# duckietown/gym-duckietown

Measured on AMD Instinct MI355X. Metric: env-steps/sec (4096 envs, 640x480 RGB) at 1/2/4/8 MI355X; % HBM roofline, higher is better.
Workload: dtype f32 raster -> u8 frames; f64 physics

## Files before the change

gym-duckietown_amd/csrc/dtsim_api.hip:

```cpp
#include <hip/hip_runtime.h>

#include <cmath>
#include <cstdarg>
#include <cstdio>
#include <cstdlib>
#include <cstring>
#include <memory>
#include <string>
#include <vector>

#include "dtsim_dev.h"
#include <dlfcn.h>
#include <mutex>

namespace {

thread_local std::string g_err;

int fail(int code, const char* fmt, ...) {
  char buf[512];
  va_list ap;
  va_start(ap, fmt);
  vsnprintf(buf, sizeof buf, fmt, ap);
  va_end(ap);
  g_err = buf;
  return code;
}

#define HIPCHK(expr)                                                                       \
  do {                                                                                     \
    hipError_t _e = (expr);                                                                \
    if (_e != hipSuccess) return fail(DTSIM_E_HIP, "%s failed: %s", #expr, hipGetErrorString(_e)); \
  } while (0)

struct ProfSlot {
  std::vector<std::pair<hipEvent_t, hipEvent_t>> pending;
  std::vector<std::pair<hipEvent_t, hipEvent_t>> free_;
};

struct HipFree {
  void operator()(void* p) const { (void)hipFree(p); }
};
template <typename T>
using DevPtr = std::unique_ptr<T, HipFree>;

template <typename T>
hipError_t dev_alloc(DevPtr<T>& out, size_t n) {
  T* p = nullptr;
  hipError_t e = hipMalloc(&p, sizeof(T) * n);
  if (e == hipSuccess) out.reset(p);
  return e;
}

template <typename T>
hipError_t dev_upload(DevPtr<T>& out, const T* src, size_t n, size_t min_n = 0) {
  DevPtr<T> p;
  hipError_t e = dev_alloc(p, std::max(n, min_n));
  if (e == hipSuccess && n) e = hipMemcpy(p.get(), src, sizeof(T) * n, hipMemcpyHostToDevice);
  if (e == hipSuccess) out = std::move(p);
  return e;
}

template <typename T>
hipError_t dev_grow(DevPtr<T>& buf, size_t n, hipStream_t s) {
  DevPtr<T> p;
  hipError_t e = dev_alloc(p, n);
  if (e == hipSuccess && buf) e = hipStreamSynchronize(s);
  if (e == hipSuccess) buf = std::move(p);
  return e;
}

struct ObserveSlot {
  ObservePlan plan;
  DevPtr<int32_t> d_tab;
};

struct AssetSlot {
  AssetTables T;
  DevPtr<uint32_t> d_texels;
  DevPtr<TexDev> d_tex;
  DevPtr<MeshDev> d_meshes;
  DevPtr<TriDev> d_tris;
};

struct MapSlot : MapScalars {
  DevPtr<uint64_t> d_blobs;
  DevPtr<DynInit> d_dyn;
  bool renderable = false;
  DevPtr<RenderMapDev> d_rmaps;
  DevPtr<uint32_t> d_rtiles;
  DevPtr<TileLds> d_tilerecs;
  DevPtr<ObjInstDev> d_robjs;
  DevPtr<uint8_t> d_qtex;
  DevPtr<uint32_t> d_qtiles;
  DevPtr<char> d_obj[DT_SLABS];
  void release_render() {
    renderable = false;
    d_rmaps.reset(); d_rtiles.reset(); d_tilerecs.reset(); d_robjs.reset(); d_qtex.reset(); d_qtiles.reset();
    for (auto& p : d_obj) p.reset();
  }
};

}

struct dtsim {
  dtsim_config cfg{};
  hipStream_t stream = nullptr;
  bool own_stream = false;
  int N = 0;
  DevPtr<char> slab;
  size_t slab_bytes = 0;
  SimArrays A{};
  bool have_maps = false, have_reset = false;
  MapSlot maps;
  DevPtr<dtsim_init_state> d_states;
  DevPtr<uint8_t> d_mask;
  DevPtr<dtsim_init_state> d_pool;
  int n_pool = 0;
  DevPtr<char> d_actions;
  size_t actions_cap = 0;
  DevPtr<int32_t> d_qenv;
  DevPtr<double> d_qpose;
  DevPtr<dtsim_probe> d_qout;
  DevPtr<dtsim_agent_info> d_agent;
  bool rendered = false;
  bool masked = false;
  RenderParams last_R{};
  bool last_segment = false;
  bool leds_ok = false;
  DevPtr<float> d_leds;
  int leds_cap = 0;
  DevPtr<float> d_lines;
  int lines_cap = 0;
  int render_tables = 0;
  int render_pipe = 0;
  int q_cap = 0;
  DevPtr<uint8_t> frames_own;
  uint8_t* frames = nullptr;
  size_t frames_bytes = 0;
  DevPtr<float> d_lut;
  bool have_lut = false;
  int n_cal = 0;
  bool camera_rand = false;
  DevPtr<int32_t> d_cal_src;
  DevPtr<int32_t> d_env_cal;
  DevPtr<uint8_t> d_scratch;
  AssetSlot assets;
  DevPtr<uint32_t> d_texels_seg;
  DevPtr<uint8_t> d_mesh_seg;
  DevPtr<char> d_render[DT_SLABS];
  bool raster_old = false;
  int step_lanes = 1;
  DevPtr<dtsim_reset_sampler> d_sampler;
  ObserveSlot obs, obsc;
  ProfSlot prof[DTSIM_KERNEL__COUNT];
};

namespace {

template <typename T>
T* carve(char*& p, size_t count) {
  T* r = reinterpret_cast<T*>(p);
  size_t bytes = (count * sizeof(T) + 255) & ~size_t(255);
  p += bytes;
  return r;
}

size_t layout_arrays(SimArrays& A, int N, char* base) {
  char* p = base;
  const size_t n = (size_t)N;
  A.N = N;
  A.pos_x = carve<double>(p, n); A.pos_z = carve<double>(p, n); A.angle = carve<double>(p, n);
  A.q_x = carve<double>(p, n); A.q_y = carve<double>(p, n); A.q_c = carve<double>(p, n); A.q_s = carve<double>(p, n);
  A.vel_u = carve<double>(p, n); A.vel_w = carve<double>(p, n);
  A.ring = carve<double>(p, n * DTSIM_MAX_DELAY * 2);
  A.war = carve<double>(p, n); A.wal = carve<double>(p, n); A.wheel_dist = carve<double>(p, n);
  A.timestamp = carve<double>(p, n); A.speed = carve<double>(p, n); A.reward = carve<double>(p, n);
  A.lane = carve<double>(p, n * 4); A.prox = carve<double>(p, n); A.wheels = carve<double>(p, n * 2);
  A.ob_cx = carve<double>(p, n * DTSIM_MAX_DYNAMIC); A.ob_cz = carve<double>(p, n * DTSIM_MAX_DYNAMIC);
  A.ob_sx = carve<double>(p, n * DTSIM_MAX_DYNAMIC); A.ob_sz = carve<double>(p, n * DTSIM_MAX_DYNAMIC);
  A.ob_corners = carve<double>(p, n * DTSIM_MAX_DYNAMIC * 8);
  A.ob_vel = carve<double>(p, n * DTSIM_MAX_DYNAMIC); A.ob_wait = carve<double>(p, n * DTSIM_MAX_DYNAMIC);
  A.ob_time = carve<double>(p, n * DTSIM_MAX_DYNAMIC); A.ob_angle = carve<double>(p, n * DTSIM_MAX_DYNAMIC);
  A.ob_wiggle = carve<double>(p, n * DTSIM_MAX_DYNAMIC); A.ob_yrot = carve<double>(p, n * DTSIM_MAX_DYNAMIC);
  A.cam = carve<float>(p, n * 6); A.colors = carve<float>(p, n * 16);
  A.ring_head = carve<int32_t>(p, n); A.step_count = carve<int32_t>(p, n);
  A.tile_i = carve<int32_t>(p, n); A.tile_j = carve<int32_t>(p, n);
  A.map_id = carve<int32_t>(p, n); A.episode = carve<int32_t>(p, n);
  A.done = carve<uint8_t>(p, n); A.done_code = carve<uint8_t>(p, n); A.in_lane = carve<uint8_t>(p, n);
  A.ob_active = carve<uint8_t>(p, n * DTSIM_MAX_DYNAMIC);
  A.ob_visible = carve<uint8_t>(p, n * DTSIM_MAX_OBJECTS);
  A.ob_light = carve<uint8_t>(p, n * DTSIM_MAX_OBJECTS);
  A.tl_time = carve<double>(p, n);
  A.ob_cy = carve<double>(p, n * DTSIM_MAX_DYNAMIC);
  A.ob_ext = carve<double>(p, n * DTSIM_MAX_DYNAMIC * 5);
  return (size_t)(p - base);
}

StepParams step_params(const dtsim* h, int n_steps) {
  StepParams P{};
  P.n_steps = n_steps;
  P.frame_skip = h->cfg.frame_skip;
  P.max_steps = h->cfg.max_steps;
  P.delay_steps = h->cfg.delay_steps;
  P.action_mode = h->cfg.action_mode;
  P.actions_f64 = (h->cfg.flags & DTSIM_F_ACTIONS_F64) ? 1 : 0;
  P.auto_reset = ((h->cfg.flags & DTSIM_F_AUTO_RESET) && (h->n_pool > 0 || h->d_sampler)) ? 1 : 0;
  P.n_pool = h->n_pool;
  P.sampler = h->d_sampler.get();
  P.delta_time = h->cfg.delta_time;
  P.robot_speed = h->cfg.robot_speed;
  P.gain = h->cfg.gain; P.trim = h->cfg.trim; P.radius = h->cfg.radius; P.k = h->cfg.k; P.limit = h->cfg.limit;
  P.lanes = h->step_lanes;
  P.light_capture = (h->cfg.flags & DTSIM_F_LIGHT_CAPTURE) ? 1 : 0;
  P.domain_rand = (h->cfg.flags & DTSIM_F_DOMAIN_RAND) ? 1 : 0;
  P.camera_rand = h->camera_rand ? 1 : 0;
  return P;
}

void render_scratch(const dtsim* h, int max_tris, RenderParams* R) {
  void* base[DT_SLABS];
  for (int i = 0; i < DT_SLABS; ++i) base[i] = i < DT_SLAB_STRIS ? h->d_render[i].get() : h->maps.d_obj[i].get();
  dt_render_layout(h->N, h->cfg.cam_width, h->cfg.cam_height, max_tris, nullptr, base, R);
}

void render_scene(const dtsim* h, bool segment, RenderParams* R) {
  const AssetSlot& a = h->assets;
  const MapSlot& m = h->maps;
  R->texels = segment ? h->d_texels_seg.get() : a.d_texels.get(); R->tex = a.d_tex.get();
  R->meshes = a.d_meshes.get(); R->tris = a.d_tris.get();
  R->n_maps = m.M.n_maps;
  R->maps = m.d_rmaps.get(); R->tiles = m.d_rtiles.get(); R->objs = m.d_robjs.get();
  R->max_tris = m.d_obj[DT_SLAB_STRIS] ? m.max_tris : 0;
  R->tile_recs = m.d_tilerecs.get(); R->n_tile_recs = m.n_tilerecs; R->tex_w = m.tex_w; R->tex_h = m.tex_h;
  R->qtex = m.d_qtex.get(); R->qtiles = m.d_qtiles.get(); R->n_qtiles = m.n_qtiles; R->qlog2 = m.qlog2; R->q_per_m = m.q_per_m;
  R->qmax_tiles = std::max(m.grid_rows, m.grid_cols);
}

int check_renderable(const dtsim* h, const char* who) {
  if (h->have_maps && !h->maps.renderable)
    return fail(DTSIM_E_STATE, "%s: dtsim_set_assets replaced the assets the maps were packed against: call dtsim_set_maps again", who);
  return DTSIM_OK;
}

struct ProfScope {
  dtsim* h; int k; hipEvent_t a = nullptr, b = nullptr; bool on;
  ProfScope(dtsim* h_, int k_) : h(h_), k(k_), on((h_->cfg.flags & DTSIM_F_PROFILE) != 0) {
    if (!on) return;
    ProfSlot& s = h->prof[k];
    if (!s.free_.empty()) { a = s.free_.back().first; b = s.free_.back().second; s.free_.pop_back(); }
    else { (void)hipEventCreate(&a); (void)hipEventCreate(&b); }
    (void)hipEventRecord(a, h->stream);
  }
  ~ProfScope() {
    if (!on) return;
    (void)hipEventRecord(b, h->stream);
    h->prof[k].pending.emplace_back(a, b);
  }
};

}

extern "C" {

int dtsim_abi_version(void) { return DTSIM_ABI_VERSION; }
const char* dtsim_last_error(void) { return g_err.c_str(); }

int dtsim_device_count(void) {
  int n = 0;
  hipError_t e = hipGetDeviceCount(&n);
  if (e != hipSuccess) return fail(DTSIM_E_NOGPU, "hipGetDeviceCount: %s", hipGetErrorString(e));
  return n;
}

int dtsim_create(const dtsim_config* cfg, dtsim_t** out) {
  if (!cfg || !out) return fail(DTSIM_E_INVALID, "null argument");
  *out = nullptr;
  if (cfg->struct_size != sizeof(dtsim_config))
    return fail(DTSIM_E_INVALID, "dtsim_config.struct_size %u != %zu (ABI mismatch)", cfg->struct_size,
                sizeof(dtsim_config));
  if (cfg->num_envs <= 0) return fail(DTSIM_E_INVALID, "num_envs must be > 0");
  if (cfg->delay_steps < 0 || cfg->delay_steps > DTSIM_MAX_DELAY)
    return fail(DTSIM_E_LIMIT, "delay_steps %d outside [0,%d]", cfg->delay_steps, DTSIM_MAX_DELAY);
  if (cfg->frame_skip < 1 || cfg->delta_time <= 0) return fail(DTSIM_E_INVALID, "bad frame_skip/delta_time");
  if (cfg->cam_width <= 0 || cfg->cam_height <= 0) return fail(DTSIM_E_INVALID, "bad camera size");
  int ndev = 0;
  if (hipGetDeviceCount(&ndev) != hipSuccess || ndev <= 0)
    return fail(DTSIM_E_NOGPU, "no HIP device visible: libdtsim has no CPU fallback");
  if (cfg->device < 0 || cfg->device >= ndev) return fail(DTSIM_E_INVALID, "device %d out of range", cfg->device);
  HIPCHK(hipSetDevice(cfg->device));
  dtsim* h = new dtsim();
  { const char* ro = getenv("DTSIM_RASTER_OLD"); h->raster_old = ro && ro[0] == '1'; }
  h->step_lanes = cfg->num_envs * 4 <= 32768 ? 4 : cfg->num_envs * 2 <= 32768 ? 2 : 1;
  h->cfg = *cfg;
  h->N = cfg->num_envs;
  if (cfg->stream) { h->stream = (hipStream_t)cfg->stream; }
  else {
    hipError_t e = hipStreamCreateWithFlags(&h->stream, hipStreamNonBlocking);
    if (e != hipSuccess) { delete h; return fail(DTSIM_E_HIP, "hipStreamCreate: %s", hipGetErrorString(e)); }
    h->own_stream = true;
  }
  SimArrays tmp{};
  h->slab_bytes = layout_arrays(tmp, h->N, reinterpret_cast<char*>(4096));
  hipError_t e = dev_alloc(h->slab, h->slab_bytes);
  if (e != hipSuccess) { dtsim_destroy(h); return fail(DTSIM_E_HIP, "hipMalloc(state %zu B): %s", h->slab_bytes, hipGetErrorString(e)); }
  (void)hipMemsetAsync(h->slab.get(), 0, h->slab_bytes, h->stream);
  layout_arrays(h->A, h->N, h->slab.get());
  (void)hipMemsetAsync(h->A.map_id, 0xFF, sizeof(int32_t) * (size_t)h->N, h->stream);
  e = dev_alloc(h->d_states, (size_t)h->N);
  if (e == hipSuccess) e = dev_alloc(h->d_mask, (size_t)h->N);
  if (e != hipSuccess) { dtsim_destroy(h); return fail(DTSIM_E_HIP, "hipMalloc(reset staging): %s", hipGetErrorString(e)); }
  if (cfg->flags & DTSIM_F_RENDER) {
    h->frames_bytes = (size_t)h->N * cfg->cam_height * cfg->cam_width * 3;
    e = dev_alloc(h->frames_own, h->frames_bytes);
    if (e != hipSuccess) { dtsim_destroy(h); return fail(DTSIM_E_HIP, "hipMalloc(frames %zu B): %s", h->frames_bytes, hipGetErrorString(e)); }
    h->frames = h->frames_own.get();
    e = dev_alloc(h->d_lut, 4 * (size_t)cfg->cam_height * cfg->cam_width);
    size_t bytes[DT_SLABS]; dt_render_layout(h->N, cfg->cam_width, cfg->cam_height, 0, bytes);
    for (int i = DT_SLAB_ENV; i <= DT_SLAB_QEND && e == hipSuccess; ++i) e = dev_alloc(h->d_render[i], bytes[i]);
    RenderParams R{}; render_scratch(h, 0, &R);
    if (e == hipSuccess) e = hipMemset(R.dump, 0, sizeof(RenderDump));
    if (e != hipSuccess) { dtsim_destroy(h); return fail(DTSIM_E_HIP, "hipMalloc(render scratch): %s", hipGetErrorString(e)); }
    if (!(cfg->flags & DTSIM_F_DISTORTION)) {
      int rc = dtsim_set_distortion_lut(h, nullptr, nullptr);
      if (rc != DTSIM_OK) { dtsim_destroy(h); return rc; }
    }
  }
  *out = h;
  return DTSIM_OK;
}

void dtsim_destroy(dtsim_t* h) {
  if (!h) return;
  (void)hipSetDevice(h->cfg.device);
  if (h->stream) (void)hipStreamSynchronize(h->stream);
  for (auto& s : h->prof) {
    for (auto& p : s.pending) { (void)hipEventDestroy(p.first); (void)hipEventDestroy(p.second); }
    for (auto& p : s.free_) { (void)hipEventDestroy(p.first); (void)hipEventDestroy(p.second); }
  }
  if (h->own_stream && h->stream) (void)hipStreamDestroy(h->stream);
  delete h;
}

int dtsim_set_assets(dtsim_t* h, const dtsim_texture* textures, int n_textures, const dtsim_mesh* meshes,
                     int n_meshes) {
  if (!h) return fail(DTSIM_E_INVALID, "null handle");
  h->leds_ok = false;
  h->render_tables = 0;
  AssetSlot next;
  std::string err;
  if (int rc = dt_pack_assets(next.T, err, textures, n_textures, meshes, n_meshes)) return fail(rc, "%s", err.c_str());
  HIPCHK(hipSetDevice(h->cfg.device));
  HIPCHK(hipStreamSynchronize(h->stream));
  HIPCHK(dev_upload(next.d_texels, next.T.pool.data(), next.T.pool.size()));
  HIPCHK(dev_upload(next.d_tex, next.T.tex.data(), next.T.tex.size()));
  HIPCHK(dev_upload(next.d_meshes, next.T.meshes.data(), next.T.meshes.size()));
  HIPCHK(dev_upload(next.d_tris, next.T.tris.data(), next.T.tris.size()));
  next.T.tris = {};
  h->assets = std::move(next);
  h->maps.release_render();
  h->d_texels_seg.reset();
  return DTSIM_OK;
}

int dtsim_set_segment_assets(dtsim_t* h, const dtsim_texture* textures, int n_textures, const uint8_t* mesh_rgb, int n_meshes) {
  if (!h) return fail(DTSIM_E_INVALID, "null handle");
  std::vector<uint32_t> pool;
  std::vector<uint8_t> rgbx;
  std::string err;
  if (int rc = dt_pack_segment_texels(pool, rgbx, err, textures, n_textures, mesh_rgb, n_meshes, h->assets.T)) return fail(rc, "%s", err.c_str());
  HIPCHK(hipSetDevice(h->cfg.device));
  HIPCHK(hipStreamSynchronize(h->stream));
  DevPtr<uint32_t> d_texels_seg;
  DevPtr<uint8_t> d_mesh_seg;
  HIPCHK(dev_upload(d_texels_seg, pool.data(), pool.size(), 1));
  HIPCHK(dev_upload(d_mesh_seg, rgbx.data(), rgbx.size()));
  h->d_texels_seg = std::move(d_texels_seg); h->d_mesh_seg = std::move(d_mesh_seg);
  return DTSIM_OK;
}

int dtsim_set_maps(dtsim_t* h, const dtsim_map* maps, int n_maps) {
  if (!h) return fail(DTSIM_E_INVALID, "null argument");
  h->leds_ok = false;
  h->render_tables = 0;
  MapTables T;
  std::string err;
  if (int rc = dt_pack_maps(T, err, maps, n_maps, h->assets.T, (h->cfg.flags & DTSIM_F_RENDER) != 0)) return fail(rc, "%s", err.c_str());
  HIPCHK(hipSetDevice(h->cfg.device));
  HIPCHK(hipStreamSynchronize(h->stream));
  MapSlot next;
  static_cast<MapScalars&>(next) = T;
  HIPCHK(dev_upload(next.d_blobs, T.blobs.data(), T.blobs.size()));
  HIPCHK(dev_upload(next.d_dyn, T.dyn.data(), T.dyn.size()));
  HIPCHK(dev_upload(next.d_rmaps, T.rmaps.data(), T.rmaps.size()));
  HIPCHK(dev_upload(next.d_rtiles, T.rtiles.data(), T.rtiles.size(), 1));
  HIPCHK(dev_upload(next.d_robjs, T.robjs.data(), T.robjs.size(), 1));
  HIPCHK(dev_upload(next.d_tilerecs, T.trecs.data(), T.trecs.size(), 1));
  HIPCHK(dev_upload(next.d_qtex, reinterpret_cast<const uint8_t*>(T.qblocks.data()), T.qblocks.size() * 4));
  HIPCHK(dev_upload(next.d_qtiles, T.qtiles.data(), T.qtiles.size()));
  size_t bytes[DT_SLABS]; dt_render_layout(h->N, h->cfg.cam_width, h->cfg.cam_height, T.max_tris, bytes);
  for (int i = DT_SLAB_STRIS; i <= DT_SLAB_OBJMASK; ++i)
    if (bytes[i] && (h->cfg.flags & DTSIM_F_RENDER)) HIPCHK(dev_alloc(next.d_obj[i], bytes[i]));
  HIPCHK(hipMemsetAsync(h->A.map_id, 0xFF, sizeof(int32_t) * (size_t)h->N, h->stream));
  next.M.blobs = next.d_blobs.get();
  next.M.dyn = next.d_dyn.get();
  next.renderable = true;
  h->maps = std::move(next);
  h->have_maps = true;
  h->have_reset = false;
  return DTSIM_OK;
}

static void drop_luts(dtsim_t* h) {
  h->d_cal_src.reset(); h->d_env_cal.reset(); h->d_scratch.reset();
  h->n_cal = 0;
}

int dtsim_set_distortion_lut(dtsim_t* h, const float* rmapx, const float* rmapy) {
  if (!h) return fail(DTSIM_E_INVALID, "null handle");
  h->leds_ok = false;
  h->render_tables = 0;
  if (!h->d_lut) return fail(DTSIM_E_STATE, "handle created without DTSIM_F_RENDER");
  if ((rmapx == nullptr) != (rmapy == nullptr)) return fail(DTSIM_E_INVALID, "rmapx/rmapy must both be given");
  if (rmapx && !(h->cfg.flags & DTSIM_F_DISTORTION)) return fail(DTSIM_E_STATE, "handle created without DTSIM_F_DISTORTION");
  HIPCHK(hipSetDevice(h->cfg.device));
  const int W = h->cfg.cam_width, H = h->cfg.cam_height;
  std::vector<float> lut;
  dt_pack_lut(W, H, rmapx, rmapy, lut);
  HIPCHK(hipStreamSynchronize(h->stream));
  HIPCHK(dev_upload(h->d_lut, lut.data(), lut.size()));
  drop_luts(h);
  h->have_lut = true;
  return DTSIM_OK;
}

int dtsim_set_distortion_luts(dtsim_t* h, int n_cal, const int32_t* src_index, const int32_t* env_cal, uint32_t flags) {
  if (!h) return fail(DTSIM_E_INVALID, "null handle");
  if (flags & ~(uint32_t)DTSIM_LUTS_CAMERA_RAND) return fail(DTSIM_E_INVALID, "unknown flags 0x%x", flags);
  if (!h->d_lut) return fail(DTSIM_E_STATE, "handle created without DTSIM_F_RENDER");
  if (n_cal == 0) {
    if (src_index || env_cal) return fail(DTSIM_E_INVALID, "n_cal = 0 takes no tables");
    if ((flags & DTSIM_LUTS_CAMERA_RAND) && (h->cfg.flags & DTSIM_F_LIGHT_CAPTURE))
      return fail(DTSIM_E_STATE, "DTSIM_LUTS_CAMERA_RAND with DTSIM_F_LIGHT_CAPTURE is not supported");
    HIPCHK(hipSetDevice(h->cfg.device));
    HIPCHK(hipStreamSynchronize(h->stream));
    drop_luts(h);
    h->camera_rand = (flags & DTSIM_LUTS_CAMERA_RAND) != 0;
    return DTSIM_OK;
  }
  if (n_cal < 0 || !src_index || !env_cal) return fail(DTSIM_E_INVALID, "n_cal %d, src_index %p, env_cal %p", n_cal, (const void*)src_index, (const void*)env_cal);
  if (!(h->cfg.flags & DTSIM_F_DISTORTION)) return fail(DTSIM_E_STATE, "handle created without DTSIM_F_DISTORTION");
  if (h->cfg.flags & DTSIM_F_LIGHT_CAPTURE) return fail(DTSIM_E_STATE, "per-env distortion tables with DTSIM_F_LIGHT_CAPTURE are not supported");
  const int W = h->cfg.cam_width, H = h->cfg.cam_height;
  const size_t hw = (size_t)W * H;
  for (int e = 0; e < h->N; ++e)
    if (env_cal[e] < 0 || env_cal[e] >= n_cal) return fail(DTSIM_E_INVALID, "env_cal[%d] = %d outside [0, %d)", e, env_cal[e], n_cal);
  for (size_t i = 0; i < (size_t)n_cal * hw; ++i)
    if (src_index[i] < -1 || src_index[i] >= (int64_t)hw) return fail(DTSIM_E_INVALID, "src_index[%zu] = %d outside [-1, %zu)", i, src_index[i], hw);
  HIPCHK(hipSetDevice(h->cfg.device));
  DevPtr<int32_t> d_src, d_cal;
  DevPtr<uint8_t> d_scr;
  HIPCHK(dev_upload(d_src, src_index, hw * n_cal));
  HIPCHK(dev_upload(d_cal, env_cal, (size_t)h->N));
  HIPCHK(dev_alloc(d_scr, h->frames_bytes));
  if (int rc = dtsim_set_distortion_lut(h, nullptr, nullptr)) return rc;
  h->d_cal_src = std::move(d_src); h->d_env_cal = std::move(d_cal); h->d_scratch = std::move(d_scr);
  h->n_cal = n_cal;
  h->camera_rand = (flags & DTSIM_LUTS_CAMERA_RAND) != 0;
  return DTSIM_OK;
}

int dtsim_build_remap_maps(int width, int height, int n_cal, const double* K, const double* D, const double* inv_new_K, float* rmapx, float* rmapy) {
  if (width < 5 || height < 5 || n_cal < 0 || (n_cal && (!K || !D || !inv_new_K || !rmapx || !rmapy)))
    return fail(DTSIM_E_INVALID, "dtsim_build_remap_maps: %d x %d, n_cal %d, null tables", width, height, n_cal);
  dt_build_remap_maps(width, height, n_cal, K, D, inv_new_K, rmapx, rmapy);
  return DTSIM_OK;
}

int dtsim_fill_pack_remap(int width, int height, int n_cal, float* rmapx, float* rmapy, const int32_t* hole_order, const int64_t* hole_off,
                          int32_t* src_index) {
  if (width <= 0 || height <= 0 || n_cal < 0 || (n_cal && (!rmapx || !rmapy || !hole_off)))
    return fail(DTSIM_E_INVALID, "dtsim_fill_pack_remap: %d x %d, n_cal %d, null tables", width, height, n_cal);
  const int64_t hw = (int64_t)width * height;
  for (int i = 0; i < n_cal; ++i) {
    if (hole_off[i] < 0 || hole_off[i + 1] < hole_off[i] || (hole_off[i + 1] > hole_off[i] && !hole_order))
      return fail(DTSIM_E_INVALID, "hole_off[%d..%d] = %lld, %lld", i, i + 1, (long long)hole_off[i], (long long)hole_off[i + 1]);
    for (int64_t k = hole_off[i]; k < hole_off[i + 1]; ++k)
      if (hole_order[k] < 0 || hole_order[k] >= hw) return fail(DTSIM_E_INVALID, "hole_order[%lld] = %d outside the image", (long long)k, hole_order[k]);
  }
  dt_fill_pack_remap(width, height, n_cal, rmapx, rmapy, hole_order, hole_off, src_index);
  return DTSIM_OK;
}

static int check_states(const dtsim* h, const dtsim_init_state* st, int n, const uint8_t* mask) {
  for (int e = 0; e < n; ++e) {
    if (mask && !mask[e]) continue;
    const int mid = st[e].map_id & ~DTSIM_MAP_RELOAD;
    if (st[e].map_id < 0 || mid >= h->maps.M.n_maps) return fail(DTSIM_E_INVALID, "state %d: map_id %d out of range", e, st[e].map_id);
  }
  return DTSIM_OK;
}

int dtsim_set_reset_sampler(dtsim_t* h, const dtsim_reset_sampler* sampler) {
  if (!h) return fail(DTSIM_E_INVALID, "null handle");
  HIPCHK(hipSetDevice(h->cfg.device));
  HIPCHK(hipStreamSynchronize(h->stream));
  if (!sampler) {
    h->d_sampler.reset();
    return DTSIM_OK;
  }
  if (!h->have_maps) return fail(DTSIM_E_STATE, "dtsim_set_reset_sampler before dtsim_set_maps");
  if (sampler->max_attempts <= 0 || !(sampler->accept_start_angle_deg > 0))
    return fail(DTSIM_E_INVALID, "sampler: max_attempts %d, accept_start_angle_deg %g", sampler->max_attempts, sampler->accept_start_angle_deg);
  for (int m = 0; m < h->maps.M.n_maps; ++m) {
    const int i = sampler->start_tile[m][0], j = sampler->start_tile[m][1];
    if (i < 0) continue;
    if (i >= h->maps.grid_w[m] || j < 0 || j >= h->maps.grid_h[m]) return fail(DTSIM_E_INVALID, "sampler: start tile (%d,%d) outside map %d", i, j, m);
  }
  HIPCHK(dev_upload(h->d_sampler, sampler, 1));
  return DTSIM_OK;
}

int dtsim_reset_done(dtsim_t* h) {
  if (!h) return fail(DTSIM_E_INVALID, "null handle");
  if (!h->have_reset) return fail(DTSIM_E_STATE, "dtsim_reset_done before the first dtsim_reset");
  if (!h->d_sampler) return fail(DTSIM_E_STATE, "dtsim_reset_done needs dtsim_set_reset_sampler");
  h->rendered = false;
  HIPCHK(hipSetDevice(h->cfg.device));
  {
    ProfScope ps(h, DTSIM_KERNEL_RESET);
    dt_launch_reset(h->stream, h->A, h->maps.M, step_params(h, 0), h->A.done, nullptr);
  }
  HIPCHK(hipGetLastError());
  return DTSIM_OK;
}

int dtsim_reset(dtsim_t* h, const uint8_t* mask, const dtsim_init_state* states) {
  if (!h) return fail(DTSIM_E_INVALID, "null argument");
  if (!h->have_maps) return fail(DTSIM_E_STATE, "dtsim_reset before dtsim_set_maps");
  h->rendered = false;
  if (!states) {
    if (!h->d_sampler) return fail(DTSIM_E_STATE, "dtsim_reset(states = NULL) needs dtsim_set_reset_sampler");
    HIPCHK(hipSetDevice(h->cfg.device));
    if (mask) HIPCHK(hipMemcpyAsync(h->d_mask.get(), mask, (size_t)h->N, hipMemcpyHostToDevice, h->stream));
    {
      ProfScope ps(h, DTSIM_KERNEL_RESET);
      dt_launch_reset(h->stream, h->A, h->maps.M, step_params(h, 0), mask ? h->d_mask.get() : nullptr, nullptr);
    }
    HIPCHK(hipGetLastError());
    HIPCHK(hipStreamSynchronize(h->stream));
    h->have_reset = true;
    return DTSIM_OK;
  }
  int rc = check_states(h, states, h->N, mask);
  if (rc) return rc;
  HIPCHK(hipSetDevice(h->cfg.device));
  HIPCHK(hipMemcpyAsync(h->d_states.get(), states, sizeof(dtsim_init_state) * (size_t)h->N, hipMemcpyHostToDevice, h->stream));
  if (mask) HIPCHK(hipMemcpyAsync(h->d_mask.get(), mask, (size_t)h->N, hipMemcpyHostToDevice, h->stream));
  {
    ProfScope ps(h, DTSIM_KERNEL_RESET);
    dt_launch_reset(h->stream, h->A, h->maps.M, step_params(h, 0), mask ? h->d_mask.get() : nullptr, h->d_states.get());
  }
  HIPCHK(hipGetLastError());
  HIPCHK(hipStreamSynchronize(h->stream));
  h->have_reset = true;
  return DTSIM_OK;
}

int dtsim_set_spawn_pool(dtsim_t* h, const dtsim_init_state* pool, int n_pool) {
  if (!h || !pool || n_pool <= 0) return fail(DTSIM_E_INVALID, "bad pool");
  if (!h->have_maps) return fail(DTSIM_E_STATE, "dtsim_set_spawn_pool before dtsim_set_maps");
  int rc = check_states(h, pool, n_pool, nullptr);
  if (rc) return rc;
  HIPCHK(hipSetDevice(h->cfg.device));
  HIPCHK(hipStreamSynchronize(h->stream));
  HIPCHK(dev_upload(h->d_pool, pool, (size_t)n_pool));
  h->n_pool = n_pool;
  return DTSIM_OK;
}

int dtsim_step(dtsim_t* h, const void* actions, int n_steps, int actions_on_device) {
  return dtsim_step_ex(h, actions, n_steps, actions_on_device, 0u);
}

int dtsim_step_ex(dtsim_t* h, const void* actions, int n_steps, int actions_on_device, uint32_t flags) {
  if (!h || !actions || n_steps <= 0) return fail(DTSIM_E_INVALID, "bad argument");
  if (flags & ~(uint32_t)(DTSIM_STEP_ONE_UPDATE | DTSIM_STEP_POSE_ONLY)) return fail(DTSIM_E_INVALID, "unknown step flags 0x%x", flags);
  if (!h->have_maps || !h->have_reset) return fail(DTSIM_E_STATE, "dtsim_step before dtsim_set_maps/dtsim_reset");
  h->rendered = false;
  HIPCHK(hipSetDevice(h->cfg.device));
  const size_t esz = (h->cfg.flags & DTSIM_F_ACTIONS_F64) ? 8 : 4;
  const size_t bytes = (size_t)n_steps * h->N * 2 * esz;
  const void* dptr = actions;
  if (!actions_on_device) {
    if (bytes > h->actions_cap) {
      HIPCHK(dev_grow(h->d_actions, bytes, h->stream));
      h->actions_cap = bytes;
    }
    HIPCHK(hipMemcpyAsync(h->d_actions.get(), actions, bytes, hipMemcpyHostToDevice, h->stream));
    dptr = h->d_actions.get();
  }
  {
    ProfScope ps(h, DTSIM_KERNEL_STEP);
    StepParams sp = step_params(h, n_steps);
    sp.step_flags = flags;
    dt_launch_step(h->stream, h->A, h->maps.M, sp, dptr, h->d_pool.get());
  }
  HIPCHK(hipGetLastError());
  return DTSIM_OK;
}

int dtsim_render(dtsim_t* h) { return dtsim_render_ex(h, 0u); }

static int render_pass(dtsim_t* h, uint32_t flags, const uint8_t* mask);
int dtsim_render_ex(dtsim_t* h, uint32_t flags) { return render_pass(h, flags, nullptr); }
int dtsim_render_masked(dtsim_t* h, uint32_t flags, const uint8_t* mask) {
  if (!mask) return fail(DTSIM_E_INVALID, "dtsim_render_masked: null mask");
  return render_pass(h, flags, mask);
}

static int render_pass(dtsim_t* h, uint32_t flags, const uint8_t* mask) {
  if (!h) return fail(DTSIM_E_INVALID, "null handle");
  if (flags & ~(uint32_t)(DTSIM_RENDER_SEGMENT | DTSIM_RENDER_GL_FILTER)) return fail(DTSIM_E_INVALID, "unknown render flags 0x%x", flags);
  const bool segment = (flags & DTSIM_RENDER_SEGMENT) != 0;
  if (segment && !h->d_texels_seg) return fail(DTSIM_E_STATE, "DTSIM_RENDER_SEGMENT before dtsim_set_segment_assets");
  if (!h->frames) return fail(DTSIM_E_STATE, "handle created without DTSIM_F_RENDER");
  if (!h->have_maps || !h->have_reset) return fail(DTSIM_E_STATE, "dtsim_render before dtsim_set_maps/dtsim_reset");
  if (!h->have_lut) return fail(DTSIM_E_STATE, "DTSIM_F_DISTORTION set but dtsim_set_distortion_lut was not called");
  if (int rc = check_renderable(h, "dtsim_render")) return rc;
  HIPCHK(hipSetDevice(h->cfg.device));
  RenderParams R{};
  R.N = h->N; R.W = h->cfg.cam_width; R.H = h->cfg.cam_height;
  R.distortion = (h->cfg.flags & DTSIM_F_DISTORTION) ? 1 : 0;
  R.domain_rand = (h->cfg.flags & DTSIM_F_DOMAIN_RAND) ? 1 : 0;
  R.frames = h->n_cal ? h->d_scratch.get() : h->frames;
  R.lut = h->d_lut.get();
  R.segment = segment ? 1 : 0; R.mesh_seg = h->d_mesh_seg.get();
  render_scene(h, segment, &R);
  render_scratch(h, R.max_tris, &R);
  R.light = ((h->cfg.flags & DTSIM_F_LIGHT_CAPTURE) && !R.domain_rand) ? 1 : 0;
  if (flags & DTSIM_RENDER_GL_FILTER) R.qtex = nullptr;
  const int pipe = dt_raster_pipe(R, h->maps.grid_rows, h->maps.grid_cols, h->raster_old);
  {
    ProfScope ps(h, DTSIM_KERNEL_RENDER);
    h->render_tables = dt_launch_render(h->stream, h->A, R, pipe, h->render_tables, mask);
    h->render_pipe = pipe | (R.light ? DTSIM_PIPE_ENV_LIGHT : 0);
    if (h->n_cal) dt_launch_remap_cal(h->stream, h->d_scratch.get(), h->frames, h->d_cal_src.get(), h->d_env_cal.get(), mask, h->N, R.W, R.H);
  }
  HIPCHK(hipGetLastError());
  h->rendered = true; h->last_R = R; h->last_segment = segment; h->leds_ok = true; h->masked = mask != nullptr;
  return DTSIM_OK;
}

int dtsim_draw_lines(dtsim_t* h, const float* lines, const int32_t* env_idx, int n) {
  if (!h || (n > 0 && !lines)) return fail(DTSIM_E_INVALID, "null argument");
  if (n < 0) return fail(DTSIM_E_INVALID, "n = %d", n);
  if (!h->frames) return fail(DTSIM_E_STATE, "handle created without DTSIM_F_RENDER");
  if (int rc = check_renderable(h, "dtsim_draw_lines")) return rc;
  if (!h->have_maps || !h->have_reset || !h->have_lut || !h->rendered) return fail(DTSIM_E_STATE, "dtsim_draw_lines before the first dtsim_render (the pass writes the cameras the lines go through)");
  if (h->masked) return fail(DTSIM_E_STATE, "dtsim_draw_lines after dtsim_render_masked: the post-passes need a full dtsim_render");
  if (h->n_cal) return fail(DTSIM_E_STATE, "dtsim_draw_lines with per-env distortion tables installed (the overlays read the single table)");
  if (n == 0) return DTSIM_OK;
  for (int i = 0; i < n; ++i) {
    const int e = env_idx ? env_idx[i] : 0;
    if (e < 0 || e >= h->N) return fail(DTSIM_E_INVALID, "env_idx[%d] = %d out of range [0, %d)", i, e, h->N);
    if (env_idx && i && env_idx[i] < env_idx[i - 1]) return fail(DTSIM_E_INVALID, "env_idx must be non-decreasing (segments grouped by env)");
  }
  HIPCHK(hipSetDevice(h->cfg.device));
  if (h->lines_cap < n) {
    const int cap = std::max(n, 1024);
    HIPCHK(dev_grow(h->d_lines, 9 * (size_t)cap, h->stream));
    h->lines_cap = cap;
  }
  HIPCHK(hipMemcpyAsync(h->d_lines.get(), lines, sizeof(float) * 9 * (size_t)n, hipMemcpyHostToDevice, h->stream));
  RenderParams R{};
  R.N = h->N; R.W = h->cfg.cam_width; R.H = h->cfg.cam_height; R.frames = h->frames; R.lut = h->d_lut.get();
  render_scratch(h, 0, &R);
  int i0 = 0;
  while (i0 < n) {
    const int e = env_idx ? env_idx[i0] : 0;
    int i1 = i0;
    while (i1 < n && (env_idx ? env_idx[i1] : 0) == e) ++i1;
    dt_launch_overlay_lines(h->stream, R, h->d_lines.get(), i0, i1 - i0, e);
    i0 = i1;
  }
  HIPCHK(hipGetLastError());
  HIPCHK(hipStreamSynchronize(h->stream));
  return DTSIM_OK;
}

int dtsim_draw_leds(dtsim_t* h, const float* spheres, const int32_t* env_idx, int n) {
  if (!h || (n > 0 && !spheres)) return fail(DTSIM_E_INVALID, "null argument");
  if (n < 0) return fail(DTSIM_E_INVALID, "n = %d", n);
  if (!h->frames) return fail(DTSIM_E_STATE, "handle created without DTSIM_F_RENDER");
  if (int rc = check_renderable(h, "dtsim_draw_leds")) return rc;
  if (!h->rendered || !h->leds_ok || h->last_segment) return fail(DTSIM_E_STATE, "dtsim_draw_leds needs a preceding dtsim_render (colour view): it tests the spheres against that pass's scene");
  if (h->masked) return fail(DTSIM_E_STATE, "dtsim_draw_leds after dtsim_render_masked: the post-passes need a full dtsim_render");
  if (h->n_cal) return fail(DTSIM_E_STATE, "dtsim_draw_leds with per-env distortion tables installed (the overlays read the single table)");
  if (n == 0) return DTSIM_OK;
  for (int i = 0; i < n; ++i) {
    const int e = env_idx ? env_idx[i] : 0;
    if (e < 0 || e >= h->N) return fail(DTSIM_E_INVALID, "env_idx[%d] = %d out of range [0, %d)", i, e, h->N);
    if (env_idx && i && env_idx[i] < env_idx[i - 1]) return fail(DTSIM_E_INVALID, "env_idx must be non-decreasing (spheres grouped by env, in draw order)");
  }
  HIPCHK(hipSetDevice(h->cfg.device));
  if (h->leds_cap < n) {
    const int cap = std::max(n, 256);
    HIPCHK(dev_grow(h->d_leds, 8 * (size_t)cap, h->stream));
    h->leds_cap = cap;
  }
  HIPCHK(hipMemcpyAsync(h->d_leds.get(), spheres, sizeof(float) * 8 * (size_t)n, hipMemcpyHostToDevice, h->stream));
  RenderParams R = h->last_R;
  R.frames = h->frames;
  int i0 = 0;
  while (i0 < n) {
    const int e = env_idx ? env_idx[i0] : 0;
    int i1 = i0;
    while (i1 < n && (env_idx ? env_idx[i1] : 0) == e) ++i1;
    dt_launch_overlay_leds(h->stream, R, h->d_leds.get(), i0, i1 - i0, e);
    i0 = i1;
  }
  HIPCHK(hipGetLastError());
  HIPCHK(hipStreamSynchronize(h->stream));
  return DTSIM_OK;
}

void* dtsim_frames_devptr(dtsim_t* h) { return h ? h->frames : nullptr; }
size_t dtsim_frames_bytes(const dtsim_t* h) { return h ? h->frames_bytes : 0; }

int dtsim_bind_frames(dtsim_t* h, void* devptr) {
  if (!h) return fail(DTSIM_E_INVALID, "null handle");
  if (!h->frames_own) return fail(DTSIM_E_STATE, "handle created without DTSIM_F_RENDER");
  h->frames = devptr ? (uint8_t*)devptr : h->frames_own.get();
  return DTSIM_OK;
}

namespace {
typedef int (*nccl_allgather_fn)(const void*, void*, size_t, int , void* , hipStream_t);
typedef const char* (*nccl_errstr_fn)(int);
nccl_allgather_fn g_nccl_allgather = nullptr;
nccl_errstr_fn g_nccl_errstr = nullptr;
std::once_flag g_nccl_once;
std::string g_nccl_why;
void resolve_rccl() {
  std::call_once(g_nccl_once, [] {
    void* lib = nullptr;
    for (const char* name : {"librccl.so.1", "librccl.so", "/opt/rocm/lib/librccl.so.1"}) {
      lib = dlopen(name, RTLD_NOW | RTLD_GLOBAL);
      if (lib) break;
      if (const char* e = dlerror()) g_nccl_why = e;
    }
    if (!lib) return;
    g_nccl_allgather = reinterpret_cast<nccl_allgather_fn>(dlsym(lib, "ncclAllGather"));
    g_nccl_errstr = reinterpret_cast<nccl_errstr_fn>(dlsym(lib, "ncclGetErrorString"));
    if (!g_nccl_allgather) { const char* e = dlerror(); g_nccl_why = e ? e : "ncclAllGather not exported"; }
  });
}
}

int dtsim_allgather_frames(dtsim_t* h, void* nccl_comm, void* recv, const void* send, size_t send_bytes) {
  if (!h || !nccl_comm || !recv) return fail(DTSIM_E_INVALID, "bad argument");
  if (!send) {
    if (!h->frames) return fail(DTSIM_E_STATE, "handle created without DTSIM_F_RENDER");
    send = h->frames;
    send_bytes = dtsim_frames_bytes(h);
  }
  if (send_bytes == 0) return fail(DTSIM_E_INVALID, "empty send buffer");
  resolve_rccl();
  if (!g_nccl_allgather)
    return fail(DTSIM_E_STATE, "librccl.so (ncclAllGather) could not be loaded: %s", g_nccl_why.empty() ? "library or symbol not found" : g_nccl_why.c_str());
  HIPCHK(hipSetDevice(h->cfg.device));
  const int rc = g_nccl_allgather(send, recv, send_bytes,  1, nccl_comm, h->stream);
  if (rc != 0) return fail(DTSIM_E_HIP, "ncclAllGather: %s", g_nccl_errstr ? g_nccl_errstr(rc) : "error");
  return DTSIM_OK;
}

static int observe_run(dtsim_t* h, bool cubic, void* out, int out_h, int out_w, int flags, const uint8_t* mask,
                       const int32_t* bounds_x, const int32_t* taps_x, int ksize_x, const int32_t* bounds_y, const int32_t* taps_y, int ksize_y) {
  if (!h || !out) return fail(DTSIM_E_INVALID, "bad argument");
  if (!h->frames) return fail(DTSIM_E_STATE, "handle created without DTSIM_F_RENDER");
  const int W = h->cfg.cam_width, H = h->cfg.cam_height;
  ObserveSlot& slot = cubic ? h->obsc : h->obs;
  ObservePlan next;
  std::string err;
  int rc = cubic ? dt_observe_pack_cubic(next, err, W, H, h->N, out_h, out_w, bounds_x, taps_x, bounds_y, taps_y)
                 : dt_observe_pack(next, err, W, H, h->N, out_h, out_w, bounds_x, taps_x, ksize_x, bounds_y, taps_y, ksize_y);
  if (rc != DTSIM_OK) return fail(rc, "%s", err.c_str());
  HIPCHK(hipSetDevice(h->cfg.device));
  if (!slot.d_tab || !next.same_tables(slot.plan)) {
    rc = cubic ? dt_observe_plan_cubic(next, err)
               : dt_observe_plan(next, err, getenv("DTSIM_OBSERVE_STAGED") != nullptr, getenv("DTSIM_OBSERVE_GENERIC") != nullptr);
    if (rc != DTSIM_OK) return fail(rc, "%s", err.c_str());
    HIPCHK(hipStreamSynchronize(h->stream));
    HIPCHK(dev_upload(slot.d_tab, next.tab.data(), next.tab.size()));
    slot.plan = std::move(next);
  }
  const ObservePlan& plan = slot.plan;
  ObserveParams P = plan.P;
  P.chw = (flags & DTSIM_OBS_CHW) ? 1 : 0; P.f32 = (flags & DTSIM_OBS_F32) ? 1 : 0;
  P.frames = h->frames; P.out = out;
  const int32_t* tab = slot.d_tab.get();
  P.bx = tab + plan.off_bx; P.kkx = tab + plan.off_kkx; P.by = tab + plan.off_by; P.kky = tab + plan.off_kky;
  {
    ProfScope ps(h, DTSIM_KERNEL_OBSERVE);
    dt_launch_observe(h->stream, plan, P, mask);
  }
  HIPCHK(hipGetLastError());
  return DTSIM_OK;
}

int dtsim_observe(dtsim_t* h, void* out, int out_h, int out_w, int flags,
                  const int32_t* bounds_x, const int32_t* taps_x, int ksize_x,
                  const int32_t* bounds_y, const int32_t* taps_y, int ksize_y) {
  return observe_run(h, false, out, out_h, out_w, flags, nullptr, bounds_x, taps_x, ksize_x, bounds_y, taps_y, ksize_y);
}
int dtsim_observe_masked(dtsim_t* h, void* out, int out_h, int out_w, int flags, const uint8_t* mask,
                         const int32_t* bounds_x, const int32_t* taps_x, int ksize_x,
                         const int32_t* bounds_y, const int32_t* taps_y, int ksize_y) {
  if (!mask) return fail(DTSIM_E_INVALID, "dtsim_observe_masked: null mask");
  return observe_run(h, false, out, out_h, out_w, flags, mask, bounds_x, taps_x, ksize_x, bounds_y, taps_y, ksize_y);
}
int dtsim_observe_cubic(dtsim_t* h, void* out, int out_h, int out_w, int flags,
                        const int32_t* first_x, const int32_t* taps_x, const int32_t* first_y, const int32_t* taps_y) {
  return observe_run(h, true, out, out_h, out_w, flags, nullptr, first_x, taps_x, 4, first_y, taps_y, 4);
}
int dtsim_observe_cubic_masked(dtsim_t* h, void* out, int out_h, int out_w, int flags, const uint8_t* mask,
                               const int32_t* first_x, const int32_t* taps_x, const int32_t* first_y, const int32_t* taps_y) {
  if (!mask) return fail(DTSIM_E_INVALID, "dtsim_observe_cubic_masked: null mask");
  return observe_run(h, true, out, out_h, out_w, flags, mask, first_x, taps_x, 4, first_y, taps_y, 4);
}

int dtsim_copy_rows(dtsim_t* h, void* dst, const void* src, size_t row_bytes, const uint8_t* mask) {
  if (!h || !dst || !src || !mask) return fail(DTSIM_E_INVALID, "dtsim_copy_rows: null argument");
  if (row_bytes == 0) return DTSIM_OK;
  HIPCHK(hipSetDevice(h->cfg.device));
  dt_launch_copy_rows(h->stream, h->N, dst, src, row_bytes, mask);
  HIPCHK(hipGetLastError());
  return DTSIM_OK;
}

int dtsim_query(dtsim_t* h, int n, const int32_t* env_idx, const double* poses, double safety_factor,
                dtsim_probe* out) {
  if (!h || n <= 0 || !env_idx || !poses || !out) return fail(DTSIM_E_INVALID, "bad argument");
  if (!h->have_maps || !h->have_reset) return fail(DTSIM_E_STATE, "dtsim_query before dtsim_set_maps/dtsim_reset");
  for (int i = 0; i < n; ++i)
    if (env_idx[i] < 0 || env_idx[i] >= h->N) return fail(DTSIM_E_INVALID, "env_idx[%d]=%d out of range", i, env_idx[i]);
  HIPCHK(hipSetDevice(h->cfg.device));
  if (n > h->q_cap) {
    const int cap = n < 256 ? 256 : n;
    HIPCHK(dev_grow(h->d_qenv, cap, h->stream));
    HIPCHK(dev_grow(h->d_qpose, 3 * (size_t)cap, h->stream));
    HIPCHK(dev_grow(h->d_qout, cap, h->stream));
    h->q_cap = cap;
  }
  HIPCHK(hipMemcpyAsync(h->d_qenv.get(), env_idx, sizeof(int32_t) * n, hipMemcpyHostToDevice, h->stream));
  HIPCHK(hipMemcpyAsync(h->d_qpose.get(), poses, sizeof(double) * 3 * n, hipMemcpyHostToDevice, h->stream));
  {
    ProfScope ps(h, DTSIM_KERNEL_QUERY);
    dt_launch_query(h->stream, h->A, h->maps.M, step_params(h, 0), n, h->d_qenv.get(), h->d_qpose.get(), safety_factor, h->d_qout.get());
  }
  HIPCHK(hipGetLastError());
  HIPCHK(hipMemcpyAsync(out, h->d_qout.get(), sizeof(dtsim_probe) * n, hipMemcpyDeviceToHost, h->stream));
  HIPCHK(hipStreamSynchronize(h->stream));
  return DTSIM_OK;
}

namespace {
struct FieldDesc { void* base; size_t elem; int comps; size_t comp_stride_elems; bool planar; };

bool field_desc(dtsim* h, int field, FieldDesc& d) {
  const SimArrays& A = h->A;
  const size_t N = (size_t)h->N;
  switch (field) {
    case DTSIM_FIELD_ANGLE: d = {A.angle, 8, 1, N, true}; return true;
    case DTSIM_FIELD_REWARD: d = {A.reward, 8, 1, N, true}; return true;
    case DTSIM_FIELD_DONE: d = {A.done, 1, 1, N, true}; return true;
    case DTSIM_FIELD_DONE_CODE: d = {A.done_code, 1, 1, N, true}; return true;
    case DTSIM_FIELD_STEP_COUNT: d = {A.step_count, 4, 1, N, true}; return true;
    case DTSIM_FIELD_LANE: d = {A.lane, 8, 4, N, true}; return true;
    case DTSIM_FIELD_IN_LANE: d = {A.in_lane, 1, 1, N, true}; return true;
    case DTSIM_FIELD_PROX: d = {A.prox, 8, 1, N, true}; return true;
    case DTSIM_FIELD_SPEED: d = {A.speed, 8, 1, N, true}; return true;
    case DTSIM_FIELD_TIMESTAMP: d = {A.timestamp, 8, 1, N, true}; return true;
    case DTSIM_FIELD_WHEELS: d = {A.wheels, 8, 2, N, true}; return true;
    case DTSIM_FIELD_MAP_ID: d = {A.map_id, 4, 1, N, true}; return true;
    case DTSIM_FIELD_OBJ_ACTIVE: d = {A.ob_active, 1, DTSIM_MAX_DYNAMIC, N, true}; return true;
    case DTSIM_FIELD_OBJ_YROT: d = {A.ob_yrot, 8, DTSIM_MAX_DYNAMIC, N, true}; return true;
    case DTSIM_FIELD_OBJ_VISIBLE: d = {A.ob_visible, 1, DTSIM_MAX_OBJECTS, N, true}; return true;
    case DTSIM_FIELD_OBJ_LIGHT: d = {A.ob_light, 1, DTSIM_MAX_OBJECTS, N, true}; return true;
    case DTSIM_FIELD_OBJ_Y: d = {A.ob_cy, 8, DTSIM_MAX_DYNAMIC, N, true}; return true;
    case DTSIM_FIELD_EPISODE: d = {A.episode, 4, 1, N, true}; return true;
    case DTSIM_FIELD_CAMERA: d = {A.cam, 4, 6, N, true}; return true;
    case DTSIM_FIELD_COLORS: d = {A.colors, 4, 16, N, true}; return true;
    case DTSIM_FIELD_WHEEL_DIST: d = {A.wheel_dist, 8, 1, N, true}; return true;
    default: return false;
  }
}

size_t public_bytes(const dtsim* h, int field) {
  const size_t N = (size_t)h->N;
  switch (field) {
    case DTSIM_FIELD_POS: return N * 3 * 8;
    case DTSIM_FIELD_TILE: return N * 2 * 4;
    case DTSIM_FIELD_OBJ_CENTER: return N * DTSIM_MAX_DYNAMIC * 2 * 8;
    case DTSIM_FIELD_OBJ_PARAMS: return N * DTSIM_MAX_DYNAMIC * 3 * 8;
    case DTSIM_FIELD_OBJ_EXTRA: return N * DTSIM_MAX_DYNAMIC * 5 * 8;
    case DTSIM_FIELD_STATE_BLOB: return h->slab_bytes;
    case DTSIM_FIELD_RENDER_POS: return N * 4;
    case DTSIM_FIELD_RENDER_PIPE: return N * 4;
    default: {
      FieldDesc d;
      if (!field_desc(const_cast<dtsim*>(h), field, d)) return 0;
      return N * d.comps * d.elem;
    }
  }
}

int xfer_planar(dtsim* h, void* const* bases, int ncomp, size_t elem, void* host, bool to_host) {
  const size_t N = (size_t)h->N;
  std::vector<char> tmp(N * elem);
  for (int c = 0; c < ncomp; ++c) {
    if (to_host) {
      if (bases[c] == nullptr) { memset(tmp.data(), 0, tmp.size()); }
      else {
        hipError_t e = hipMemcpy(tmp.data(), bases[c], N * elem, hipMemcpyDeviceToHost);
        if (e != hipSuccess) return fail(DTSIM_E_HIP, "hipMemcpy D2H: %s", hipGetErrorString(e));
      }
      for (size_t i = 0; i < N; ++i) memcpy((char*)host + (i * ncomp + c) * elem, tmp.data() + i * elem, elem);
    } else {
      if (bases[c] == nullptr) continue;
      for (size_t i = 0; i < N; ++i) memcpy(tmp.data() + i * elem, (const char*)host + (i * ncomp + c) * elem, elem);
      hipError_t e = hipMemcpy(bases[c], tmp.data(), N * elem, hipMemcpyHostToDevice);
      if (e != hipSuccess) return fail(DTSIM_E_HIP, "hipMemcpy H2D: %s", hipGetErrorString(e));
    }
  }
  return DTSIM_OK;
}

__global__ void k_agent_info(SimArrays A, int e, dtsim_agent_info* out) {
  const size_t N = A.N;
  dtsim_agent_info r;
  r.pos[0] = A.pos_x[e]; r.pos[1] = 0.0; r.pos[2] = A.pos_z[e];
  r.angle = A.angle[e]; r.speed = A.speed[e]; r.timestamp = A.timestamp[e];
// ... 126 lines not shown
```

gym-duckietown_amd/csrc/dtsim_dev.h:

```cpp
#pragma once
#include <hip/hip_runtime.h>
#include <stdint.h>
#include "../../include/dtsim.h"
#include "observe_plan.h"
#include "scene_tables.h"

#define DT_CAMERA_FORWARD_DIST 0.066
#define DT_ROBOT_WIDTH (0.13 + 0.02)
#define DT_ROBOT_LENGTH 0.18
#define DT_CENTER_SHIFT (DT_CAMERA_FORWARD_DIST - (DT_ROBOT_LENGTH / 2))
#define DT_SAFETY_RAD_MULT 1.8
#define DT_AGENT_SAFETY_RAD ((DT_ROBOT_LENGTH / 2) * DT_SAFETY_RAD_MULT)
#define DT_REWARD_INVALID_POSE (-1000.0)

struct SimArrays {
  int32_t N;
  double *pos_x, *pos_z, *angle;
  double *q_x, *q_y, *q_c, *q_s, *vel_u, *vel_w;
  double *ring;
  double *war, *wal;
  double *wheel_dist;
  double *timestamp, *speed;
  double *reward;
  double *lane;
  double *prox;
  double *wheels;
  double *ob_cx, *ob_cz, *ob_sx, *ob_sz;
  double *ob_corners;
  double *ob_vel, *ob_wait, *ob_time, *ob_angle, *ob_wiggle, *ob_yrot;
  float *cam;
  float *colors;
  int32_t *ring_head, *step_count, *tile_i, *tile_j, *map_id, *episode;
  uint8_t *done, *done_code, *in_lane;
  uint8_t *ob_active;
  uint8_t *ob_visible;
  uint8_t *ob_light;
  double *ob_cy;
  double *ob_ext;
  double *tl_time;
};

struct StepParams {
  int32_t n_steps, frame_skip, max_steps, delay_steps;
  int32_t action_mode, actions_f64, auto_reset, n_pool;
  uint32_t step_flags;
  int32_t light_capture, domain_rand;
  int32_t lanes;
  int32_t camera_rand;
  const dtsim_reset_sampler* sampler;
  double delta_time, robot_speed;
  double gain, trim, radius, k, limit;
};

void dt_launch_step(hipStream_t s, const SimArrays& A, const MapSet& M, const StepParams& P,
                    const void* actions, const dtsim_init_state* pool);
void dt_launch_reset(hipStream_t s, const SimArrays& A, const MapSet& M, const StepParams& P,
                     const uint8_t* mask, const dtsim_init_state* states);
void dt_launch_query(hipStream_t s, const SimArrays& A, const MapSet& M, const StepParams& P, int n,
                     const int32_t* env_idx, const double* poses, double safety_factor, dtsim_probe* out);

struct alignas(16) ScreenTri {
  float bx0, bx1, by0, by1;
  float sx[3], sy[3], iw[3];
  float inv_area;
  int32_t index;
  int32_t pad;
  float cw[3][3];
  float uw[3], vw[3];
  int32_t tex;
};
static_assert(sizeof(ScreenTri) == 128, "ScreenTri is 128 bytes");
struct ObjBox { float bx0, bx1, by0, by1; int32_t first, count, pad[2]; };

#ifndef DT_WAVE_W
#define DT_WAVE_W 128
#endif
#ifndef DT_PPT
#define DT_PPT 4
#endif
#ifndef DT_V3_WW
#define DT_V3_WW 128
#endif
#define DT_TILE_W DT_WAVE_W
#define DT_TILE_H (4 * (64 * DT_PPT / DT_WAVE_W))
#ifndef DT_ENVS_PER_BLOCK
#define DT_ENVS_PER_BLOCK 64
#endif
#ifndef DT_ITEM_B
#define DT_ITEM_B 8
#endif
#define DT_ITEMS_PER_WG (4 * (DT_PPT * DT_ENVS_PER_BLOCK) / DT_ITEM_B)
static inline size_t dt_raster_tiles(int W, int H) {
  return (size_t)((W + DT_TILE_W - 1) / DT_TILE_W) * (size_t)((H + DT_TILE_H - 1) / DT_TILE_H);
}
static inline size_t dt_raster_groups(int N, int W, int H) { return dt_raster_tiles(W, H) * (((size_t)N + DT_ENVS_PER_BLOCK - 1) / DT_ENVS_PER_BLOCK); }

struct RenderParams {
  int32_t N, W, H, distortion;
  int32_t domain_rand, n_maps, n_tile_recs;
  int32_t tex_w, tex_h;
  const TileLds* tile_recs;
  uint8_t* frames;
  const float* lut;
  const uint32_t* texels;
  const TexDev* tex;
  const RenderMapDev* maps;
  const uint32_t* tiles;
  const ObjInstDev* objs;
  const MeshDev* meshes;
  const TriDev* tris;
  void* envcam;
  int32_t max_tris, segment;
  ScreenTri* stris;
  float4* tribox;
  ObjBox* objbox;
  float* blockbox;
  unsigned long long* objmask;
  uint2* objrange;
  uint16_t* queue;
  int32_t* qcount;
  uint16_t* qend;
  int32_t* work;
  uint32_t* items;
  uint32_t* items2;
  const uint8_t* mesh_seg;
  const uint8_t* qtex;
  const uint32_t* qtiles;
  int32_t n_qtiles, qlog2;
  float q_per_m;
  int32_t qmax_tiles;
  int32_t* envpos;
  void* dump;
  void* pixtab;
  void* envv;
  void* envd;
  int32_t q3_rows;
  int32_t light;
};
#define DT_WORK_INTS 8
#define DT_WORK_LIVE 7
struct RenderDump { uint8_t store[64 * 16]; };
enum RenderSlab { DT_SLAB_ENV, DT_SLAB_PIX, DT_SLAB_QUEUE, DT_SLAB_QCOUNT, DT_SLAB_ITEMS, DT_SLAB_QEND, DT_SLAB_STRIS, DT_SLAB_OBJBOX, DT_SLAB_OBJMASK, DT_SLABS };
void dt_render_layout(int N, int W, int H, int max_tris, size_t* bytes, void* const* base = nullptr, RenderParams* R = nullptr);
int dt_raster_pipe(RenderParams& R, int grid_rows, int grid_cols, bool raster_old);
int dt_launch_render(hipStream_t s, const SimArrays& A, const RenderParams& R, int pipe, int tables, const uint8_t* mask = nullptr);
void dt_launch_overlay_lines(hipStream_t s, const RenderParams& R, const float* d_lines, int first, int count, int env);
void dt_launch_overlay_leds(hipStream_t s, const RenderParams& R, const float* d_spheres, int first, int count, int env);
void dt_launch_remap_cal(hipStream_t s, const uint8_t* scratch, uint8_t* frames, const int32_t* src, const int32_t* env_cal,
                         const uint8_t* mask, int N, int W, int H);
void dt_build_remap_maps(int W, int H, int n_cal, const double* K, const double* D, const double* ir, float* rx, float* ry);
void dt_fill_pack_remap(int W, int H, int n_cal, float* rx, float* ry, const int32_t* order, const int64_t* order_off, int32_t* src_index);

void dt_launch_observe(hipStream_t s, const ObservePlan& plan, const ObserveParams& P, const uint8_t* mask = nullptr);
void dt_launch_copy_rows(hipStream_t s, int N, void* dst, const void* src, size_t row_bytes, const uint8_t* mask);
```

gym-duckietown_amd/csrc/render.hip:

```cpp
#include "dtsim_dev.h"
#include <hip/hip_fp16.h>
#include <type_traits>
#include <algorithm>
#include <map>
#include <mutex>
#include <tuple>

typedef int v3_i32x4 __attribute__((ext_vector_type(4)));
typedef uint32_t v3_u32x3 __attribute__((ext_vector_type(3)));
__device__ void v3_buf_store_v3i32(v3_u32x3 data, v3_i32x4 rsrc, int voffset, int soffset, int aux) __asm("llvm.amdgcn.raw.buffer.store.v3i32");
typedef uint32_t v3_u32x4 __attribute__((ext_vector_type(4)));
__device__ void v3_buf_store_v4i32(v3_u32x4 data, v3_i32x4 rsrc, int voffset, int soffset, int aux) __asm("llvm.amdgcn.raw.buffer.store.v4i32");
#define V3_RSRC_W3 0x00027000
__device__ inline v3_i32x4 v3_rsrc(const void* p, uint32_t bytes) {
  v3_i32x4 r;
  r.x = (int)(uint32_t)reinterpret_cast<uintptr_t>(p); r.y = (int)((reinterpret_cast<uintptr_t>(p) >> 32) & 0xFFFFu); r.z = (int)bytes; r.w = V3_RSRC_W3;
  return r;
}


#define RB 256
#define PPT DT_PPT
#define WAVE_W DT_WAVE_W
#define SLOT_X(k, l) (((k) * 64 + (l)) % WAVE_W)
// ... 1030 lines not shown
  }
}

template <bool OBJ>
struct ChunkObjMasks {
  static_assert(ENVS_PER_BLOCK <= 64, "one lane per env of the chunk");
  uint32_t lo, hi;
  int e0;
  __device__ void load(const RenderParams& R, const int e0_, const int e1, const int n_blk, const int blk, const int lane) {
    uint32_t om_lo = 0u, om_hi = 0u;
    if (OBJ && lane < e1 - e0_) {
      const unsigned long long v = R.objmask[(size_t)(e0_ + lane) * n_blk + blk];
      om_lo = (uint32_t)v; om_hi = (uint32_t)(v >> 32);
    }
    lo = om_lo; hi = om_hi; e0 = e0_;
  }
  __device__ unsigned long long of(const int e) const {
    if (!OBJ) return 0ull;
    return ((unsigned long long)(uint32_t)__builtin_amdgcn_readlane((int)hi, e - e0) << 32) | (uint32_t)__builtin_amdgcn_readlane((int)lo, e - e0);
  }
};

__device__ inline uint32_t spxy_pack(const float4& l, const int W, const int H) {
  const float sx = (l.x + 1.f) * 0.5f * (float)W, sy = (1.f - l.y) * 0.5f * (float)H;
  return (uint32_t)__half_as_ushort(__float2half(sx)) | ((uint32_t)__half_as_ushort(__float2half(sy)) << 16);
}
__device__ inline void spxy_unpack(uint32_t t, float& sx, float& sy) {
  asm volatile("" : "+v"(t));
  sx = __half2float(__ushort_as_half((unsigned short)(t & 0xFFFFu)));
  sy = __half2float(__ushort_as_half((unsigned short)(t >> 16)));
}

struct alignas(4) U3 { uint32_t a, b, c; };

template <bool DR, bool OBJ>
__global__ __launch_bounds__(RB) void k_raster(RenderParams R, const EnvCam* __restrict__ cams,
                                               const EnvFast* __restrict__ fasts, uint8_t* __restrict__ frames, const uint32_t* __restrict__ texels,
                                               const float4* __restrict__ lut, const RenderMapDev* __restrict__ maps,
                                               const TileLds* __restrict__ tile_recs, uint16_t* __restrict__ queue,
                                               int32_t* __restrict__ qcount) {
  extern __shared__ uint32_t s_mem[];
  TileLds* s_tiles = reinterpret_cast<TileLds*>(s_mem);

  const int tid = threadIdx.x;
  const int npix = R.W * R.H;
  const int tiles_x = (R.W + DT_TILE_W - 1) / DT_TILE_W, n_tiles = tiles_x * ((R.H + DT_TILE_H - 1) / DT_TILE_H);
  const int tile = blockIdx.x % n_tiles;
  const int chunk = blockIdx.x / n_tiles;
  const int e0 = chunk * ENVS_PER_BLOCK;
  const int e1 = min(e0 + ENVS_PER_BLOCK, R.N);
  {
    const uint32_t* src = reinterpret_cast<const uint32_t*>(tile_recs);
    for (int i = tid; i < R.n_tile_recs * (int)(sizeof(TileLds) / 4); i += RB) s_mem[i] = src[i];
  }
  __syncthreads();

  const int wave = tid >> 6, lane = tid & 63;
  const int blk = tile * 4 + __builtin_amdgcn_readfirstlane(wave);
  const int tile_x0 = (tile % tiles_x) * DT_TILE_W;
  const int wave_y0 = (tile / tiles_x) * DT_TILE_H + wave * (WAVE_PIX / WAVE_W);
  const float aspect = (float)R.W / (float)R.H;
  const float ex_n = 0.375f * 2.f / (float)R.W * 1.01f, ey_n = 0.375f * 2.f / (float)R.H * 1.01f;

  float nx[PPT], ny[PPT];
  bool ok[PPT];
#pragma unroll
  for (int k = 0; k < PPT; ++k) {
    if (tile_x0 + SLOT_X(k, lane) < R.W && wave_y0 + SLOT_Y(k, lane) < R.H) {
      const float4 l = lut[(wave_y0 + SLOT_Y(k, lane)) * R.W + tile_x0 + SLOT_X(k, lane)];
      nx[k] = l.x; ny[k] = l.y; ok[k] = l.z != 0.f;
    } else { nx[k] = ny[k] = 0.f; ok[k] = false; }
  }
  PixInv pv[PPT];
  if (!DR) {
    const CamShared cs = default_cam(aspect);
#pragma unroll
    for (int k = 0; k < PPT; ++k) {
      pv[k] = pix_inv(nx[k], ny[k], ok[k], cs.tx, cs.ty, cs.sth, cs.cth, cs.Cy, cs.L, ex_n, ey_n);
      pv[k].ndl = fminf(fmaf(cs.dif, pv[k].ndl, cs.base), 1.f);
    }
  }

  float spx[PPT], spy[PPT];
  float wbx0 = 1e30f, wbx1 = -1e30f, wby0 = 1e30f, wby1 = -1e30f;
#pragma unroll
  for (int k = 0; k < PPT; ++k) {
    spx[k] = (nx[k] + 1.f) * 0.5f * (float)R.W; spy[k] = (1.f - ny[k]) * 0.5f * (float)R.H;
    if (ok[k]) { wbx0 = fminf(wbx0, spx[k]); wbx1 = fmaxf(wbx1, spx[k]); wby0 = fminf(wby0, spy[k]); wby1 = fmaxf(wby1, spy[k]); }
  }
#pragma unroll
  for (int d = 32; d > 0; d >>= 1) {
    wbx0 = fminf(wbx0, __shfl_xor(wbx0, d)); wbx1 = fmaxf(wbx1, __shfl_xor(wbx1, d));
    wby0 = fminf(wby0, __shfl_xor(wby0, d)); wby1 = fmaxf(wby1, __shfl_xor(wby1, d));
  }

  uint16_t* w_queue = queue + ((size_t)blockIdx.x * (RB / 64) + wave) * QREGION;
  int qn = 0, qo = 0;
  int qend_v = 0;
  uint32_t* s_px = s_mem + R.n_tile_recs * (sizeof(TileLds) / 4) + wave * WAVE_PIX;
  const int st_x = tile_x0 + (lane * 4) % WAVE_W, st_y = wave_y0 + (lane * 4) / WAVE_W;
  const bool aligned_rows = (R.W & 3) == 0;
  const bool st_ok = aligned_rows && lane * 4 < WAVE_PIX && st_x < R.W && st_y < R.H;
  const size_t st_off = ((size_t)st_y * R.W + st_x) * 3;
  const int tw1 = R.tex_w + 1, xmask = R.tex_w - 1, ymask = R.tex_h - 1;

  uint32_t om_lo = 0u, om_hi = 0u;
  if (OBJ && lane < e1 - e0) {
    const unsigned long long v = R.objmask[(size_t)(e0 + lane) * (n_tiles * 4) + blk];
    om_lo = (uint32_t)v; om_hi = (uint32_t)(v >> 32);
  }
  for (int e = e0; e < e1; ++e) {
    const EnvFast f = fasts[e];
    float base0 = 0.f, base1 = 0.f, base2 = 0.f, dif0 = 0.f, dif1 = 0.f, dif2 = 0.f;
    if (DR) {
      const EnvCam c = cams[e];
      base0 = c.base[0]; base1 = c.base[1]; base2 = c.base[2]; dif0 = c.dif[0]; dif1 = c.dif[1]; dif2 = c.dif[2];
      const DrCam dc = dr_cam(c, ex_n, ey_n);
#pragma unroll
      for (int k = 0; k < PPT; ++k)
        pv[k] = pix_inv_dr(nx[k], ny[k], ok[k], dc, c.L);
    }
    const uint32_t hor_rgb = f.hor_rgb;
    const float A = f.A, B = f.B, Cxi = f.Cxi, Czi = f.Czi;

    uint32_t px[PPT];
    bool edge[PPT], oedge[PPT];
#pragma unroll
    for (int k = 0; k < PPT; ++k) oedge[k] = false;
    bool any_work = false;
#pragma unroll
    for (int k = 0; k < PPT; ++k) any_work |= (pv[k].flags & (PF_VALID | PF_SKY)) == PF_VALID;
    if (!__ballot(any_work)) {
#pragma unroll
      for (int k = 0; k < PPT; ++k) { px[k] = (pv[k].flags & PF_VALID) ? hor_rgb : 0u; edge[k] = false; }
    } else {
      float fx[PPT], fz[PPT], gxs[PPT], gzs[PPT];
      bool cand[PPT], is_tile[PPT], fast[PPT];
      bool need_ground = false;
      TileLds tr[PPT];
#pragma unroll
      for (int k = 0; k < PPT; ++k) {
        const PixInv& p = pv[k];
        const float gx = fmaf(p.lf, B, fmaf(p.lr, A, Cxi));
        const float gz = fmaf(p.lf, -A, fmaf(p.lr, B, Czi));
        gxs[k] = gx; gzs[k] = gz;
        fx[k] = __builtin_amdgcn_fractf(gx); fz[k] = __builtin_amdgcn_fractf(gz);
        const int ti = flr_i32(gx), tj = flr_i32(gz);
        cand[k] = (p.flags & (PF_VALID | PF_SKY | PF_ALWAYS_EDGE)) == PF_VALID;
        const bool ingrid = cand[k] & ((p.flags & PF_TILE_OK) != 0) & ((unsigned)ti < (unsigned)f.gw) & ((unsigned)tj < (unsigned)f.gh);
        const int idx = ingrid ? f.tile_off + (int)__umul24(tj, f.gw) + ti : f.tile_off;
        tr[k] = s_tiles[idx];
        is_tile[k] = ingrid & (tr[k].flags != 0u);
        const float dmax = absmax(fx[k] - 0.5f, fz[k] - 0.5f);
        const bool inside = dmax < fmaf(-p.mrg, f.its, 0.5f);
        fast[k] = ingrid & (tr[k].flags == 3u) & inside;
        need_ground |= cand[k] & !is_tile[k];
        edge[k] = ((p.flags & (PF_VALID | PF_ALWAYS_EDGE)) == (PF_VALID | PF_ALWAYS_EDGE)) | (is_tile[k] & !fast[k]);
      }
      bool any_fast = false;
#pragma unroll
      for (int k = 0; k < PPT; ++k) any_fast |= fast[k];
      if (!__ballot(any_fast)) {
#pragma unroll
        for (int k = 0; k < PPT; ++k) px[k] = (pv[k].flags & PF_VALID) ? hor_rgb : 0u;
      } else {
      uint2 top2[PPT], bot2[PPT];
      int wxi[PPT], wyi[PPT];
      const uint8_t* tex_bytes = reinterpret_cast<const uint8_t*>(texels);
      const uint32_t row_bytes = (uint32_t)tw1 * 4u;
#pragma unroll
      for (int k = 0; k < PPT; ++k) {
        const float x = fmaf(tr[k].mxz, fz[k], fmaf(tr[k].mxx, fx[k], tr[k].ox));
        const float y = fmaf(tr[k].myz, fz[k], fmaf(tr[k].myx, fx[k], tr[k].oy));
        const int xf = gl_fix(x), yf = gl_fix(y);
        wxi[k] = xf & 255; wyi[k] = yf & 255;
        const uint32_t x0 = (uint32_t)((xf >> 8) & xmask), y0 = (uint32_t)((yf >> 8) & ymask);
        const uint32_t off = (__umul24(y0, (uint32_t)tw1) + x0 + tr[k].tex_off) << 2;
        __builtin_memcpy(&top2[k], tex_bytes + off, 8);
        __builtin_memcpy(&bot2[k], tex_bytes + (off + row_bytes), 8);
      }
#pragma unroll
      for (int k = 0; k < PPT; ++k) {
        const PixInv& p = pv[k];
        int T[3];
        gl_linear_rgb(top2[k].x, top2[k].y, bot2[k].x, bot2[k].y, wxi[k], wyi[k], T);
        float v0 = (float)T[0], v1 = (float)T[1], v2 = (float)T[2];
        if (DR) {
          v0 *= fminf(fmaf(dif0, p.ndl, base0), 1.f);
          v1 *= fminf(fmaf(dif1, p.ndl, base1), 1.f);
          v2 *= fminf(fmaf(dif2, p.ndl, base2), 1.f);
        } else { v0 *= p.ndl; v1 *= p.ndl; v2 *= p.ndl; }
        uint32_t rgb = 0;
        rgb = __builtin_amdgcn_cvt_pk_u8_f32(v0, 0, rgb);
        rgb = __builtin_amdgcn_cvt_pk_u8_f32(v1, 1, rgb);
        rgb = __builtin_amdgcn_cvt_pk_u8_f32(v2, 2, rgb);
        px[k] = fast[k] ? rgb : ((p.flags & PF_VALID) ? hor_rgb : 0u);
      }
      }
      if (__ballot(need_ground)) {
        const EnvCam c = cams[e];
#pragma unroll
        for (int k = 0; k < PPT; ++k) {
          const PixInv& p = pv[k];
          const bool gcand = cand[k] & !is_tile[k];
          const float wx = gxs[k] * f.ts, wz = gzs[k] * f.ts;
          const float wxg = fmaf(f.kg, wx - f.Cx, f.Cx), wzg = fmaf(f.kg, wz - f.Cz, f.Cz);
          const bool clear = (wx < -p.mrg) | (wx > f.gw_m + p.mrg) | (wz < -p.mrg) | (wz > f.gh_m + p.mrg);
          const bool inq = (fabsf(wxg) + 2.f * p.mrg < GROUND_HALF) & (fabsf(wzg) + 2.f * p.mrg < GROUND_HALF);
          const bool gfast = gcand & clear & inq & ((p.flags & PF_GROUND_OK) != 0);
          const float ndl = ground_ndl(c, wxg, wzg);
          uint32_t rgb = 0;
          rgb = __builtin_amdgcn_cvt_pk_u8_f32(c.gnd[0] * fminf(c.base[0] + c.dif[0] * ndl, 1.f), 0, rgb);
          rgb = __builtin_amdgcn_cvt_pk_u8_f32(c.gnd[1] * fminf(c.base[1] + c.dif[1] * ndl, 1.f), 1, rgb);
          rgb = __builtin_amdgcn_cvt_pk_u8_f32(c.gnd[2] * fminf(c.base[2] + c.dif[2] * ndl, 1.f), 2, rgb);
          px[k] = gfast ? rgb : px[k];
          edge[k] = edge[k] | (gcand & !gfast);
        }
      }
    }

    if (OBJ) {
      unsigned long long om = ((unsigned long long)(uint32_t)__builtin_amdgcn_readlane((int)om_hi, e - e0) << 32) |
                              (uint32_t)__builtin_amdgcn_readlane((int)om_lo, e - e0);
      const ObjBox* boxes = R.objbox + (size_t)e * DTSIM_MAX_OBJECTS;
      while (om) {
        const ObjBox ob = boxes[__builtin_ctzll(om)];
        om &= om - 1ull;
#pragma unroll
        for (int k = 0; k < PPT; ++k)
          if (ok[k] && spx[k] >= ob.bx0 && spx[k] <= ob.bx1 && spy[k] >= ob.by0 && spy[k] <= ob.by1) oedge[k] = true;
      }
    }

    if (aligned_rows) {
#pragma unroll
      for (int k = 0; k < PPT; ++k) s_px[k * 64 + lane] = px[k];
      const uint4 q = *reinterpret_cast<const uint4*>(s_px + (lane * 4) % WAVE_PIX);
      if (st_ok) {
        uint32_t* d32 = reinterpret_cast<uint32_t*>(frames + (size_t)e * npix * 3 + st_off);
        __builtin_nontemporal_store(q.x | (q.y << 24), d32);
        __builtin_nontemporal_store((q.y >> 8) | (q.z << 16), d32 + 1);
        __builtin_nontemporal_store((q.z >> 16) | (q.w << 8), d32 + 2);
      }
    } else {
#pragma unroll
      for (int k = 0; k < PPT; ++k)
        if (tile_x0 + SLOT_X(k, lane) < R.W && wave_y0 + SLOT_Y(k, lane) < R.H) {
          uint8_t* dst = frames + ((size_t)e * npix + (size_t)(wave_y0 + SLOT_Y(k, lane)) * R.W + tile_x0 + SLOT_X(k, lane)) * 3;
          dst[0] = (uint8_t)px[k]; dst[1] = (uint8_t)(px[k] >> 8); dst[2] = (uint8_t)(px[k] >> 16);
        }
    }

    bool any_edge = false, any_oedge = false;
#pragma unroll
    for (int k = 0; k < PPT; ++k) { any_oedge |= oedge[k]; edge[k] &= !oedge[k]; any_edge |= edge[k]; }
    const uint32_t etag = (uint32_t)(e - e0) << 8;
    if (OBJ && __ballot(any_oedge)) {
#pragma unroll
      for (int k = 0; k < PPT; ++k) {
        const bool ek = oedge[k];
        const unsigned long long mk = __ballot(ek);
        if (ek) {
          const int rank = __builtin_amdgcn_mbcnt_hi((uint32_t)(mk >> 32), __builtin_amdgcn_mbcnt_lo((uint32_t)mk, 0u));
          w_queue[QREGION - 1 - (qo + rank)] = (uint16_t)(etag | QE_PLANE_EDGE | (uint32_t)(k * 64 + lane));
        }
        qo += __popcll(mk);
      }
    }
    if (__ballot(any_edge)) {
#pragma unroll
      for (int k = 0; k < PPT; ++k) {
        const bool ek = edge[k];
        const unsigned long long mk = __ballot(ek);
        if (ek) {
          const int rank = __builtin_amdgcn_mbcnt_hi((uint32_t)(mk >> 32), __builtin_amdgcn_mbcnt_lo((uint32_t)mk, 0u));
          w_queue[qn + rank] = (uint16_t)(etag | (uint32_t)(k * 64 + lane));
        }
        qn += __popcll(mk);
      }
    }
    if (OBJ) qend_v = lane >= e - e0 ? qo : qend_v;
  }
  if (lane == 0) qcount[blockIdx.x * (RB / 64) + wave] = qn;
  if (OBJ && lane < ENVS_PER_BLOCK) R.qend[((size_t)blockIdx.x * (RB / 64) + wave) * ENVS_PER_BLOCK + lane] = (uint16_t)qend_v;
  __shared__ int s_nb[RB / 64], s_no[RB / 64];
  if (lane == 0) { s_nb[wave] = (qn + 63) >> 6; s_no[wave] = qo; }
  __syncthreads();
  if (tid == 0) {
    int nb = 0, no = 0;
#pragma unroll
    for (int r = 0; r < RB / 64; ++r) { nb += s_nb[r]; no += s_no[r]; }
    if (nb > 0) {
      const int ni = (nb + ITEM_B - 1) / ITEM_B;
      const int pos = atomicAdd(R.work, ni);
      for (int i = 0; i < ni; ++i) R.items[pos + i] = (uint32_t)blockIdx.x * ITEMS_PER_WG + (uint32_t)i;
    }
    if (OBJ && no > 0) push_obj_items(R, (uint32_t)blockIdx.x);
  }
}


struct alignas(16) PixTab { float lr, lf, lit; uint32_t mi; };
struct alignas(16) SampTab { uint32_t dlr[2], dlf[2]; uint32_t flags; uint32_t pad[3]; };
static_assert(sizeof(PixTab) == 16 && sizeof(SampTab) == 32, "table records");

__global__ void k_pix_setup(RenderParams R, const float4* __restrict__ lut, PixTab* __restrict__ pixtab, SampTab* __restrict__ samptab) {
  const int pix = blockIdx.x * blockDim.x + threadIdx.x;
  if (pix >= R.W * R.H) return;
  const float aspect = (float)R.W / (float)R.H;
  const float ex_n = 0.375f * 2.f / (float)R.W * 1.01f, ey_n = 0.375f * 2.f / (float)R.H * 1.01f;
  const CamShared cs = default_cam(aspect);
  const float4 l = lut[pix];
  const bool ok = l.z != 0.f;
  const PixInv p = pix_inv(l.x, l.y, ok, cs.tx, cs.ty, cs.sth, cs.cth, cs.Cy, cs.L, ex_n, ey_n);
  const bool cand = (p.flags & (PF_VALID | PF_SKY)) == PF_VALID;
  const bool plain = cand && !(p.flags & PF_ALWAYS_EDGE) && (p.flags & PF_TILE_OK) && (p.flags & PF_GROUND_OK);
  PixTab t;
  t.lr = p.lr; t.lf = p.lf;
  t.lit = !ok ? -1.f : !cand ? 0.f : fminf(fmaf(cs.dif, p.ndl, cs.base), 1.f);
  t.mi = plain ? (uint32_t)fminf(floorf(fmaf(p.mrg, R.q_per_m, 0.5f)), 65534.f) : 0xFFFFu;
  t.mi |= (uint32_t)__half_as_ushort(__float2half_ru(fminf(p.mrg, 60000.f))) << 16;
  pixtab[pix] = t;
  SampTab sp;
  const float ox[4] = {-0.125f, 0.375f, -0.375f, 0.125f};
  const float oy[4] = {0.375f, 0.125f, -0.125f, -0.375f};
  const float sxn = 2.f / (float)R.W, syn = 2.f / (float)R.H;
  sp.flags = 0u;
  float dlr[4], dlf[4];
#pragma unroll
  for (int k = 0; k < 4; ++k) {
    const Ray r = make_ray(l.x + ox[k] * sxn, l.y - oy[k] * syn, cs.tx, cs.ty, cs.sth, cs.cth);
    dlr[k] = dlf[k] = 0.f;
    if (r.yla < 0.f) {
      const float inv = frcp(-r.yla);
      const float t = cs.Cy * inv, tg = (cs.Cy - GROUND_Y) * inv;
      dlr[k] = fminf(fmaxf(t * r.xe - p.lr, -60000.f), 60000.f); dlf[k] = fminf(fmaxf(t * r.fwd - p.lf, -60000.f), 60000.f);
      if (t >= NEAR_Z && t <= FAR_Z) sp.flags |= 1u << k;
      if (tg >= NEAR_Z && tg <= FAR_Z) sp.flags |= 16u << k;
    }
  }
#pragma unroll
  for (int j = 0; j < 2; ++j) {
    sp.dlr[j] = (uint32_t)__half_as_ushort(__float2half_rn(dlr[2 * j])) | ((uint32_t)__half_as_ushort(__float2half_rn(dlr[2 * j + 1])) << 16);
    sp.dlf[j] = (uint32_t)__half_as_ushort(__float2half_rn(dlf[2 * j])) | ((uint32_t)__half_as_ushort(__float2half_rn(dlf[2 * j + 1])) << 16);
  }
  sp.pad[0] = __float_as_uint(t.lr); sp.pad[1] = __float_as_uint(t.lf); sp.pad[2] = __float_as_uint(t.lit);
  samptab[pix] = sp;
}

__device__ inline float med3f(float x, float lo, float hi) { return __builtin_amdgcn_fmed3f(x, lo, hi); }

#define Q8_SNAP 32768.f
#define Q8_LIT (1.f / 256.f)
__device__ inline uint32_t q8_bits(float X) { return __float_as_uint(X + Q8_SNAP); }
__device__ inline uint32_t q8_cell(uint32_t b) { return (b >> 8) & 0x7FFFu; }
__device__ inline float q8_frac(uint32_t b) { return (float)(b & 255u); }
__device__ inline uint32_t q8_rec256(uint32_t xb, uint32_t zb, uint32_t m) {
  uint32_t P, Zs;
  asm("v_mul_u32_u24_sdwa %0, %1, %2 dst_sel:DWORD dst_unused:UNUSED_PAD src0_sel:BYTE_1 src1_sel:DWORD" : "=v"(P) : "v"(xb), "s"(0x1010u));
  asm("v_lshlrev_b32_sdwa %0, 6, %1 dst_sel:DWORD dst_unused:UNUSED_PAD src0_sel:DWORD src1_sel:BYTE_1" : "=v"(Zs) : "v"(zb));
  return ((P & 0xFC030u) | Zs) & m;
}
typedef float f2_t __attribute__((ext_vector_type(2)));
__device__ inline f2_t fma2(f2_t a, f2_t b, f2_t c) { return __builtin_elementwise_fma(a, b, c); }
__device__ inline uint32_t quad_weights8(float a8, float b8, float l) {
#pragma clang fp contract(off)
  const float u = a8 * l, v = fmaf(l, 256.f, -u);
  const float w11 = u * b8, w01 = v * b8, w10 = fmaf(u, 256.f, -w11), w00 = fmaf(v, 256.f, -w01);
  uint32_t W = __builtin_amdgcn_cvt_pk_u8_f32(w00, 0, 0u);
  W = __builtin_amdgcn_cvt_pk_u8_f32(w10, 1, W);
  W = __builtin_amdgcn_cvt_pk_u8_f32(w01, 2, W);
  return __builtin_amdgcn_cvt_pk_u8_f32(w11, 3, W);
}
__device__ inline float env_lit8(const EnvL& l, float lr, float lf, float base8) {
#pragma clang fp contract(off)
  const float dx = l.Lr - lr, dz = l.Lf - lf;
  return fminf(fmaf(l.kd8, frsq(fmaf(dx, dx, fmaf(dz, dz, l.h2))), base8), Q8_LIT);
}
__device__ inline float env_base8() { return default_cam(1.f).base * Q8_LIT; }
__device__ inline f2_t env_lit8_2(const EnvL& l, const f2_t lr, const f2_t lf) {
#pragma clang fp contract(off)
  const f2_t dx = f2_t{l.Lr, l.Lr} - lr, dz = f2_t{l.Lf, l.Lf} - lf;
  const f2_t d2 = fma2(dx, dx, fma2(dz, dz, f2_t{l.h2, l.h2}));
  const float b8 = env_base8();
  const f2_t t = fma2(f2_t{l.kd8, l.kd8}, f2_t{frsq(d2.x), frsq(d2.y)}, f2_t{b8, b8});
  return f2_t{fminf(t.x, Q8_LIT), fminf(t.y, Q8_LIT)};
}
__device__ inline uint32_t quad_filter(const uint4& q, float a8, float b8, float I) {
  const uint32_t W = quad_weights8(a8, b8, I * Q8_LIT);
  const uint32_t vr = __builtin_amdgcn_udot4(q.x, W, 128u, false), vg = __builtin_amdgcn_udot4(q.y, W, 128u, false),
                 vb = __builtin_amdgcn_udot4(q.z, W, 128u, false);
  const uint32_t rg = __builtin_amdgcn_perm(vg, vr, 0x0c0c0501u);
  return __builtin_amdgcn_perm(vb, rg, 0x0c050100u);
}
__device__ inline void quad_filter3(const uint4& q, float a8, float b8, float I, float out[3]) {
  const uint32_t W = quad_weights8(a8, b8, I * Q8_LIT);
  out[0] = (float)__builtin_amdgcn_udot4(q.x, W, 0u, false) * (1.f / 256.f);
  out[1] = (float)__builtin_amdgcn_udot4(q.y, W, 0u, false) * (1.f / 256.f);
  out[2] = (float)__builtin_amdgcn_udot4(q.z, W, 0u, false) * (1.f / 256.f);
}

#define RQ_LIST 256
__device__ inline void store_rgb(uint8_t* frames, const int npix, const int e, const int pix, const uint32_t rgb) {
  uint8_t* dst = frames + ((size_t)e * npix + pix) * 3;
  const bool odd = (reinterpret_cast<uintptr_t>(dst) & 1u) != 0u;
  uint8_t* p8 = odd ? dst : dst + 2;
  uint16_t* p16 = reinterpret_cast<uint16_t*>(odd ? dst + 1 : dst);
  *p8 = (uint8_t)(odd ? rgb : rgb >> 16);
  *p16 = (uint16_t)(odd ? rgb >> 8 : rgb);
}
template <bool S256, bool LIGHT = false>
__device__ inline void resolve_region_q(const RenderParams& R, const EnvCam* __restrict__ cams, const EnvQ* __restrict__ envq,
                                        const PixTab* __restrict__ pixtab, const SampTab* __restrict__ samptab,
                                        const uint8_t* __restrict__ qtex, const uint32_t* s_qt, uint32_t* w_list,
                                        const uint16_t* w_queue, const int n, const int e0, const int tile_x0, const int wave_y0,
                                        const int lane, const EnvL* __restrict__ envl) {
  const int npix = R.W * R.H;
  const int LS = R.qlog2;
  const uint32_t SM = (1u << LS) - 1u;
  const float Sf = (float)(1 << LS), lo = 0.5f * Sf;
  const char* qtb = reinterpret_cast<const char*>(s_qt);
  const uint32_t tex_min = 32u;

  auto tile_entry = [&](float X, float Z, const float Xhi, const float Zhi, const uint32_t tab_b, const uint32_t pitch4, uint32_t& ta,
                        float& ox, float& oz) -> uint2 {
    const float Xc = med3f(X - 0.5f, lo, Xhi), Zc = med3f(Z - 0.5f, lo, Zhi);
    const uint32_t ti = (uint32_t)flr_i32(Xc) >> LS, tj = (uint32_t)flr_i32(Zc) >> LS;
    ox = (float)(ti << LS) + 0.5f; oz = (float)(tj << LS) + 0.5f;
    ta = (ti << 3) + __umul24(tj, pitch4) + tab_b;
    return *reinterpret_cast<const uint2*>(qtb + ta);
  };
  auto tile_quad = [&](const uint2 te, const uint32_t xb, const uint32_t zb) -> uint4 {
    if (S256) return *reinterpret_cast<const uint4*>(qtex + (te.x | q8_rec256(xb, zb, te.y)));
    const uint32_t local = (((q8_cell(zb) & SM) << LS) | (q8_cell(xb) & SM)) & te.y;
    return *reinterpret_cast<const uint4*>(qtex + (te.x + (local << 4)));
  };

  auto phase1 = [&](auto utag, const int r0) __attribute__((always_inline)) -> int {
    constexpr int U = decltype(utag)::value;
    int n_list = 0;
    bool have[U], interior[U], tagged[U], skip[U];
    int pix[U], el[U], env[U];
    PixTab pt[U];
    float Xu[U], Zu[U];
    uint2 te_c[U];
#pragma unroll
    for (int u = 0; u < U; ++u) {
      have[u] = r0 + u * 64 + lane < n;
      const int qoff = r0 + u * 64 + lane;
      const uint32_t ent = have[u] ? (uint32_t)__builtin_nontemporal_load(w_queue + qoff) : 0u;
      el[u] = (int)((ent >> 8) & 63u);
      tagged[u] = (ent & QE_ALWAYS_EDGE) != 0u;
      skip[u] = !__ballot(have[u] && !tagged[u]);
      const int lp = (int)(ent & 255u);
      pix[u] = (wave_y0 + lp / WAVE_W) * R.W + tile_x0 + lp % WAVE_W;
    }
    float4 qa[U];
    uint4 qb[U];
#pragma unroll
    for (int u = 0; u < U; ++u) {
      qa[u] = make_float4(0.f, 0.f, 0.f, 0.f); qb[u] = make_uint4(0u, 0u, 0u, 0u); env[u] = 0;
      pt[u] = PixTab{0.f, 0.f, 0.f, 0xFFFFu};
      if (skip[u]) continue;
      pt[u] = pixtab[pix[u]];
      const EnvQ* fq = envq + min(e0 + el[u], R.N - 1);
      qa[u] = *reinterpret_cast<const float4*>(&fq->A);
      qb[u] = *reinterpret_cast<const uint4*>(&fq->Xhi);
      const uint4 qd = *reinterpret_cast<const uint4*>(&fq->reach);
      env[u] = (int)qd.y;
      if constexpr (LIGHT) { const EnvL l = envl[min(e0 + el[u], R.N - 1)]; pt[u].lit = pt[u].lit > 0.f ? 256.f * env_lit8(l, pt[u].lr, pt[u].lf, env_base8()) : pt[u].lit; }
    }
#pragma unroll
    for (int u = 0; u < U; ++u) {
      interior[u] = false; Xu[u] = Zu[u] = 0.f; te_c[u] = make_uint2(0u, 0u);
      if (skip[u]) continue;
      const float A = qa[u].x, B = qa[u].y, Cx = qa[u].z, Cz = qa[u].w;
      const float Xhi = __uint_as_float(qb[u].x), Zhi = __uint_as_float(qb[u].y);
      Xu[u] = fmaf(pt[u].lf, B, fmaf(pt[u].lr, A, Cx)); Zu[u] = fmaf(pt[u].lf, -A, fmaf(pt[u].lr, B, Cz));
      uint32_t ta_c;
      float ox, oz;
      te_c[u] = tile_entry(Xu[u], Zu[u], Xhi, Zhi, qb[u].z, qb[u].w, ta_c, ox, oz);
      const float mrg = __half2float(__ushort_as_half((unsigned short)(pt[u].mi >> 16)));
      const float ux = Xu[u] - ox, uz = Zu[u] - oz;
      const float d = fminf(fminf(ux, Sf - ux), fminf(uz, Sf - uz));
      const bool in_range = Xu[u] - 0.5f >= lo && Xu[u] - 0.5f <= Xhi && Zu[u] - 0.5f >= lo && Zu[u] - 0.5f <= Zhi;
      interior[u] = have[u] && !tagged[u] && in_range && te_c[u].x >= tex_min && pt[u].lit > 0.f && (pt[u].mi & 0xFFFFu) < 0xFFF0u && d > mrg * R.q_per_m;
    }
    uint4 qc[U];
#pragma unroll
    for (int u = 0; u < U; ++u) { qc[u] = make_uint4(0u, 0u, 0u, 0u); if (!skip[u] && interior[u]) qc[u] = tile_quad(te_c[u], q8_bits(Xu[u]), q8_bits(Zu[u])); }
#pragma unroll
    for (int u = 0; u < U; ++u) {
      if (!skip[u]) {
        const uint32_t rgb = quad_filter(qc[u], q8_frac(q8_bits(Xu[u])), q8_frac(q8_bits(Zu[u])), pt[u].lit);
        if (interior[u]) store_rgb(R.frames, npix, env[u], pix[u], rgb);
      }
      const bool msaa = have[u] && !interior[u];
      const unsigned long long mm = __ballot(msaa);
      if (msaa) w_list[n_list + __builtin_amdgcn_mbcnt_hi((uint32_t)(mm >> 32), __builtin_amdgcn_mbcnt_lo((uint32_t)mm, 0u))] = (uint32_t)pix[u] | ((uint32_t)el[u] << 24);
      n_list += __popcll(mm);
    }
    return n_list;
  };
  for (int r0 = 0; r0 < n; r0 += RQ_LIST) {
    const int rem = n - r0;
    const int n_list = rem > 128 ? phase1(std::integral_constant<int, 4>{}, r0)
                     : rem > 64 ? phase1(std::integral_constant<int, 2>{}, r0) : phase1(std::integral_constant<int, 1>{}, r0);
    __builtin_amdgcn_fence(__ATOMIC_RELEASE, "wavefront");
    __builtin_amdgcn_wave_barrier();
    __builtin_amdgcn_fence(__ATOMIC_ACQUIRE, "wavefront");
    for (int l0 = 0; l0 < n_list; l0 += 64) {
      const bool have = l0 + lane < n_list;
      const uint32_t le = have ? w_list[l0 + lane] : 0u;
      const int pix = (int)(le & 0xFFFFFFu), el = (int)(le >> 24);
      const SampTab sp = samptab[pix];
      const PixTab pt = pixtab[pix];
      const EnvQ* fq = envq + min(e0 + el, R.N - 1);
      const float A = fq->A, B = fq->B, Cx = fq->Cx, Cz = fq->Cz, Xhi = fq->Xhi, Zhi = fq->Zhi;
      const uint32_t tab_b = fq->tab_b, pitch4 = fq->pitch4;
      const int e = (int)fq->env;
      const EnvCam* c = cams + e;
      const float wCx = c->Cx, wCy = c->Cy, wCz = c->Cz, sa = c->sa, ca = c->ca;
      const float kg = (wCy - GROUND_Y) / wCy;
      const float Xu = fmaf(pt.lf, B, fmaf(pt.lr, A, Cx)), Zu = fmaf(pt.lf, -A, fmaf(pt.lr, B, Cz));
      const uint32_t xub = q8_bits(Xu), zub = q8_bits(Zu);
      const float ax = q8_frac(xub), az = q8_frac(zub);
      float lit = pt.lit > 0.f ? pt.lit : 0.55f;
      if constexpr (LIGHT) { if (pt.lit > 0.f) lit = 256.f * env_lit8(envl[min(e0 + el, R.N - 1)], pt.lr, pt.lf, env_base8()); }
      uint32_t key[4];
      uint2 te[4];
      int n_sky = 0, n_gnd = 0;
      float gwx = 0.f, gwz = 0.f;
#pragma unroll
      for (int s = 3; s >= 0; --s) {
        const uint32_t hr = sp.dlr[s >> 1], hf = sp.dlf[s >> 1];
        const float slr = pt.lr + __half2float(__ushort_as_half((unsigned short)((s & 1) ? hr >> 16 : hr)));
        const float slf = pt.lf + __half2float(__ushort_as_half((unsigned short)((s & 1) ? hf >> 16 : hf)));
        const float Xs = fmaf(slf, B, fmaf(slr, A, Cx)), Zs = fmaf(slf, -A, fmaf(slr, B, Cz));
        uint32_t ta;
        float sox, soz;
        te[s] = tile_entry(Xs, Zs, Xhi, Zhi, tab_b, pitch4, ta, sox, soz);
        const bool s_in = Xs - 0.5f >= lo && Xs - 0.5f <= Xhi && Zs - 0.5f >= lo && Zs - 0.5f <= Zhi;
        const bool is_tile = ((sp.flags >> s) & 1u) && s_in && te[s].x != 0u;
        const float wx = kg * (slr * sa + slf * ca) + wCx, wz = kg * (slr * ca - slf * sa) + wCz;
        const bool is_gnd = !is_tile && ((sp.flags >> (4 + s)) & 1u) && fabsf(wx) <= GROUND_HALF && fabsf(wz) <= GROUND_HALF;
        key[s] = !have ? 0u : is_tile ? 2u + ta : is_gnd ? 1u : 0u;
        n_sky += key[s] == 0u; n_gnd += key[s] == 1u;
        if (is_gnd) { gwx = wx; gwz = wz; }
      }
      float acc[3];
      acc[0] = (float)n_sky * c->hor[0]; acc[1] = (float)n_sky * c->hor[1]; acc[2] = (float)n_sky * c->hor[2];
      if (__ballot(have && n_gnd > 0)) {
        if (pt.lit > 0.f && (pt.lr != 0.f || pt.lf != 0.f)) {
          gwx = kg * (pt.lr * sa + pt.lf * ca) + wCx; gwz = kg * (pt.lr * ca - pt.lf * sa) + wCz;
        }
        const float a_ = fminf(fmaxf((gwx + GROUND_HALF) * (0.5f / GROUND_HALF), 0.f), 1.f);
        const float b_ = fminf(fmaxf((gwz + GROUND_HALF) * (0.5f / GROUND_HALF), 0.f), 1.f);
        const float n0 = c->gndl[0] + a_ * (c->gndl[1] - c->gndl[0]), n1 = c->gndl[2] + a_ * (c->gndl[3] - c->gndl[2]);
        const float ndl = n0 + b_ * (n1 - n0);
#pragma unroll
        for (int k = 0; k < 3; ++k) acc[k] += (float)n_gnd * (c->gnd[k] * fminf(c->base[k] + c->dif[k] * ndl, 1.f));
      }
      uint32_t todo = 0u;
#pragma unroll
      for (int s = 0; s < 4; ++s) todo |= key[s] >= 2u ? (1u << s) : 0u;
      while (__ballot(todo != 0u)) {
        const int s0 = todo ? __builtin_ctz(todo) : 0;
        const uint32_t k0 = s0 == 0 ? key[0] : s0 == 1 ? key[1] : s0 == 2 ? key[2] : key[3];
        uint2 t0;
        t0.x = s0 == 0 ? te[0].x : s0 == 1 ? te[1].x : s0 == 2 ? te[2].x : te[3].x;
        t0.y = s0 == 0 ? te[0].y : s0 == 1 ? te[1].y : s0 == 2 ? te[2].y : te[3].y;
        int cnt = 0;
#pragma unroll
        for (int s = 0; s < 4; ++s) { const bool same = ((todo >> s) & 1u) && key[s] == k0; cnt += same; todo &= same ? ~(1u << s) : ~0u; }
        const uint4 qt = tile_quad(t0, xub, zub);
        float col[3];
        quad_filter3(qt, ax, az, lit, col);
#pragma unroll
        for (int k = 0; k < 3; ++k) acc[k] += (float)cnt * col[k];
      }
      const float o[3] = {0.25f * acc[0], 0.25f * acc[1], 0.25f * acc[2]};
      if (have) store_rgb(R.frames, npix, e, pix, pack_rgb(o));
    }
    __builtin_amdgcn_fence(__ATOMIC_RELEASE, "wavefront");
    __builtin_amdgcn_wave_barrier();
  }
}


#ifndef DT_Q_WAVES
#define DT_Q_WAVES 5
#endif
#ifndef DT_Q_PRIO
#define DT_Q_PRIO 3
#endif
template <bool OBJ, bool S256, bool LIGHT = false, bool SUB = false>
__global__ __launch_bounds__(RB) __attribute__((amdgpu_waves_per_eu(OBJ ? DT_Q_WAVES - 1 : DT_Q_WAVES, OBJ ? DT_Q_WAVES - 1 : DT_Q_WAVES))) void k_raster_q(RenderParams R, const EnvCam* __restrict__ cams, const EnvFast* __restrict__ fasts,
                                                 const EnvQ* __restrict__ envq, uint8_t* __restrict__ frames,
                                                 const uint8_t* __restrict__ qtex, const float4* __restrict__ lut, const PixTab* __restrict__ pixtab, const SampTab* __restrict__ samptab,
                                                 const uint32_t* __restrict__ qtiles, uint16_t* __restrict__ queue,
                                                 int32_t* __restrict__ qcount, const EnvL* __restrict__ envl) {
  extern __shared__ uint32_t s_mem[];
  uint32_t* s_qt = s_mem;
  const int tid = threadIdx.x;
  const int npix = R.W * R.H;
  const int tiles_x = (R.W + DT_TILE_W - 1) / DT_TILE_W, n_tiles = tiles_x * ((R.H + DT_TILE_H - 1) / DT_TILE_H);
  const RasterWg wg = raster_wg<SUB, false>(R, n_tiles, blockIdx.x);
  if (!wg.live) return;
  const int tile = wg.tile, rwg = wg.rwg(n_tiles), e0 = wg.e0(), e1 = wg.e1();
  for (int i = tid; i < R.n_qtiles * 2; i += RB) s_qt[i] = qtiles[i];
  __syncthreads();

  const int wave = tid >> 6, lane = tid & 63;
  const int tile_x0 = (tile % tiles_x) * DT_TILE_W;
  const int wave_y0 = (tile / tiles_x) * DT_TILE_H + wave * (WAVE_PIX / WAVE_W);
  const int LS = R.qlog2;
  const uint32_t SM = (1u << LS) - 1u;
  const float lo = 0.5f * (float)(1 << LS);

  float lr[PPT], lf[PPT], lit[PPT];
  uint32_t Mi[PPT];
  bool cand[PPT], gok[PPT], valid[PPT];
  uint32_t spxy[PPT];
  bool any_cand = false;
#pragma unroll
  for (int k = 0; k < PPT; ++k) {
    PixTab t{0.f, 0.f, -1.f, 0xFFFFu};
    const bool inimg = tile_x0 + SLOT_X(k, lane) < R.W && wave_y0 + SLOT_Y(k, lane) < R.H;
    const int pix = (wave_y0 + SLOT_Y(k, lane)) * R.W + tile_x0 + SLOT_X(k, lane);
    if (inimg) t = pixtab[pix];
    lr[k] = t.lr; lf[k] = t.lf; lit[k] = fmaxf(t.lit, 0.f); Mi[k] = t.mi;
    valid[k] = t.lit >= 0.f; cand[k] = t.lit > 0.f; gok[k] = (t.mi & 0xFFFFu) != 0xFFFFu;
    any_cand |= cand[k];
    spxy[k] = 0u;
    if (OBJ && inimg) spxy[k] = spxy_pack(lut[pix], R.W, R.H);
  }

  uint16_t* w_queue = queue + ((size_t)rwg * (RB / 64) + wave) * QREGION;
  int qn = 0, qo = 0;
  int qend_v = 0;
  uint32_t* s_px = s_mem + R.n_qtiles * 2 + wave * WAVE_PIX;
  const int st_x = tile_x0 + (lane * 4) % WAVE_W, st_y = wave_y0 + (lane * 4) / WAVE_W;
  const bool st_ok = lane * 4 < WAVE_PIX && st_x < R.W && st_y < R.H;
  const size_t st_off = ((size_t)st_y * R.W + st_x) * 3;

  ChunkObjMasks<OBJ> objmasks;
  objmasks.load(R, e0, e1, n_tiles * 4, tile * 4 + __builtin_amdgcn_readfirstlane(wave), lane);
  auto push_obj = [&](const int e, const uint32_t env, unsigned long long om, bool oedge[PPT]) __attribute__((always_inline)) {
// ... 557 lines not shown
          for (int k = 0; k < 3; ++k) pe[vb][k] += t * (pe[vf][k] - pe[vb][k]);
          w0 = -pe[0][2]; w1 = -pe[1][2];
        }
        if (ok) {
#pragma unroll
          for (int v = 0; v < 2; ++v) {
            float ndl;
            if (c.L[3] == 0.f) ndl = c.cth * c.L[1] + c.sth * c.L[2];
            else {
              const float lx = c.L[0] - pe[v][0], ly = c.L[1] - pe[v][1], lz = c.L[2] - pe[v][2];
              ndl = (c.cth * ly + c.sth * lz) * rsqrtf(lx * lx + ly * ly + lz * lz);
            }
            lit[v] = fmaxf(ndl, 0.f);
          }
          const float ndl = 0.5f * (lit[0] + lit[1]);
          sg.ax = (pe[0][0] / w0 / c.tx + 1.f) * 0.5f * (float)R.W; sg.ay = (1.f - pe[0][1] / w0 / c.ty) * 0.5f * (float)R.H;
          sg.bx = (pe[1][0] / w1 / c.tx + 1.f) * 0.5f * (float)R.W; sg.by = (1.f - pe[1][1] / w1 / c.ty) * 0.5f * (float)R.H;
          const float dx = sg.bx - sg.ax, dy = sg.by - sg.ay, l2 = dx * dx + dy * dy;
          sg.inv_len2 = l2 > 1e-12f ? 1.f / l2 : -1.f;
          sg.r = 255.f * fminf(L[6] * (c.base[0] + c.dif[0] * ndl), 1.f);
          sg.g = 255.f * fminf(L[7] * (c.base[1] + c.dif[1] * ndl), 1.f);
          sg.b = 255.f * fminf(L[8] * (c.base[2] + c.dif[2] * ndl), 1.f);
        }
      }
      s_seg[tid] = sg;
    }
    __syncthreads();
    if (!live) continue;
    const int n = min(256, count - base);
    for (int i = 0; i < n; ++i) {
      const OvSeg sg = s_seg[i];
      if (sg.inv_len2 < 0.f) continue;
      if (sxp < fminf(sg.ax, sg.bx) - 1.f || sxp > fmaxf(sg.ax, sg.bx) + 1.f || syp < fminf(sg.ay, sg.by) - 1.f || syp > fmaxf(sg.ay, sg.by) + 1.f) continue;
      const float dx = sg.bx - sg.ax, dy = sg.by - sg.ay;
#pragma unroll
      for (int q = 0; q < 4; ++q) {
        const float qx = sxp + ox[q] - sg.ax, qy = syp + oy[q] - sg.ay;
        const float u = (qx * dx + qy * dy) * sg.inv_len2;
        const float cr = qx * dy - qy * dx;
        const bool in = u >= 0.f && u <= 1.f && cr * cr * sg.inv_len2 <= 0.25f;
        if (in && !((covered >> q) & 1u)) { covered |= 1u << q; acc[0] += sg.r; acc[1] += sg.g; acc[2] += sg.b; }
      }
    }
  }
  if (live && covered) {
    const float nf = (float)(4 - __popc(covered));
    uint8_t* dst = R.frames + ((size_t)env * R.W * R.H + pix) * 3;
#pragma unroll
    for (int k = 0; k < 3; ++k) dst[k] = (uint8_t)(fminf(fmaxf(0.25f * (nf * (float)dst[k] + acc[k]), 0.f), 255.f) + 0.5f);
  }
}


struct LedS { float ex, ey, ez, r, cr, cg, cb, a, bx0, bx1, by0, by1; };
__global__ __launch_bounds__(256) void k_overlay_leds(RenderParams R, const EnvCam* __restrict__ cams, const float* __restrict__ spheres,
                                                      const int first, const int count, const int env) {
  __shared__ LedS s_led[64];
  const int tid = threadIdx.x;
  const int pix = blockIdx.x * 256 + tid;
  const EnvCam c = cams[env];
  const MapU m = map_u(R.maps[c.map_id]);
  const TileLds* tiles = reinterpret_cast<const TileLds*>(R.tile_recs);
  float nx = 0.f, ny = 0.f, sxp = 0.f, syp = 0.f;
  bool live = false;
  if (pix < R.W * R.H) {
    const float4 l = reinterpret_cast<const float4*>(R.lut)[pix];
    live = l.z != 0.f;
    nx = l.x; ny = l.y;
    sxp = (l.x + 1.f) * 0.5f * (float)R.W; syp = (1.f - l.y) * 0.5f * (float)R.H;
  }
  const float ox[4] = {-0.125f, 0.375f, -0.375f, 0.125f};
  const float oy[4] = {0.375f, 0.125f, -0.125f, -0.375f};
  const float sxn = 2.f / (float)R.W, syn = 2.f / (float)R.H;
  float add[3] = {0.f, 0.f, 0.f};
  float depth[4] = {0.f, 0.f, 0.f, 0.f};
  bool have_depth = false, any = false;
  for (int base = 0; base < count; base += 64) {
    __syncthreads();
    if (tid < 64) {
      LedS sp; sp.r = -1.f; sp.ex = sp.ey = sp.ez = sp.cr = sp.cg = sp.cb = sp.a = 0.f; sp.bx0 = sp.by0 = 1.f; sp.bx1 = sp.by1 = 0.f;
      if (base + tid < count) {
        const float* S = spheres + (size_t)(first + base + tid) * 8;
        const float rx = S[0] - c.Cx, ry = S[1] - c.Cy, rz = S[2] - c.Cz;
        const float xla = rx * c.sa + rz * c.ca, zla = -(rx * c.ca - rz * c.sa);
        sp.ex = xla; sp.ey = ry * c.cth - zla * c.sth; sp.ez = ry * c.sth + zla * c.cth;
        const float w = -sp.ez, r = S[3];
        if (r > 0.f && w + r > NEAR_Z) {
          sp.r = r; sp.cr = S[4]; sp.cg = S[5]; sp.cb = S[6]; sp.a = S[7];
          const float wn = fmaxf(w - r, NEAR_Z);
          const float cx = (sp.ex / w / c.tx + 1.f) * 0.5f * (float)R.W, cy = (1.f - sp.ey / w / c.ty) * 0.5f * (float)R.H;
          const float rad = r / wn / fminf(c.tx / (float)R.W, c.ty / (float)R.H) * 0.5f * 1.5f + 2.f;
          sp.bx0 = cx - rad; sp.bx1 = cx + rad; sp.by0 = cy - rad; sp.by1 = cy + rad;
          if (!(w > 0.f)) { sp.bx0 = sp.by0 = -1e30f; sp.bx1 = sp.by1 = 1e30f; }
        }
      }
      s_led[tid] = sp;
    }
    __syncthreads();
    if (!live) continue;
    const int n = min(64, count - base);
    for (int i = 0; i < n; ++i) {
      const LedS sp = s_led[i];
      if (!(sp.r > 0.f) || sxp < sp.bx0 || sxp > sp.bx1 || syp < sp.by0 || syp > sp.by1) continue;
      if (!have_depth) {
        have_depth = true;
        float wbest[4] = {0.f, 0.f, 0.f, 0.f};
        int tbest[4] = {-1, -1, -1, -1};
        if (R.stris && R.objbox) {
          const ObjBox* boxes = R.objbox + (size_t)env * DTSIM_MAX_OBJECTS;
          const ScreenTri* tb = R.stris + (size_t)env * R.max_tris;
          const int n_obj = R.maps[c.map_id].n_obj;
          for (int o = 0; o < n_obj; ++o) {
            const ObjBox ob = boxes[o];
            if (ob.count <= 0 || sxp < ob.bx0 - 1.f || sxp > ob.bx1 + 1.f || syp < ob.by0 - 1.f || syp > ob.by1 + 1.f) continue;
            for (int t = ob.first; t < ob.first + ob.count; ++t) test_tri(tb[t], sxp, syp, wbest, tbest);
          }
        }
#pragma unroll
        for (int q = 0; q < 4; ++q) {
          const Ray rs = make_ray(nx + ox[q] * sxn, ny - oy[q] * syn, c.tx, c.ty, c.sth, c.cth);
          const Hit h = classify(c, m, tiles, rs);
          float d = h.cls == CLS_SKY ? 3.0e38f : h.t;
          if (tbest[q] >= 0) d = fminf(d, 1.f / wbest[q]);
          depth[q] = d;
        }
      }
#pragma unroll
      for (int q = 0; q < 4; ++q) {
        const float dx = (nx + ox[q] * sxn) * c.tx, dy = (ny - oy[q] * syn) * c.ty;
        const float a = dx * dx + dy * dy + 1.f;
        const float b = dx * sp.ex + dy * sp.ey - sp.ez;
        const float cc = sp.ex * sp.ex + sp.ey * sp.ey + sp.ez * sp.ez - sp.r * sp.r;
        const float disc = b * b - a * cc;
        if (!(disc > 0.f)) continue;
        const float t = (b - sqrtf(disc)) / a;
        if (!(t >= NEAR_Z && t <= FAR_Z && t < depth[q])) continue;
        const float px = t * dx, py = t * dy, pz = -t;
        const float inv_r = 1.f / sp.r;
        const float nxe = (px - sp.ex) * inv_r, nye = (py - sp.ey) * inv_r, nze = (pz - sp.ez) * inv_r;
        float ndl;
        if (c.L[3] == 0.f) ndl = nxe * c.L[0] + nye * c.L[1] + nze * c.L[2];
        else {
          const float lx = c.L[0] - px, ly = c.L[1] - py, lz = c.L[2] - pz;
          ndl = (nxe * lx + nye * ly + nze * lz) * rsqrtf(lx * lx + ly * ly + lz * lz);
        }
        ndl = fmaxf(ndl, 0.f);
        add[0] += sp.a * 255.f * fminf(sp.cr * (c.base[0] + c.dif[0] * ndl), 1.f);
        add[1] += sp.a * 255.f * fminf(sp.cg * (c.base[1] + c.dif[1] * ndl), 1.f);
        add[2] += sp.a * 255.f * fminf(sp.cb * (c.base[2] + c.dif[2] * ndl), 1.f);
        depth[q] = t;
        any = true;
      }
    }
  }
  if (live && any) {
    uint8_t* dst = R.frames + ((size_t)env * R.W * R.H + pix) * 3;
#pragma unroll
    for (int k = 0; k < 3; ++k) dst[k] = (uint8_t)(fminf(fmaxf((float)dst[k] + 0.25f * add[k], 0.f), 255.f) + 0.5f);
  }
}

}

void dt_launch_overlay_leds(hipStream_t s, const RenderParams& R, const float* d_spheres, int first, int count, int env) {
  if (count <= 0) return;
  hipLaunchKernelGGL(k_overlay_leds, dim3((unsigned)((R.W * R.H + 255) / 256)), dim3(256), 0, s, R, reinterpret_cast<const EnvCam*>(R.envcam), d_spheres, first, count, env);
}

void dt_launch_overlay_lines(hipStream_t s, const RenderParams& R, const float* d_lines, int first, int count, int env) {
  if (count <= 0) return;
  hipLaunchKernelGGL(k_overlay_lines, dim3((unsigned)((R.W * R.H + 255) / 256)), dim3(256), 0, s, R, reinterpret_cast<const EnvCam*>(R.envcam), d_lines, first, count, env);
}

template <class K> static size_t resident_blocks(K kernel, size_t lds) {
  static std::mutex mu;
  static std::map<std::tuple<int, size_t, const void*>, size_t> cache;
  int dev = 0;
  (void)hipGetDevice(&dev);
  std::lock_guard<std::mutex> lk(mu);
  const auto key = std::make_tuple(dev, lds, reinterpret_cast<const void*>(kernel));
  auto it = cache.find(key);
  if (it != cache.end()) return it->second;
  int per_cu = 0, n_cu = 0;
  if (hipOccupancyMaxActiveBlocksPerMultiprocessor(&per_cu, kernel, RB, lds) != hipSuccess || per_cu < 1) per_cu = 3;
  if (hipDeviceGetAttribute(&n_cu, hipDeviceAttributeMultiprocessorCount, dev) != hipSuccess || n_cu < 1) n_cu = 256;
  return cache[key] = (size_t)per_cu * (size_t)n_cu;
}

#define DT_SCRATCH_ALIGN 64
static_assert(DT_SCRATCH_ALIGN % 64 == 0 && DT_SCRATCH_ALIGN % alignof(EnvD) == 0 && DT_SCRATCH_ALIGN % alignof(float4) == 0,
              "EnvQ, EnvV and EnvD records are 64-byte aligned (one scalar load each), tribox 16-byte aligned (float4)");
struct Slab {
  char* base; size_t bytes = 0;
  template <class T> T* take(size_t n) {
    const size_t off = (bytes + DT_SCRATCH_ALIGN - 1) / DT_SCRATCH_ALIGN * DT_SCRATCH_ALIGN;
    bytes = off + n * sizeof(T); return base ? reinterpret_cast<T*>(base + off) : nullptr;
  }
};
struct EnvRecs { EnvCam* cams; EnvFast* fasts; EnvQ* envq; EnvV* envv; EnvD* envd; EnvL* envl; PixTab* pixtab; SampTab* samptab; };
static EnvRecs render_layout(int N, int W, int H, int max_tris, size_t* bytes, void* const* base, RenderParams& R) {
  const size_t n = (size_t)N, n_pix = (size_t)W * H, n_tiles = dt_raster_tiles(W, H), n_wg = dt_raster_groups(N, W, H);
  Slab sl[DT_SLABS];
  for (int i = 0; i < DT_SLABS; ++i) sl[i].base = base ? static_cast<char*>(base[i]) : nullptr;
  Slab &env = sl[DT_SLAB_ENV], &pix = sl[DT_SLAB_PIX], &qc = sl[DT_SLAB_QCOUNT], &it = sl[DT_SLAB_ITEMS], &ob = sl[DT_SLAB_OBJMASK];
  EnvRecs x;
  R.envcam = x.cams = env.take<EnvCam>(n); x.fasts = env.take<EnvFast>(n); x.envq = env.take<EnvQ>(n); R.envpos = env.take<int32_t>(n);
  R.envv = x.envv = env.take<EnvV>(n + 1); R.envd = x.envd = env.take<EnvD>(n); x.envl = env.take<EnvL>(n + 1);
  R.pixtab = x.pixtab = pix.take<PixTab>(n_pix); x.samptab = pix.take<SampTab>(n_pix); R.dump = pix.take<RenderDump>(1);
  R.queue = sl[DT_SLAB_QUEUE].take<uint16_t>(n_wg * (RB / 64) * QREGION);
  R.qcount = qc.take<int32_t>(n_wg * (RB / 64)); R.work = qc.take<int32_t>(DT_WORK_INTS);
  R.items = it.take<uint32_t>(n_wg * ITEMS_PER_WG); R.items2 = it.take<uint32_t>(n_wg * ENVS_PER_BLOCK);
  R.qend = sl[DT_SLAB_QEND].take<uint16_t>(n_wg * (RB / 64) * ENVS_PER_BLOCK);
  if (max_tris > 0) {
    R.stris = sl[DT_SLAB_STRIS].take<ScreenTri>(n * max_tris); R.tribox = sl[DT_SLAB_STRIS].take<float4>(n * max_tris);
    R.objbox = sl[DT_SLAB_OBJBOX].take<ObjBox>(n * DTSIM_MAX_OBJECTS);
    R.blockbox = reinterpret_cast<float*>(ob.take<float4>(n_tiles * 4)); R.objrange = ob.take<uint2>((size_t)DTSIM_MAX_MAPS * DTSIM_MAX_OBJECTS);
    R.objmask = ob.take<unsigned long long>(n * n_tiles * 4);
  }
  if (bytes) for (int i = 0; i < DT_SLABS; ++i) bytes[i] = sl[i].bytes;
  return x;
}
void dt_render_layout(int N, int W, int H, int max_tris, size_t* bytes, void* const* base, RenderParams* R) { RenderParams tmp{}; render_layout(N, W, H, max_tris, bytes, base, R ? *R : tmp); }

int dt_raster_pipe(RenderParams& R, int grid_rows, int grid_cols, bool raster_old) {
  const bool v3 = R.qlog2 == 8 && grid_rows <= V3_MAX_ROWS && grid_cols <= V3_MAP_COLS && R.n_maps * V3_MAP_COLS <= V3_TAB_PITCH / 2 && !raster_old;
  R.q3_rows = v3 ? grid_rows : 0;
  const bool records = R.qtex && !R.segment && (R.W & 3) == 0;
  if (records && !R.domain_rand && (size_t)R.n_qtiles * 8 <= 32768 && !(R.qlog2 == 8 && R.qmax_tiles >= 256)) return v3 ? DTSIM_PIPE_V3 : DTSIM_PIPE_Q;
  if (records && R.domain_rand && v3) return DTSIM_PIPE_V3DR;
  return (R.domain_rand || R.segment || R.light) ? DTSIM_PIPE_GENERIC_ENV : DTSIM_PIPE_GENERIC;
}

template <bool SUB>
static void launch_raster_resolve(hipStream_t s, const RenderParams& R, const EnvRecs& x, int pipe, bool has_pos) {
  const bool obj = R.max_tris > 0, quad = pipe == DTSIM_PIPE_V3 || pipe == DTSIM_PIPE_Q;
  const int n_chunks = (R.N + ENVS_PER_BLOCK - 1) / ENVS_PER_BLOCK;
  const size_t lds = (size_t)R.n_tile_recs * sizeof(TileLds);
  const size_t lds1 = lds + (size_t)RB * PPT * sizeof(uint32_t);
  const size_t lds2 = lds + (size_t)(RB / 64) * ENVS_PER_BLOCK * sizeof(EnvCam);
  const dim3 grid((unsigned)(dt_raster_tiles(R.W, R.H) * n_chunks));
  const dim3 gridq((unsigned)raster_wg_grid(dt_raster_tiles(R.W, R.H), n_chunks));
  const size_t ldsq = (size_t)R.n_qtiles * 8 + (size_t)RB * PPT * sizeof(uint32_t);
  const size_t lds_tab = (size_t)R.q3_rows * V3_TAB_PITCH * 4;
  const size_t lds3 = lds_tab + (size_t)(RB / 64) * V3_WAVE_LDS * 4 + (size_t)ENVS_PER_BLOCK * sizeof(EnvQ);
  const size_t ldsd = lds_tab + (size_t)(RB / 64) * RQ_LIST * 4;
  const bool s256 = R.qlog2 == 8 && R.qmax_tiles < 256;
#define LAUNCH_RASTER(DR_, OBJ_)                                                                              \
  hipLaunchKernelGGL((k_raster<DR_, OBJ_>), grid, dim3(RB), lds1, s, R, x.cams, x.fasts, R.frames, R.texels,                  \
                     reinterpret_cast<const float4*>(R.lut), R.maps, R.tile_recs, R.queue, R.qcount)
#define LAUNCH_Q(OBJ_, S256_) do { if (R.light) hipLaunchKernelGGL((k_raster_q<OBJ_, S256_, true, SUB>), gridq, dim3(RB), ldsq, s, R, x.cams, x.fasts, x.envq, R.frames, \
                                           R.qtex, reinterpret_cast<const float4*>(R.lut), x.pixtab, x.samptab, R.qtiles, R.queue, R.qcount, x.envl); \
                                else hipLaunchKernelGGL((k_raster_q<OBJ_, S256_, false, SUB>), gridq, dim3(RB), ldsq, s, R, x.cams, x.fasts, x.envq, R.frames, R.qtex, \
                                           reinterpret_cast<const float4*>(R.lut), x.pixtab, x.samptab, R.qtiles, R.queue, R.qcount, nullptr); } while (0)
#define LAUNCH_V3(OBJ_) do { if (R.light) hipLaunchKernelGGL((k_raster_v3<OBJ_, true, SUB>), gridq, dim3(RB), lds3, s, R, x.cams, x.fasts, x.envq, x.envv, R.frames, \
                                           R.qtex, reinterpret_cast<const float4*>(R.lut), x.pixtab, x.samptab, R.qtiles, R.queue, R.qcount, x.envl); \
                                else hipLaunchKernelGGL((k_raster_v3<OBJ_, false, SUB>), gridq, dim3(RB), lds3, s, R, x.cams, x.fasts, x.envq, x.envv, R.frames, R.qtex, \
                                           reinterpret_cast<const float4*>(R.lut), x.pixtab, x.samptab, R.qtiles, R.queue, R.qcount, nullptr); } while (0)
  switch (pipe) {
    case DTSIM_PIPE_V3: if (obj) LAUNCH_V3(true); else LAUNCH_V3(false); break;
    case DTSIM_PIPE_Q: if (obj) { if (s256) LAUNCH_Q(true, true); else LAUNCH_Q(true, false); } else if (s256) LAUNCH_Q(false, true); else LAUNCH_Q(false, false); break;
    case DTSIM_PIPE_V3DR:
      if (obj) hipLaunchKernelGGL((k_raster_v3dr<true, SUB>), gridq, dim3(RB), ldsd, s, R, x.cams, x.envd, R.frames, R.qtex, reinterpret_cast<const float4*>(R.lut), R.qtiles, R.queue, R.qcount);
      else hipLaunchKernelGGL((k_raster_v3dr<false, SUB>), gridq, dim3(RB), ldsd, s, R, x.cams, x.envd, R.frames, R.qtex, reinterpret_cast<const float4*>(R.lut), R.qtiles, R.queue, R.qcount);
      break;
    case DTSIM_PIPE_GENERIC_ENV: if (obj) LAUNCH_RASTER(true, true); else LAUNCH_RASTER(true, false); break;
    default: if (obj) LAUNCH_RASTER(false, true); else LAUNCH_RASTER(false, false);
  }
#undef LAUNCH_V3
#undef LAUNCH_Q
#undef LAUNCH_RASTER
  if (pipe == DTSIM_PIPE_V3DR) {
    const dim3 rgrid((unsigned)std::min<size_t>(grid.x, resident_blocks(k_resolve_dr, lds_tab)));
    hipLaunchKernelGGL(k_resolve_dr, rgrid, dim3(RB), lds_tab, s, R, x.cams, x.envd, R.qtex, reinterpret_cast<const float4*>(R.lut), R.qtiles, R.queue, R.qcount);
  } else if (!quad) {
    const dim3 rgrid((unsigned)std::min<size_t>(grid.x, resident_blocks(k_resolve, lds2)));
    hipLaunchKernelGGL(k_resolve, rgrid, dim3(RB), lds2, s, R, x.cams, R.queue, R.qcount);
  }
  if (obj) {
    const size_t lds4 = lds + (size_t)(RB / 64) * TRI_CAP * sizeof(TriCov) + (size_t)(RB / 64) * RO_SCR_BYTES;
    const dim3 rgrid((unsigned)std::min<size_t>(grid.x, resident_blocks(k_resolve_obj<DT_RES_NB>, lds4)));
    hipLaunchKernelGGL(k_resolve_obj<DT_RES_NB>, rgrid, dim3(RB), lds4, s, R, x.cams, R.queue, 1, has_pos ? x.envq : (const EnvQ*)nullptr);
  }
}

int dt_launch_render(hipStream_t s, const SimArrays& A, const RenderParams& R_in, int pipe, int tables, const uint8_t* mask) {
  RenderParams R = R_in;
  tables &= 3;
  void* base[DT_SLABS] = {R.envcam, R.pixtab}; RenderParams carved{};
  const EnvRecs x = render_layout(A.N, R.W, R.H, 0, nullptr, base, carved);
  const bool quad = pipe == DTSIM_PIPE_V3 || pipe == DTSIM_PIPE_Q, v3dr = pipe == DTSIM_PIPE_V3DR;
  int32_t* pos = ((quad || v3dr) && R.envpos && A.N > ENVS_PER_BLOCK) ? R.envpos : nullptr;
  const bool sub = mask && (quad || v3dr) && R.envpos;
  if (sub) {
    pos = R.envpos;
    (void)hipMemsetAsync(R.work, 0, DT_WORK_INTS * sizeof(int32_t), s);
    hipLaunchKernelGGL(k_env_sort<true>, dim3(1), dim3(1024), 0, s, A, R.maps, pos, mask, R.work + DT_WORK_LIVE);
    tables |= 4;
  } else if (pos) { hipLaunchKernelGGL(k_env_sort<false>, dim3(1), dim3(1024), 0, s, A, R.maps, pos, nullptr, nullptr); tables |= 4; }
#define LAUNCH_CAM(M_) hipLaunchKernelGGL(k_cam_setup<M_>, dim3((A.N + 63) / 64), dim3(64), 0, s, A, R.domain_rand, R.segment,                  \
                     (float)R.W / (float)R.H, x.cams, x.fasts, R.maps, (quad || v3dr) ? x.envq : nullptr, R.qlog2, pos, quad ? x.envv : nullptr,  \
                     v3dr ? x.envd : nullptr, R.W, R.H, R.light, (quad && R.light) ? x.envl : nullptr)
  if (sub) LAUNCH_CAM(true); else LAUNCH_CAM(false);
#undef LAUNCH_CAM
  if (!sub) (void)hipMemsetAsync(R.work, 0, DT_WORK_INTS * sizeof(int32_t), s);
  if (R.max_tris > 0) {
    if (!(tables & 2)) hipLaunchKernelGGL(k_blk_setup, dim3((unsigned)dt_raster_tiles(R.W, R.H)), dim3(RB), 0, s, R, reinterpret_cast<const float4*>(R.lut), reinterpret_cast<float4*>(R.blockbox));
    tables |= 2;
    if (sub) hipLaunchKernelGGL(k_obj_setup<true>, dim3(A.N), dim3(DT_OBJSETUP_T), 0, s, A, R, x.cams, pos);
    else hipLaunchKernelGGL(k_obj_setup<false>, dim3(A.N), dim3(DT_OBJSETUP_T), 0, s, A, R, x.cams, pos);
  }

  if (quad && !(tables & 1)) {
    hipLaunchKernelGGL(k_pix_setup, dim3((R.W * R.H + 255) / 256), dim3(256), 0, s, R, reinterpret_cast<const float4*>(R.lut), x.pixtab, x.samptab);
    tables |= 1;
  }
  if (sub) launch_raster_resolve<true>(s, R, x, pipe, true);
  else launch_raster_resolve<false>(s, R, x, pipe, pos != nullptr);
  return tables;
}
```

gym-duckietown_amd/csrc/render_v3.inc:

```

#ifndef DT_V3_WAVES
#define DT_V3_WAVES 6
#endif
#ifndef DT_V3_WAVES_OBJ
#define DT_V3_WAVES_OBJ (DT_V3_WAVES - 1)
#endif
#define DT_V3_SW (DT_V3_WW / 4)
#define V3_ROWS (WAVE_PIX / DT_V3_WW)
#define V3_WX (DT_TILE_W / DT_V3_WW)
static_assert(PPT == 4 && DT_V3_WW == 128 && DT_V3_WW == WAVE_W && DT_TILE_W % DT_V3_WW == 0 && (RB / 64) % V3_WX == 0 &&
              V3_ROWS * ((RB / 64) / V3_WX) == DT_TILE_H, "k_raster_v3 / k_raster_v3dr: 128 x 2 wavefront blocks tiling the 128 x 8 workgroup tile "
              "(the generic k_resolve / k_resolve_obj decode the queue entries as row-major pixel numbers of such a block)");
#define V3_MAX_ROWS 24
#define V3_SEL_TILE 0x0c0c0602u
#define V3_WAVE_LDS RQ_LIST
static_assert(DT_V3_WW == 4 * DT_V3_SW && 64 % DT_V3_SW == 0, "four slots side by side");
#define V3_PIX(k, l) (((l) / DT_V3_SW) * DT_V3_WW + (k) * DT_V3_SW + ((l) % DT_V3_SW))
#define V3_XP_LANE(l) (((l) / DT_V3_SW) * DT_V3_WW + ((l) % DT_V3_SW))
#define V3_XO1 "96"
#define V3_XO1G "97"
#define V3_XO1B "98"
#define V3_XO2 "192"
#define V3_XO2G "193"
#define V3_XO2B "194"
#define V3_XO3 "288"
#define V3_XO3G "289"
#define V3_XO3B "290"
#define V3_ROW16 (DT_V3_WW * 3 / 16)

struct U4 { uint32_t a, b, c, d; };
#define V3_XPOSE_WAIT " s_waitcnt lgkmcnt(0)"

struct C3 { uint32_t rb, g; };
__device__ inline C3 c3_of_rgb(const uint32_t rgb) { return C3{rgb, rgb}; }

struct GndK { float Cx, Cz, sa, ca, kg, gnd[3], base[3], dif[3], gndl[4], pad[2]; };

template <bool LIGHT>
__device__ inline void resolve_region_v3(const RenderParams& R, const EnvCam* __restrict__ cams, const SampTab* __restrict__ samptab,
                                         const uint8_t* __restrict__ qtex, const uint32_t* s_qt, const uint16_t* w_queue, const int n,
                                         const int e0, const int bx0, const int by0, const int lane, const uint4* s_envq,
                                         const EnvL* __restrict__ envl) {
  const int npix = R.W * R.H;
  const float Sf = (float)(1 << R.qlog2), lo = 0.5f * Sf;
  const char* qtb = reinterpret_cast<const char*>(s_qt);
  for (int r0 = 0; r0 < n; r0 += RQ_LIST) {
    const int n_list = min(n - r0, RQ_LIST);
    for (int l0 = 0; l0 < n_list; l0 += 64) {
      const bool have = l0 + lane < n_list;
      const uint32_t ent = have ? (uint32_t)__builtin_nontemporal_load(w_queue + r0 + l0 + lane) : 0u;
      const int lp = (int)(ent & 255u);
      const int el = (int)((ent >> 8) & 63u);
      const int pix = have ? (by0 + lp / DT_V3_WW) * R.W + bx0 + lp % DT_V3_WW : 0;
      const SampTab sp = samptab[pix];
      PixTab pt;
      pt.lr = __uint_as_float(sp.pad[0]); pt.lf = __uint_as_float(sp.pad[1]); pt.lit = __uint_as_float(sp.pad[2]); pt.mi = 0u;
      const uint4* fl = s_envq + el * 4;
      const uint4 a4 = fl[0];
      const float4 qa = make_float4(__uint_as_float(a4.x), __uint_as_float(a4.y), __uint_as_float(a4.z), __uint_as_float(a4.w));
      const uint4 qb = fl[1], qd = fl[3];
      const float A = qa.x, B = qa.y, Cx = qa.z, Cz = qa.w, Xhi = __uint_as_float(qb.x), Zhi = __uint_as_float(qb.y);
      const uint32_t tab = qd.z;
      const int e = (int)qd.y;
      const float4* c4 = reinterpret_cast<const float4*>(cams + e);
      const float wCy = default_cam((float)R.W / (float)R.H).Cy;
      const float kg = (wCy - GROUND_Y) / wCy;
      const float qpm = __uint_as_float(qd.w);
      const float goff = (float)DT_QRING * Sf + 0.5f, ghalf = GROUND_HALF * qpm;
      const float Xu = fmaf(pt.lf, B, fmaf(pt.lr, A, Cx)), Zu = fmaf(pt.lf, -A, fmaf(pt.lr, B, Cz));
      const uint32_t xic = q8_bits(Xu), zic = q8_bits(Zu);
      float lit8 = (pt.lit > 0.f ? pt.lit : 0.55f) * Q8_LIT;
      if constexpr (LIGHT) { if (pt.lit > 0.f) lit8 = env_lit8(envl[min(e0 + el, R.N - 1)], pt.lr, pt.lf, env_base8()); }
      const uint32_t W8 = quad_weights8(q8_frac(xic), q8_frac(zic), lit8);
      uint32_t aS[3] = {0u, 0u, 0u};
      int n_sky = 0, n_gnd = 0;
      float gX = 0.f, gZ = 0.f;
      uint4 rec = make_uint4(0u, 0u, 0u, 0u);
      uint32_t raddr_prev = 0u;
#pragma unroll
      for (int s = 3; s >= 0; --s) {
        const uint32_t hr = sp.dlr[s >> 1], hf = sp.dlf[s >> 1];
        const float slr = pt.lr + __half2float(__ushort_as_half((unsigned short)((s & 1) ? hr >> 16 : hr)));
        const float slf = pt.lf + __half2float(__ushort_as_half((unsigned short)((s & 1) ? hf >> 16 : hf)));
        const float Xs = fmaf(slf, B, fmaf(slr, A, Cx)), Zs = fmaf(slf, -A, fmaf(slr, B, Cz));
        const float Xo = Xs - 0.5f, Zo = Zs - 0.5f;
        const float Xc = med3f(Xo, lo, Xhi), Zc = med3f(Zo, lo, Zhi);
        const bool s_in = (Xc == Xo) & (Zc == Zo);
        const uint32_t ta = (__builtin_amdgcn_perm((uint32_t)flr_i32(Zc), (uint32_t)flr_i32(Xc), 0x0c0c0501u) << 2) + tab;
        const uint32_t* tp = reinterpret_cast<const uint32_t*>(qtb + ta);
        const uint32_t tb = tp[0], sel = tp[128];
        const bool is_tile = have & (((sp.flags >> s) & 1u) != 0u) & s_in & (tb != 0u);
        const float Xg = fmaf(kg, Xs - Cx, Cx), Zg = fmaf(kg, Zs - Cz, Cz);
        const bool is_gnd = have & !is_tile & (((sp.flags >> (4 + s)) & 1u) != 0u) & (fabsf(Xg - goff) <= ghalf) & (fabsf(Zg - goff) <= ghalf);
        n_gnd += is_gnd; n_sky += !(is_tile | is_gnd);
        if (is_gnd) { gX = Xg; gZ = Zg; }
        const uint32_t raddr = is_tile ? (tb | q8_rec256(xic, zic, sel)) : 0u;
        if (s == 3 || raddr != raddr_prev) rec = *reinterpret_cast<const uint4*>(qtex + raddr);
        raddr_prev = raddr;
        aS[0] = __builtin_amdgcn_udot4(rec.x, W8, aS[0], false);
        aS[1] = __builtin_amdgcn_udot4(rec.y, W8, aS[1], false);
        aS[2] = __builtin_amdgcn_udot4(rec.z, W8, aS[2], false);
      }
      float acc[3];
      float4 hc = make_float4(0.f, 0.f, 0.f, 0.f);
      if (__ballot(n_sky > 0)) hc = c4[2];
      acc[0] = fmaf((float)n_sky, hc.y, (float)aS[0] * (1.f / 256.f));
      acc[1] = fmaf((float)n_sky, hc.z, (float)aS[1] * (1.f / 256.f));
      acc[2] = fmaf((float)n_sky, hc.w, (float)aS[2] * (1.f / 256.f));
      if (__ballot(n_gnd > 0)) {
        if (pt.lit > 0.f && (pt.lr != 0.f || pt.lf != 0.f)) { gX = fmaf(kg, Xu - Cx, Cx); gZ = fmaf(kg, Zu - Cz, Cz); }
        const float hs = 0.5f / ghalf;
        const float a_ = fminf(fmaxf(fmaf(gX - goff, hs, 0.5f), 0.f), 1.f), b_ = fminf(fmaxf(fmaf(gZ - goff, hs, 0.5f), 0.f), 1.f);
        const float4 q3 = c4[3], q4 = c4[4], q5 = c4[5], q6 = c4[6], q7 = c4[7];
        const float n0 = q6.y + a_ * (q6.z - q6.y), n1 = q6.w + a_ * (q7.x - q6.w);
        const float ndl = n0 + b_ * (n1 - n0);
        const float ng = (float)n_gnd;
        acc[0] += ng * (q3.x * fminf(q3.w + q4.z * ndl, 1.f));
        acc[1] += ng * (q3.y * fminf(q4.x + q4.w * ndl, 1.f));
        acc[2] += ng * (q3.z * fminf(q4.y + q5.x * ndl, 1.f));
      }
      const float o[3] = {0.25f * acc[0], 0.25f * acc[1], 0.25f * acc[2]};
      if (have) store_rgb(R.frames, npix, e, pix, pack_rgb(o));
    }
    __builtin_amdgcn_fence(__ATOMIC_RELEASE, "wavefront");
    __builtin_amdgcn_wave_barrier();
  }
}

template <bool OBJ, bool LIGHT = false, bool SUB = false>
__global__ __launch_bounds__(RB) __attribute__((amdgpu_waves_per_eu(OBJ ? DT_V3_WAVES_OBJ : DT_V3_WAVES, OBJ ? DT_V3_WAVES_OBJ : DT_V3_WAVES)))
void k_raster_v3(RenderParams R, const EnvCam* __restrict__ cams, const EnvFast* __restrict__ fasts, const EnvQ* __restrict__ envq,
                 const EnvV* __restrict__ envv, uint8_t* __restrict__ frames, const uint8_t* __restrict__ qtex, const float4* __restrict__ lut,
                 const PixTab* __restrict__ pixtab, const SampTab* __restrict__ samptab, const uint32_t* __restrict__ qtiles,
                 uint16_t* __restrict__ queue, int32_t* __restrict__ qcount, const EnvL* __restrict__ envl) {
  extern __shared__ uint32_t s_mem[];
  uint32_t* s_qt = s_mem;
  const int tid = threadIdx.x;
  const int npix = R.W * R.H;
  const int tiles_x = (R.W + DT_TILE_W - 1) / DT_TILE_W, n_tiles = tiles_x * ((R.H + DT_TILE_H - 1) / DT_TILE_H);
  const RasterWg wg = raster_wg<SUB, true>(R, n_tiles, blockIdx.x);
  if (!wg.live) return;
  const int NL = wg.NL, tile = wg.tile, rwg = wg.rwg(n_tiles), e0 = wg.e0(), e1 = wg.e1();
  v3_fill_tile_table(R, qtiles, s_qt, tid);
  uint4* s_envq = reinterpret_cast<uint4*>(s_mem + R.q3_rows * V3_TAB_PITCH + (RB / 64) * V3_WAVE_LDS);
  static_assert(ENVS_PER_BLOCK * 4 <= RB, "one 16-byte piece per thread");
  if (tid < ENVS_PER_BLOCK * 4) s_envq[tid] = reinterpret_cast<const uint4*>(envq + min(e0 + tid / 4, NL - 1))[tid & 3];
  __syncthreads();

  const int wave = __builtin_amdgcn_readfirstlane(tid >> 6), lane = tid & 63;
  const int bx0 = (tile % tiles_x) * DT_TILE_W + (wave % V3_WX) * DT_V3_WW;
  const int by0 = (tile / tiles_x) * DT_TILE_H + (wave / V3_WX) * V3_ROWS;
  const float lo = 0.5f * 256.f;

  float lr[PPT], lf[PPT], lit[PPT];
  uint32_t Mi[PPT];
  bool cand[PPT], gok[PPT], valid[PPT];
  uint32_t spxy[PPT];
#pragma unroll
  for (int k = 0; k < PPT; ++k) {
    PixTab t{0.f, 0.f, -1.f, 0xFFFFu};
    const int x = bx0 + V3_PIX(k, lane) % DT_V3_WW, y = by0 + V3_PIX(k, lane) / DT_V3_WW;
    const bool inimg = x < R.W && y < R.H;
    if (inimg) t = pixtab[y * R.W + x];
    lr[k] = t.lr; lf[k] = t.lf; lit[k] = fmaxf(t.lit, 0.f) * Q8_LIT; Mi[k] = t.mi;
    valid[k] = t.lit >= 0.f; cand[k] = t.lit > 0.f; gok[k] = (t.mi & 0xFFFFu) != 0xFFFFu;
    spxy[k] = 0u;
    if (OBJ && inimg) spxy[k] = spxy_pack(lut[y * R.W + x], R.W, R.H);
  }
  bool any_cand = false;
#pragma unroll
  for (int k = 0; k < PPT; ++k) any_cand |= cand[k];

  uint16_t* w_queue = queue + ((size_t)rwg * (RB / 64) + wave) * QREGION;
  int qn = 0, qo = 0;
  int qend_v = 0;
  uint32_t* w_lds = s_mem + R.q3_rows * V3_TAB_PITCH + wave * V3_WAVE_LDS;
  const int st_x = bx0 + (lane * 4) % DT_V3_WW, st_y = by0 + (lane * 4) / DT_V3_WW;
  const bool st_ok = st_x < R.W && st_y < R.H;
  const size_t st_off = ((size_t)st_y * R.W + st_x) * 3;

  ChunkObjMasks<OBJ> objmasks;
  objmasks.load(R, e0, e1, n_tiles * 4, tile * 4 + wave, lane);
  auto push_obj = [&](const int e, const uint32_t env, unsigned long long om, unsigned long long oem[PPT], const unsigned long long em[PPT]) __attribute__((always_inline)) {
    const ObjBox* boxes = R.objbox + (size_t)env * DTSIM_MAX_OBJECTS;
    bool oedge[PPT];
#pragma unroll
    for (int k = 0; k < PPT; ++k) oedge[k] = false;
    const float obj_mrg = (R.W > 2048 || R.H > 2048) ? 0.95f : (R.W > 1024 || R.H > 1024) ? 0.45f : 0.3f;
    float sx[PPT], sy[PPT];
#pragma unroll
    for (int k = 0; k < PPT; ++k) spxy_unpack(spxy[k], sx[k], sy[k]);
    while (om) {
      const int o = __builtin_ctzll(om);
      const ObjBox ob = boxes[o];
      om &= om - 1ull;
#pragma unroll
      for (int k = 0; k < PPT; ++k)
        if (valid[k] && sx[k] >= ob.bx0 - obj_mrg && sx[k] <= ob.bx1 + obj_mrg && sy[k] >= ob.by0 - obj_mrg && sy[k] <= ob.by1 + obj_mrg) oedge[k] = true;
    }
    bool any_oedge = false;
#pragma unroll
    for (int k = 0; k < PPT; ++k) any_oedge |= oedge[k];
    if (__ballot(any_oedge)) {
      const uint32_t etag = (uint32_t)(e - e0) << 8;
#pragma unroll
      for (int k = 0; k < PPT; ++k) {
        const bool ek = oedge[k];
        const unsigned long long mk = __ballot(ek);
        oem[k] = mk;
        if (ek) {
          const int rank = __builtin_amdgcn_mbcnt_hi((uint32_t)(mk >> 32), __builtin_amdgcn_mbcnt_lo((uint32_t)mk, 0u));
          w_queue[QREGION - 1 - (qo + rank)] = (uint16_t)(etag | (__builtin_amdgcn_inverse_ballot_w64(em[k]) ? QE_PLANE_EDGE : 0u) | (uint32_t)V3_PIX(k, lane));
        }
        qo += __popcll(mk);
      }
    }
  };
  const uint32_t st_voff = st_ok ? (uint32_t)st_off : 0x80000000u;
  const uint32_t frame_bytes = (uint32_t)npix * 3u;
  const bool wide = __builtin_amdgcn_readfirstlane((int)(R.W % DT_V3_WW == 0 && R.H % V3_ROWS == 0)) != 0;
  const uint32_t st_voff16 = lane < 48 ? (uint32_t)(((size_t)(by0 + lane / V3_ROW16) * R.W + bx0) * 3u) + (uint32_t)(lane % V3_ROW16) * 16u : 0x80000000u;
  auto store = [&](const uint32_t env, const U4& o) __attribute__((always_inline)) {
    const v3_i32x4 fr = v3_rsrc(frames + (size_t)env * frame_bytes, frame_bytes);
    if (wide) v3_buf_store_v4i32(v3_u32x4{o.a, o.b, o.c, o.d}, fr, (int)st_voff16, 0, 2);
    else v3_buf_store_v3i32(v3_u32x3{o.a, o.b, o.c}, fr, (int)st_voff, 0, 2);
  };
  const uint32_t xp_wr = static_cast<uint32_t>(reinterpret_cast<uintptr_t>(w_lds)) + (uint32_t)V3_XP_LANE(lane) * 3u;
  const uint32_t xp_rd = static_cast<uint32_t>(reinterpret_cast<uintptr_t>(w_lds)) + (wide ? (uint32_t)(lane % 48) * 16u : (uint32_t)lane * 12u);
  auto transpose = [&](const C3 c[PPT]) __attribute__((always_inline)) -> U4 {
    U4 out;
    out.d = 0u;
    uint2 rd01, rd23;
    const uint32_t g01 = __builtin_amdgcn_perm(c[1].g, c[0].g, 0x0c050c01u), g23 = __builtin_amdgcn_perm(c[3].g, c[2].g, 0x0c050c01u);
    asm volatile(
        "ds_write_b8 %3, %4\n ds_write_b8 %3, %5 offset:1\n ds_write_b8_d16_hi %3, %4 offset:2\n"
        "ds_write_b8 %3, %6 offset:" V3_XO1 "\n ds_write_b8_d16_hi %3, %5 offset:" V3_XO1G "\n ds_write_b8_d16_hi %3, %6 offset:" V3_XO1B "\n"
        "ds_write_b8 %3, %7 offset:" V3_XO2 "\n ds_write_b8 %3, %8 offset:" V3_XO2G "\n ds_write_b8_d16_hi %3, %7 offset:" V3_XO2B "\n"
        "ds_write_b8 %3, %9 offset:" V3_XO3 "\n ds_write_b8_d16_hi %3, %8 offset:" V3_XO3G "\n ds_write_b8_d16_hi %3, %9 offset:" V3_XO3B "\n"
        "ds_read2_b32 %0, %10 offset1:1\n ds_read2_b32 %1, %10 offset0:2 offset1:3\n" V3_XPOSE_WAIT
        : "=&v"(rd01), "=&v"(rd23)
        : "v"(xp_wr), "v"(xp_wr), "v"(c[0].rb), "v"(g01), "v"(c[1].rb), "v"(c[2].rb), "v"(g23), "v"(c[3].rb), "v"(xp_rd)
        : "memory");
    out.a = rd01.x; out.b = rd01.y; out.c = rd23.x; out.d = rd23.y;
    return out;
  };

  const bool wave_sky = !__ballot(any_cand);
  if (wave_sky) {
    C3 vm[PPT];
#pragma unroll
    for (int k = 0; k < PPT; ++k) vm[k] = c3_of_rgb(valid[k] ? 0x00FFFFFFu : 0u);
    U4 m = transpose(vm);
    asm volatile("s_waitcnt lgkmcnt(0)" : "+v"(m.a), "+v"(m.b), "+v"(m.c), "+v"(m.d));
    uint32_t hsel[4];
    {
      const uint32_t ph = wide ? (uint32_t)((lane % V3_ROW16) % 3) : 0u;
#pragma unroll
      for (int i = 0; i < 4; ++i) {
        uint32_t v = 0u;
#pragma unroll
        for (int j = 0; j < 4; ++j) v |= ((ph + 4u * i + j) % 3u) << (8 * j);
        hsel[i] = v;
      }
    }
    for (int e = e0; e < e1; ++e) {
      const EnvV f = envv[e];
      const unsigned long long om = objmasks.of(e);
      const uint32_t s0 = __builtin_amdgcn_perm(f.hor_rgb, f.hor_rgb, hsel[0]), s1 = __builtin_amdgcn_perm(f.hor_rgb, f.hor_rgb, hsel[1]),
                     s2 = __builtin_amdgcn_perm(f.hor_rgb, f.hor_rgb, hsel[2]), s3 = __builtin_amdgcn_perm(f.hor_rgb, f.hor_rgb, hsel[3]);
      if (OBJ && om) {
        unsigned long long oem[PPT] = {0ull, 0ull, 0ull, 0ull};
        const unsigned long long noe[PPT] = {0ull, 0ull, 0ull, 0ull};
        push_obj(e, f.env, om, oem, noe);
      }
      store(f.env, U4{s0 & m.a, s1 & m.b, s2 & m.c, s3 & m.d});
      if (OBJ) qend_v = lane >= e - e0 ? qo : qend_v;
    }
    if (lane == 0) qcount[rwg * (RB / 64) + wave] = OBJ ? qo : 0;
  } else {
    typedef float f2 __attribute__((ext_vector_type(2)));
    f2 lr2[PPT / 2], lf2[PPT / 2], lit2[PPT / 2];
#pragma unroll
    for (int j = 0; j < PPT / 2; ++j) {
      lr2[j] = f2{lr[2 * j], lr[2 * j + 1]}; lf2[j] = f2{lf[2 * j], lf[2 * j + 1]}; lit2[j] = f2{lit[2 * j], lit[2 * j + 1]};
    }
    const char* s_qtb = reinterpret_cast<const char*>(s_qt);
    unsigned long long candm[PPT], validm[PPT], plainm[PPT];
#pragma unroll
    for (int k = 0; k < PPT; ++k) { candm[k] = __ballot(cand[k]); validm[k] = __ballot(valid[k]); plainm[k] = __ballot(gok[k]); }
    bool mixed = false;
#pragma unroll
    for (int k = 0; k < PPT; ++k) mixed |= candm[k] != ~0ull;
    uint32_t blk_reach;
    {
      float r2 = 0.f;
#pragma unroll
      for (int k = 0; k < PPT; ++k) r2 = fmaxf(r2, lr[k] * lr[k] + lf[k] * lf[k]);
#pragma unroll
      for (int d = 32; d > 0; d >>= 1) r2 = fmaxf(r2, __shfl_xor(r2, d));
      const float r = fsqrt_(r2) * R.q_per_m * 1.0001f + 1.f;
      blk_reach = (uint32_t)__builtin_amdgcn_readfirstlane((int)(r < 1.0e9f ? (uint32_t)r : 0x7FFFFFFFu));
    }
    typedef uint4 Rec;
    struct QStage { Rec q[PPT]; f2 ax2[PPT / 2], az2[PPT / 2]; };
    auto issue_t = [&](const EnvV& f, QStage& st, auto clamp_tag) __attribute__((always_inline)) {
      constexpr bool CLAMP = decltype(clamp_tag)::value;
      const f2 vA = f2{f.A2[0], f.A2[1]}, vB = f2{f.B2[0], f.B2[1]}, vCx = f2{f.Cx2[0], f.Cx2[1]}, vCz = f2{f.Cz2[0], f.Cz2[1]};
      const f2 vK = f2{Q8_SNAP, Q8_SNAP};
#pragma unroll
      for (int j = 0; j < PPT / 2; ++j) {
        const f2 X2 = fma2(lf2[j], vB, fma2(lr2[j], vA, vCx)) + vK;
        const f2 Z2 = fma2(lf2[j], -vA, fma2(lr2[j], vB, vCz)) + vK;
#pragma unroll
        for (int h = 0; h < 2; ++h) {
          const int k = 2 * j + h;
          float X = h ? X2.y : X2.x, Z = h ? Z2.y : Z2.x;
          if (CLAMP) { X = med3f(X, lo + Q8_SNAP, f.Xhi + Q8_SNAP); Z = med3f(Z, lo + Q8_SNAP, f.Zhi + Q8_SNAP); }
          const uint32_t xi = __float_as_uint(X), zi = __float_as_uint(Z);
          if (h) { st.ax2[j].y = (float)(xi & 255u); st.az2[j].y = (float)(zi & 255u); }
          else { st.ax2[j].x = (float)(xi & 255u); st.az2[j].x = (float)(zi & 255u); }
          const uint32_t ta = (__builtin_amdgcn_perm(zi, xi, V3_SEL_TILE) << 2) + f.tab3;
          const uint32_t* tp = reinterpret_cast<const uint32_t*>(s_qtb + ta);
          const uint32_t tb = tp[0], sel = tp[V3_TAB_PITCH / 2];
          const uint32_t cell = q8_rec256(xi, zi, sel);
          st.q[k] = *reinterpret_cast<const uint4*>(qtex + (tb | cell));
        }
      }
    };
    auto issue = [&](const EnvV& f, QStage& st) __attribute__((always_inline)) {
#if DT_Q_PRIO
      __builtin_amdgcn_s_setprio(DT_Q_PRIO);
#endif
      if (f.reach > blk_reach) issue_t(f, st, std::false_type{});
      else issue_t(f, st, std::true_type{});
#if DT_Q_PRIO
      __builtin_amdgcn_s_setprio(0);
#endif
    };
    auto ground_rgb = [&](const GndK& c, const float lrk, const float lfk) __attribute__((always_inline)) -> uint32_t {
      const float wx = c.Cx + lrk * c.sa + lfk * c.ca, wz = c.Cz + lrk * c.ca - lfk * c.sa;
      const float wxg = fmaf(c.kg, wx - c.Cx, c.Cx), wzg = fmaf(c.kg, wz - c.Cz, c.Cz);
      const float a = fminf(fmaxf((wxg + GROUND_HALF) * (0.5f / GROUND_HALF), 0.f), 1.f);
      const float b = fminf(fmaxf((wzg + GROUND_HALF) * (0.5f / GROUND_HALF), 0.f), 1.f);
      const float n0 = c.gndl[0] + a * (c.gndl[1] - c.gndl[0]), n1 = c.gndl[2] + a * (c.gndl[3] - c.gndl[2]);
      const float ndl = n0 + b * (n1 - n0);
      uint32_t rgb = 0;
      rgb = __builtin_amdgcn_cvt_pk_u8_f32(c.gnd[0] * fminf(c.base[0] + c.dif[0] * ndl, 1.f), 0, rgb);
      rgb = __builtin_amdgcn_cvt_pk_u8_f32(c.gnd[1] * fminf(c.base[1] + c.dif[1] * ndl, 1.f), 1, rgb);
      rgb = __builtin_amdgcn_cvt_pk_u8_f32(c.gnd[2] * fminf(c.base[2] + c.dif[2] * ndl, 1.f), 2, rgb);
      return rgb;
    };
    auto append_edges = [&](const int e, const unsigned long long em[PPT]) __attribute__((always_inline)) {
      const uint32_t etag = (uint32_t)(e - e0) << 8;
#pragma unroll
      for (int k = 0; k < PPT; ++k) {
        const unsigned long long mk = em[k];
        if (!mk) continue;
        if (__builtin_amdgcn_inverse_ballot_w64(mk)) {
          const int rank = __builtin_amdgcn_mbcnt_hi((uint32_t)(mk >> 32), __builtin_amdgcn_mbcnt_lo((uint32_t)mk, 0u));
          w_queue[qn + rank] = (uint16_t)(etag | (uint32_t)V3_PIX(k, lane));
        }
        qn += __popcll(mk);
      }
    };
    auto finish = [&](const int e, const uint32_t env, const uint32_t hor_rgb, const QStage& st, unsigned long long om, auto mixed_tag) __attribute__((always_inline)) -> U4 {
      constexpr bool MIXED = decltype(mixed_tag)::value;
      C3 c[PPT];
      unsigned long long fastm[PPT];
      const Rec* q = st.q;
      unsigned long long slow = 0ull;
#pragma unroll
      for (int j = 0; j < PPT / 2; ++j) {
        if (j) __builtin_amdgcn_sched_barrier(0);
        f2 w00, w10, w01, w11;
        {
#pragma clang fp contract(off)
          f2 I2 = lit2[j];
          if constexpr (LIGHT) I2 = env_lit8_2(envl[e], lr2[j], lf2[j]);
          const f2 c256 = f2{256.f, 256.f};
          const f2 u = st.ax2[j] * I2, v = fma2(I2, c256, -u);
          w11 = u * st.az2[j]; w01 = v * st.az2[j];
          w10 = fma2(u, c256, -w11); w00 = fma2(v, c256, -w01);
        }
#pragma unroll
        for (int h = 0; h < 2; ++h) {
          const int k = 2 * j + h;
          const unsigned long long fm = __ballot((q[k].w & 0xFFFFu) > (Mi[k] & 0xFFFFu));
          fastm[k] = fm;
          slow |= candm[k] & ~fm;
          uint32_t W = __builtin_amdgcn_cvt_pk_u8_f32(h ? w00.y : w00.x, 0, 0u);
          W = __builtin_amdgcn_cvt_pk_u8_f32(h ? w10.y : w10.x, 1, W);
          W = __builtin_amdgcn_cvt_pk_u8_f32(h ? w01.y : w01.x, 2, W);
          W = __builtin_amdgcn_cvt_pk_u8_f32(h ? w11.y : w11.x, 3, W);
          const uint32_t vr = __builtin_amdgcn_udot4(q[k].x, W, 128u, false), vg = __builtin_amdgcn_udot4(q[k].y, W, 128u, false),
                         vb = __builtin_amdgcn_udot4(q[k].z, W, 128u, false);
          c[k].rb = __builtin_amdgcn_perm(vb, vr, 0x0c050c01u);
          c[k].g = vg;
        }
      }
      if (MIXED) {
        const C3 hc = c3_of_rgb(hor_rgb);
#pragma unroll
        for (int k = 0; k < PPT; ++k) {
          c[k].rb = cand[k] ? c[k].rb : valid[k] ? hc.rb : 0u; c[k].g = cand[k] ? c[k].g : valid[k] ? hc.g : 0u;
        }
      }
      if (!slow && !(OBJ && om)) return transpose(c);
      unsigned long long em[PPT] = {0ull, 0ull, 0ull, 0ull}, oem[PPT] = {0ull, 0ull, 0ull, 0ull};
      if (slow) {
#pragma unroll
        for (int k = 0; k < PPT; ++k) {
          const unsigned long long sk = candm[k] & ~fastm[k];
          if (!sk) continue;
          em[k] = sk;
          const unsigned long long gm = sk & __ballot((q[k].w >> 16) != 0u) & plainm[k];
          if (gm) {
            uint32_t mik = Mi[k];
            asm volatile("" : "+v"(mik));
            const float mrgk = __half2float(__ushort_as_half((unsigned short)(mik >> 16)));
            const EnvFast g = fasts[env];
            const EnvCam cc = cams[env];
            GndK K;
            K.Cx = cc.Cx; K.Cz = cc.Cz; K.sa = cc.sa; K.ca = cc.ca; K.kg = g.kg;
#pragma unroll
            for (int t = 0; t < 3; ++t) { K.gnd[t] = cc.gnd[t]; K.base[t] = cc.base[t]; K.dif[t] = cc.dif[t]; }
#pragma unroll
            for (int t = 0; t < 4; ++t) K.gndl[t] = cc.gndl[t];
            const float wx = K.Cx + lr[k] * K.sa + lf[k] * K.ca, wz = K.Cz + lr[k] * K.ca - lf[k] * K.sa;
            const float wxg = fmaf(K.kg, wx - K.Cx, K.Cx), wzg = fmaf(K.kg, wz - K.Cz, K.Cz);
            const bool clear = (wx < -mrgk) | (wx > g.gw_m + mrgk) | (wz < -mrgk) | (wz > g.gh_m + mrgk);
            const bool inq = (fabsf(wxg) + 2.f * mrgk < GROUND_HALF) & (fabsf(wzg) + 2.f * mrgk < GROUND_HALF);
            const bool gfast = __builtin_amdgcn_inverse_ballot_w64(gm) & clear & inq;
            const C3 gc = c3_of_rgb(ground_rgb(K, lr[k], lf[k]));
            c[k].rb = gfast ? gc.rb : c[k].rb; c[k].g = gfast ? gc.g : c[k].g;
            em[k] = sk & ~__ballot(gfast);
          }
        }
      }
      if (OBJ && om) {
        push_obj(e, env, om, oem, em);
#pragma unroll
        for (int k = 0; k < PPT; ++k) em[k] &= ~oem[k];
      }
      const U4 out = transpose(c);
      append_edges(e, em);
      return out;
    };
    auto run = [&](auto mixed_tag) __attribute__((always_inline)) {
      QStage sa;
      const EnvV* fp = envv + e0;
      EnvV f = fp[0];
      issue(f, sa);
      uint32_t hor = f.hor_rgb, env = f.env, env_prev;
      f = fp[1]; ++fp;
      U4 held = finish(e0, env, hor, sa, objmasks.of(e0), mixed_tag);
      if (OBJ) qend_v = qo;
      for (int e = e0 + 1; e < e1; ++e) {
        env_prev = env; hor = f.hor_rgb; env = f.env;
        issue(f, sa);
        store(env_prev, held);
        f = fp[1]; ++fp;
        held = finish(e, env, hor, sa, objmasks.of(e), mixed_tag);
        if (OBJ) qend_v = lane >= e - e0 ? qo : qend_v;
      }
      store(env, held);
    };
    if (mixed) run(std::true_type{}); else run(std::false_type{});
    if (lane == 0) qcount[rwg * (RB / 64) + wave] = OBJ ? qo : qn;
    if (qn > 0) {
      __builtin_amdgcn_s_waitcnt(0);
      resolve_region_v3<LIGHT>(R, cams, samptab, qtex, s_qt, w_queue, qn, e0, bx0, by0, lane, s_envq, envl);
    }
  }
  if (OBJ) {
    if (lane < ENVS_PER_BLOCK) R.qend[((size_t)rwg * (RB / 64) + wave) * ENVS_PER_BLOCK + lane] = (uint16_t)qend_v;
    __shared__ envmask_t s_og[RB / 64], s_oh[RB / 64];
    envmask_t oh = 0ull;
    const envmask_t og = obj_groups_of(qend_v, lane, &oh);
    if (lane == 0) { s_og[wave] = og; s_oh[wave] = oh; }
    __syncthreads();
    if (tid == 0) {
      envmask_t g = 0ull, gh = 0ull;
#pragma unroll
      for (int r = 0; r < RB / 64; ++r) { g |= s_og[r]; gh |= s_oh[r]; }
      if (g) push_obj_items(R, (uint32_t)rwg, g, gh);
    }
  }
}
```

Measured before the change: 2.751 million.

## Resolve far-field raster waves inline instead of queueing edge pixels

Adds a 'far' wave path in the v3 raster kernel. When no candidate pixel in a wave is near (below half a texel in minification), every pixel is computed directly with the exact 4-sample filter, processed in two halves, and nothing is appended to the edge queue. The exact-resolve code and the ground-fast path are moved into shared helpers, and the per-pixel plain flag and margin bits are packed into SampTab. The work-counter memset is also skipped for quad pipelines with no triangles. This aims to remove queue traffic and the second resolve pass, at the cost of doing exact filtering on pixels that did not need it and a larger kernel with higher register pressure. The old behaviour can be forced with DTSIM_FAR_QUEUE=1.

```diff
diff --git a/gym-duckietown_amd/csrc/dtsim_api.hip b/gym-duckietown_amd/csrc/dtsim_api.hip
--- a/gym-duckietown_amd/csrc/dtsim_api.hip
+++ b/gym-duckietown_amd/csrc/dtsim_api.hip
@@ -149,6 +149,7 @@
   DevPtr<uint32_t> d_texels_seg;
   DevPtr<uint8_t> d_mesh_seg;
   DevPtr<char> d_render[DT_SLABS];
+  bool far_queue = false;
   bool raster_old = false;
   int step_lanes = 1;
   DevPtr<dtsim_reset_sampler> d_sampler;
@@ -291,6 +292,7 @@
   HIPCHK(hipSetDevice(cfg->device));
   dtsim* h = new dtsim();
   { const char* ro = getenv("DTSIM_RASTER_OLD"); h->raster_old = ro && ro[0] == '1'; }
+  { const char* fq = getenv("DTSIM_FAR_QUEUE"); h->far_queue = fq && fq[0] == '1'; }
   h->step_lanes = cfg->num_envs * 4 <= 32768 ? 4 : cfg->num_envs * 2 <= 32768 ? 2 : 1;
   h->cfg = *cfg;
   h->N = cfg->num_envs;
@@ -639,6 +641,7 @@
   render_scene(h, segment, &R);
   render_scratch(h, R.max_tris, &R);
   R.light = ((h->cfg.flags & DTSIM_F_LIGHT_CAPTURE) && !R.domain_rand) ? 1 : 0;
+  R.far_queue = h->far_queue ? 1 : 0;
   if (flags & DTSIM_RENDER_GL_FILTER) R.qtex = nullptr;
   const int pipe = dt_raster_pipe(R, h->maps.grid_rows, h->maps.grid_cols, h->raster_old);
   {
diff --git a/gym-duckietown_amd/csrc/dtsim_dev.h b/gym-duckietown_amd/csrc/dtsim_dev.h
--- a/gym-duckietown_amd/csrc/dtsim_dev.h
+++ b/gym-duckietown_amd/csrc/dtsim_dev.h
@@ -136,6 +136,7 @@
   void* envd;
   int32_t q3_rows;
   int32_t light;
+  int32_t far_queue;
 };
 #define DT_WORK_INTS 8
 #define DT_WORK_LIVE 7
diff --git a/gym-duckietown_amd/csrc/render.hip b/gym-duckietown_amd/csrc/render.hip
--- a/gym-duckietown_amd/csrc/render.hip
+++ b/gym-duckietown_amd/csrc/render.hip
@@ -1356,6 +1356,7 @@
 
 struct alignas(16) PixTab { float lr, lf, lit; uint32_t mi; };
 struct alignas(16) SampTab { uint32_t dlr[2], dlf[2]; uint32_t flags; uint32_t pad[3]; };
+#define SAMP_PLAIN 0x100u
 static_assert(sizeof(PixTab) == 16 && sizeof(SampTab) == 32, "table records");
 
 __global__ void k_pix_setup(RenderParams R, const float4* __restrict__ lut, PixTab* __restrict__ pixtab, SampTab* __restrict__ samptab) {
@@ -1398,6 +1399,7 @@
     sp.dlr[j] = (uint32_t)__half_as_ushort(__float2half_rn(dlr[2 * j])) | ((uint32_t)__half_as_ushort(__float2half_rn(dlr[2 * j + 1])) << 16);
     sp.dlf[j] = (uint32_t)__half_as_ushort(__float2half_rn(dlf[2 * j])) | ((uint32_t)__half_as_ushort(__float2half_rn(dlf[2 * j + 1])) << 16);
   }
+  sp.flags |= (plain ? SAMP_PLAIN : 0u) | (t.mi & 0xFFFF0000u);
   sp.pad[0] = __float_as_uint(t.lr); sp.pad[1] = __float_as_uint(t.lf); sp.pad[2] = __float_as_uint(t.lit);
   samptab[pix] = sp;
 }
@@ -2561,7 +2563,7 @@
                      v3dr ? x.envd : nullptr, R.W, R.H, R.light, (quad && R.light) ? x.envl : nullptr)
   if (sub) LAUNCH_CAM(true); else LAUNCH_CAM(false);
 #undef LAUNCH_CAM
-  if (!sub) (void)hipMemsetAsync(R.work, 0, DT_WORK_INTS * sizeof(int32_t), s);
+  if (!sub && !(quad && R.max_tris == 0)) (void)hipMemsetAsync(R.work, 0, DT_WORK_INTS * sizeof(int32_t), s);
   if (R.max_tris > 0) {
     if (!(tables & 2)) hipLaunchKernelGGL(k_blk_setup, dim3((unsigned)dt_raster_tiles(R.W, R.H)), dim3(RB), 0, s, R, reinterpret_cast<const float4*>(R.lut), reinterpret_cast<float4*>(R.blockbox));
     tables |= 2;
diff --git a/gym-duckietown_amd/csrc/render_v3.inc b/gym-duckietown_amd/csrc/render_v3.inc
--- a/gym-duckietown_amd/csrc/render_v3.inc
+++ b/gym-duckietown_amd/csrc/render_v3.inc
@@ -37,12 +37,80 @@
 struct GndK { float Cx, Cz, sa, ca, kg, gnd[3], base[3], dif[3], gndl[4], pad[2]; };
 
 template <bool LIGHT>
+__device__ inline uint32_t exact_rgb_v3(const RenderParams& R, const bool have, const SampTab& sp, const uint4 a4, const uint4 qb, const uint4 qd,
+                                        const float4* c4, const EnvL* el, const uint8_t* __restrict__ qtex, const char* qtb) {
+  const float Sf = (float)(1 << R.qlog2), lo = 0.5f * Sf;
+  PixTab pt;
+  pt.lr = __uint_as_float(sp.pad[0]); pt.lf = __uint_as_float(sp.pad[1]); pt.lit = __uint_as_float(sp.pad[2]); pt.mi = 0u;
+  const float4 qa = make_float4(__uint_as_float(a4.x), __uint_as_float(a4.y), __uint_as_float(a4.z), __uint_as_float(a4.w));
+  const float A = qa.x, B = qa.y, Cx = qa.z, Cz = qa.w, Xhi = __uint_as_float(qb.x), Zhi = __uint_as_float(qb.y);
+  const uint32_t tab = qd.z;
+  const float wCy = default_cam((float)R.W / (float)R.H).Cy;
+  const float kg = (wCy - GROUND_Y) / wCy;
+  const float qpm = __uint_as_float(qd.w);
+  const float goff = (float)DT_QRING * Sf + 0.5f, ghalf = GROUND_HALF * qpm;
+  const float Xu = fmaf(pt.lf, B, fmaf(pt.lr, A, Cx)), Zu = fmaf(pt.lf, -A, fmaf(pt.lr, B, Cz));
+  const uint32_t xic = q8_bits(Xu), zic = q8_bits(Zu);
+  float lit8 = (pt.lit > 0.f ? pt.lit : 0.55f) * Q8_LIT;
+  if constexpr (LIGHT) { if (pt.lit > 0.f) lit8 = env_lit8(*el, pt.lr, pt.lf, env_base8()); }
+  const uint32_t W8 = quad_weights8(q8_frac(xic), q8_frac(zic), lit8);
+  uint32_t aS[3] = {0u, 0u, 0u};
+  int n_sky = 0, n_gnd = 0;
+  float gX = 0.f, gZ = 0.f;
+  uint4 rec = make_uint4(0u, 0u, 0u, 0u);
+  uint32_t raddr_prev = 0u;
+#pragma unroll
+  for (int s = 3; s >= 0; --s) {
+    const uint32_t hr = sp.dlr[s >> 1], hf = sp.dlf[s >> 1];
+    const float slr = pt.lr + __half2float(__ushort_as_half((unsigned short)((s & 1) ? hr >> 16 : hr)));
+    const float slf = pt.lf + __half2float(__ushort_as_half((unsigned short)((s & 1) ? hf >> 16 : hf)));
+    const float Xs = fmaf(slf, B, fmaf(slr, A, Cx)), Zs = fmaf(slf, -A, fmaf(slr, B, Cz));
+    const float Xo = Xs - 0.5f, Zo = Zs - 0.5f;
+    const float Xc = med3f(Xo, lo, Xhi), Zc = med3f(Zo, lo, Zhi);
+    const bool s_in = (Xc == Xo) & (Zc == Zo);
+    const uint32_t ta = (__builtin_amdgcn_perm((uint32_t)flr_i32(Zc), (uint32_t)flr_i32(Xc), 0x0c0c0501u) << 2) + tab;
+    const uint32_t* tp = reinterpret_cast<const uint32_t*>(qtb + ta);
+    const uint32_t tb = tp[0], sel = tp[128];
+    const bool is_tile = have & (((sp.flags >> s) & 1u) != 0u) & s_in & (tb != 0u);
+    const float Xg = fmaf(kg, Xs - Cx, Cx), Zg = fmaf(kg, Zs - Cz, Cz);
+    const bool is_gnd = have & !is_tile & (((sp.flags >> (4 + s)) & 1u) != 0u) & (fabsf(Xg - goff) <= ghalf) & (fabsf(Zg - goff) <= ghalf);
+    n_gnd += is_gnd; n_sky += !(is_tile | is_gnd);
+    if (is_gnd) { gX = Xg; gZ = Zg; }
+    const uint32_t raddr = is_tile ? (tb | q8_rec256(xic, zic, sel)) : 0u;
+    if (s == 3 || raddr != raddr_prev) rec = *reinterpret_cast<const uint4*>(qtex + raddr);
+    raddr_prev = raddr;
+    aS[0] = __builtin_amdgcn_udot4(rec.x, W8, aS[0], false);
+    aS[1] = __builtin_amdgcn_udot4(rec.y, W8, aS[1], false);
+    aS[2] = __builtin_amdgcn_udot4(rec.z, W8, aS[2], false);
+  }
+  float acc[3];
+  float4 hc = make_float4(0.f, 0.f, 0.f, 0.f);
+  if (__ballot(n_sky > 0)) hc = c4[2];
+  acc[0] = fmaf((float)n_sky, hc.y, (float)aS[0] * (1.f / 256.f));
+  acc[1] = fmaf((float)n_sky, hc.z, (float)aS[1] * (1.f / 256.f));
+  acc[2] = fmaf((float)n_sky, hc.w, (float)aS[2] * (1.f / 256.f));
+  if (__ballot(n_gnd > 0)) {
+    if (pt.lit > 0.f && (pt.lr != 0.f || pt.lf != 0.f)) { gX = fmaf(kg, Xu - Cx, Cx); gZ = fmaf(kg, Zu - Cz, Cz); }
+    const float hs = 0.5f / ghalf;
+    const float a_ = fminf(fmaxf(fmaf(gX - goff, hs, 0.5f), 0.f), 1.f), b_ = fminf(fmaxf(fmaf(gZ - goff, hs, 0.5f), 0.f), 1.f);
+    const float4 q3 = c4[3], q4 = c4[4], q5 = c4[5], q6 = c4[6], q7 = c4[7];
+    const float n0 = q6.y + a_ * (q6.z - q6.y), n1 = q6.w + a_ * (q7.x - q6.w);
+    const float ndl = n0 + b_ * (n1 - n0);
+    const float ng = (float)n_gnd;
+    acc[0] += ng * (q3.x * fminf(q3.w + q4.z * ndl, 1.f));
+    acc[1] += ng * (q3.y * fminf(q4.x + q4.w * ndl, 1.f));
+    acc[2] += ng * (q3.z * fminf(q4.y + q5.x * ndl, 1.f));
+  }
+  const float o[3] = {0.25f * acc[0], 0.25f * acc[1], 0.25f * acc[2]};
+  return pack_rgb(o);
+}
+
+template <bool LIGHT>
 __device__ inline void resolve_region_v3(const RenderParams& R, const EnvCam* __restrict__ cams, const SampTab* __restrict__ samptab,
                                          const uint8_t* __restrict__ qtex, const uint32_t* s_qt, const uint16_t* w_queue, const int n,
                                          const int e0, const int bx0, const int by0, const int lane, const uint4* s_envq,
                                          const EnvL* __restrict__ envl) {
   const int npix = R.W * R.H;
-  const float Sf = (float)(1 << R.qlog2), lo = 0.5f * Sf;
   const char* qtb = reinterpret_cast<const char*>(s_qt);
   for (int r0 = 0; r0 < n; r0 += RQ_LIST) {
     const int n_list = min(n - r0, RQ_LIST);
@@ -53,74 +121,12 @@
       const int el = (int)((ent >> 8) & 63u);
       const int pix = have ? (by0 + lp / DT_V3_WW) * R.W + bx0 + lp % DT_V3_WW : 0;
       const SampTab sp = samptab[pix];
-      PixTab pt;
-      pt.lr = __uint_as_float(sp.pad[0]); pt.lf = __uint_as_float(sp.pad[1]); pt.lit = __uint_as_float(sp.pad[2]); pt.mi = 0u;
       const uint4* fl = s_envq + el * 4;
       const uint4 a4 = fl[0];
-      const float4 qa = make_float4(__uint_as_float(a4.x), __uint_as_float(a4.y), __uint_as_float(a4.z), __uint_as_float(a4.w));
       const uint4 qb = fl[1], qd = fl[3];
-      const float A = qa.x, B = qa.y, Cx = qa.z, Cz = qa.w, Xhi = __uint_as_float(qb.x), Zhi = __uint_as_float(qb.y);
-      const uint32_t tab = qd.z;
       const int e = (int)qd.y;
-      const float4* c4 = reinterpret_cast<const float4*>(cams + e);
-      const float wCy = default_cam((float)R.W / (float)R.H).Cy;
-      const float kg = (wCy - GROUND_Y) / wCy;
-      const float qpm = __uint_as_float(qd.w);
-      const float goff = (float)DT_QRING * Sf + 0.5f, ghalf = GROUND_HALF * qpm;
-      const float Xu = fmaf(pt.lf, B, fmaf(pt.lr, A, Cx)), Zu = fmaf(pt.lf, -A, fmaf(pt.lr, B, Cz));
-      const uint32_t xic = q8_bits(Xu), zic = q8_bits(Zu);
-      float lit8 = (pt.lit > 0.f ? pt.lit : 0.55f) * Q8_LIT;
-      if constexpr (LIGHT) { if (pt.lit > 0.f) lit8 = env_lit8(envl[min(e0 + el, R.N - 1)], pt.lr, pt.lf, env_base8()); }
-      const uint32_t W8 = quad_weights8(q8_frac(xic), q8_frac(zic), lit8);
-      uint32_t aS[3] = {0u, 0u, 0u};
-      int n_sky = 0, n_gnd = 0;
-      float gX = 0.f, gZ = 0.f;
-      uint4 rec = make_uint4(0u, 0u, 0u, 0u);
-      uint32_t raddr_prev = 0u;
-#pragma unroll
-      for (int s = 3; s >= 0; --s) {
-        const uint32_t hr = sp.dlr[s >> 1], hf = sp.dlf[s >> 1];
-        const float slr = pt.lr + __half2float(__ushort_as_half((unsigned short)((s & 1) ? hr >> 16 : hr)));
-        const float slf = pt.lf + __half2float(__ushort_as_half((unsigned short)((s & 1) ? hf >> 16 : hf)));
-        const float Xs = fmaf(slf, B, fmaf(slr, A, Cx)), Zs = fmaf(slf, -A, fmaf(slr, B, Cz));
-        const float Xo = Xs - 0.5f, Zo = Zs - 0.5f;
-        const float Xc = med3f(Xo, lo, Xhi), Zc = med3f(Zo, lo, Zhi);
-        const bool s_in = (Xc == Xo) & (Zc == Zo);
-        const uint32_t ta = (__builtin_amdgcn_perm((uint32_t)flr_i32(Zc), (uint32_t)flr_i32(Xc), 0x0c0c0501u) << 2) + tab;
-        const uint32_t* tp = reinterpret_cast<const uint32_t*>(qtb + ta);
-        const uint32_t tb = tp[0], sel = tp[128];
-        const bool is_tile = have & (((sp.flags >> s) & 1u) != 0u) & s_in & (tb != 0u);
-        const float Xg = fmaf(kg, Xs - Cx, Cx), Zg = fmaf(kg, Zs - Cz, Cz);
-        const bool is_gnd = have & !is_tile & (((sp.flags >> (4 + s)) & 1u) != 0u) & (fabsf(Xg - goff) <= ghalf) & (fabsf(Zg - goff) <= ghalf);
-        n_gnd += is_gnd; n_sky += !(is_tile | is_gnd);
-        if (is_gnd) { gX = Xg; gZ = Zg; }
-        const uint32_t raddr = is_tile ? (tb | q8_rec256(xic, zic, sel)) : 0u;
-        if (s == 3 || raddr != raddr_prev) rec = *reinterpret_cast<const uint4*>(qtex + raddr);
-        raddr_prev = raddr;
-        aS[0] = __builtin_amdgcn_udot4(rec.x, W8, aS[0], false);
-        aS[1] = __builtin_amdgcn_udot4(rec.y, W8, aS[1], false);
-        aS[2] = __builtin_amdgcn_udot4(rec.z, W8, aS[2], false);
-      }
-      float acc[3];
-      float4 hc = make_float4(0.f, 0.f, 0.f, 0.f);
-      if (__ballot(n_sky > 0)) hc = c4[2];
-      acc[0] = fmaf((float)n_sky, hc.y, (float)aS[0] * (1.f / 256.f));
-      acc[1] = fmaf((float)n_sky, hc.z, (float)aS[1] * (1.f / 256.f));
-      acc[2] = fmaf((float)n_sky, hc.w, (float)aS[2] * (1.f / 256.f));
-      if (__ballot(n_gnd > 0)) {
-        if (pt.lit > 0.f && (pt.lr != 0.f || pt.lf != 0.f)) { gX = fmaf(kg, Xu - Cx, Cx); gZ = fmaf(kg, Zu - Cz, Cz); }
-        const float hs = 0.5f / ghalf;
-        const float a_ = fminf(fmaxf(fmaf(gX - goff, hs, 0.5f), 0.f), 1.f), b_ = fminf(fmaxf(fmaf(gZ - goff, hs, 0.5f), 0.f), 1.f);
-        const float4 q3 = c4[3], q4 = c4[4], q5 = c4[5], q6 = c4[6], q7 = c4[7];
-        const float n0 = q6.y + a_ * (q6.z - q6.y), n1 = q6.w + a_ * (q7.x - q6.w);
-        const float ndl = n0 + b_ * (n1 - n0);
-        const float ng = (float)n_gnd;
-        acc[0] += ng * (q3.x * fminf(q3.w + q4.z * ndl, 1.f));
-        acc[1] += ng * (q3.y * fminf(q4.x + q4.w * ndl, 1.f));
-        acc[2] += ng * (q3.z * fminf(q4.y + q5.x * ndl, 1.f));
-      }
-      const float o[3] = {0.25f * acc[0], 0.25f * acc[1], 0.25f * acc[2]};
-      if (have) store_rgb(R.frames, npix, e, pix, pack_rgb(o));
+      const uint32_t rgb = exact_rgb_v3<LIGHT>(R, have, sp, a4, qb, qd, reinterpret_cast<const float4*>(cams + e), LIGHT ? envl + min(e0 + el, R.N - 1) : nullptr, qtex, qtb);
+      if (have) store_rgb(R.frames, npix, e, pix, rgb);
     }
     __builtin_amdgcn_fence(__ATOMIC_RELEASE, "wavefront");
     __builtin_amdgcn_wave_barrier();
@@ -220,11 +226,14 @@
   const uint32_t frame_bytes = (uint32_t)npix * 3u;
   const bool wide = __builtin_amdgcn_readfirstlane((int)(R.W % DT_V3_WW == 0 && R.H % V3_ROWS == 0)) != 0;
   const uint32_t st_voff16 = lane < 48 ? (uint32_t)(((size_t)(by0 + lane / V3_ROW16) * R.W + bx0) * 3u) + (uint32_t)(lane % V3_ROW16) * 16u : 0x80000000u;
-  auto store = [&](const uint32_t env, const U4& o) __attribute__((always_inline)) {
+  uint32_t st_v = wide ? st_voff16 : st_voff;
+  if constexpr (!OBJ) asm volatile("" : "+v"(st_v));
+  auto store_at = [&](const uint32_t env, const U4& o, const uint32_t voff) __attribute__((always_inline)) {
     const v3_i32x4 fr = v3_rsrc(frames + (size_t)env * frame_bytes, frame_bytes);
-    if (wide) v3_buf_store_v4i32(v3_u32x4{o.a, o.b, o.c, o.d}, fr, (int)st_voff16, 0, 2);
-    else v3_buf_store_v3i32(v3_u32x3{o.a, o.b, o.c}, fr, (int)st_voff, 0, 2);
+    if (wide) v3_buf_store_v4i32(v3_u32x4{o.a, o.b, o.c, o.d}, fr, (int)voff, 0, 2);
+    else v3_buf_store_v3i32(v3_u32x3{o.a, o.b, o.c}, fr, (int)voff, 0, 2);
   };
+  auto store = [&](const uint32_t env, const U4& o) __attribute__((always_inline)) { store_at(env, o, st_v); };
   const uint32_t xp_wr = static_cast<uint32_t>(reinterpret_cast<uintptr_t>(w_lds)) + (uint32_t)V3_XP_LANE(lane) * 3u;
   const uint32_t xp_rd = static_cast<uint32_t>(reinterpret_cast<uintptr_t>(w_lds)) + (wide ? (uint32_t)(lane % 48) * 16u : (uint32_t)lane * 12u);
   auto transpose = [&](const C3 c[PPT]) __attribute__((always_inline)) -> U4 {
@@ -245,6 +254,56 @@
     return out;
   };
 
+  auto block_reach = [&](const float blr[PPT], const float blf[PPT]) __attribute__((always_inline)) -> uint32_t {
+    float r2 = 0.f;
+#pragma unroll
+    for (int k = 0; k < PPT; ++k) r2 = fmaxf(r2, blr[k] * blr[k] + blf[k] * blf[k]);
+#pragma unroll
+    for (int d = 32; d > 0; d >>= 1) r2 = fmaxf(r2, __shfl_xor(r2, d));
+    const float r = fsqrt_(r2) * R.q_per_m * 1.0001f + 1.f;
+    return (uint32_t)__builtin_amdgcn_readfirstlane((int)(r < 1.0e9f ? (uint32_t)r : 0x7FFFFFFFu));
+  };
+  auto ground_rgb = [&](const GndK& c, const float lrk, const float lfk) __attribute__((always_inline)) -> uint32_t {
+    const float wx = c.Cx + lrk * c.sa + lfk * c.ca, wz = c.Cz + lrk * c.ca - lfk * c.sa;
+    const float wxg = fmaf(c.kg, wx - c.Cx, c.Cx), wzg = fmaf(c.kg, wz - c.Cz, c.Cz);
+    const float a = fminf(fmaxf((wxg + GROUND_HALF) * (0.5f / GROUND_HALF), 0.f), 1.f);
+    const float b = fminf(fmaxf((wzg + GROUND_HALF) * (0.5f / GROUND_HALF), 0.f), 1.f);
+    const float n0 = c.gndl[0] + a * (c.gndl[1] - c.gndl[0]), n1 = c.gndl[2] + a * (c.gndl[3] - c.gndl[2]);
+    const float ndl = n0 + b * (n1 - n0);
+    uint32_t rgb = 0;
+    rgb = __builtin_amdgcn_cvt_pk_u8_f32(c.gnd[0] * fminf(c.base[0] + c.dif[0] * ndl, 1.f), 0, rgb);
+    rgb = __builtin_amdgcn_cvt_pk_u8_f32(c.gnd[1] * fminf(c.base[1] + c.dif[1] * ndl, 1.f), 1, rgb);
+    rgb = __builtin_amdgcn_cvt_pk_u8_f32(c.gnd[2] * fminf(c.base[2] + c.dif[2] * ndl, 1.f), 2, rgb);
+    return rgb;
+  };
+  auto ground_fast = [&](const float lrk, const float lfk, uint32_t mik, const uint32_t env, const unsigned long long gm, C3& ck) __attribute__((always_inline)) -> unsigned long long {
+    asm volatile("" : "+v"(mik));
+    const float mrgk = __half2float(__ushort_as_half((unsigned short)(mik >> 16)));
+    const EnvFast g = fasts[env];
+    const EnvCam cc = cams[env];
+    GndK K;
+    K.Cx = cc.Cx; K.Cz = cc.Cz; K.sa = cc.sa; K.ca = cc.ca; K.kg = g.kg;
+#pragma unroll
+    for (int t = 0; t < 3; ++t) { K.gnd[t] = cc.gnd[t]; K.base[t] = cc.base[t]; K.dif[t] = cc.dif[t]; }
+#pragma unroll
+    for (int t = 0; t < 4; ++t) K.gndl[t] = cc.gndl[t];
+    const float wx = K.Cx + lrk * K.sa + lfk * K.ca, wz = K.Cz + lrk * K.ca - lfk * K.sa;
+    const float wxg = fmaf(K.kg, wx - K.Cx, K.Cx), wzg = fmaf(K.kg, wz - K.Cz, K.Cz);
+    const bool clear = (wx < -mrgk) | (wx > g.gw_m + mrgk) | (wz < -mrgk) | (wz > g.gh_m + mrgk);
+    const bool inq = (fabsf(wxg) + 2.f * mrgk < GROUND_HALF) & (fabsf(wzg) + 2.f * mrgk < GROUND_HALF);
+    const bool gfast = __builtin_amdgcn_inverse_ballot_w64(gm) & clear & inq;
+    const C3 gc = c3_of_rgb(ground_rgb(K, lrk, lfk));
+    ck.rb = gfast ? gc.rb : ck.rb; ck.g = gfast ? gc.g : ck.g;
+    return __ballot(gfast);
+  };
+
+  bool wave_far = false;
+  if constexpr (!OBJ) {
+    bool nearp = false;
+#pragma unroll
+    for (int k = 0; k < PPT; ++k) nearp |= cand[k] && (Mi[k] & 0xFFFFu) < (1u << R.qlog2) / 2u;
+    wave_far = !R.far_queue && !__ballot(nearp);
+  }
   const bool wave_sky = !__ballot(any_cand);
   if (wave_sky) {
     C3 vm[PPT];
@@ -277,6 +336,68 @@
       if (OBJ) qend_v = lane >= e - e0 ? qo : qend_v;
     }
     if (lane == 0) qcount[rwg * (RB / 64) + wave] = OBJ ? qo : 0;
+  } else if (wave_far) {
+    int flane = lane;
+    asm volatile("" : "+v"(flane));
+    const char* s_qtb = reinterpret_cast<const char*>(s_qt);
+    auto rec_of = [&](const int k, const int l, uint4& d, uint4& h) __attribute__((always_inline)) {
+      const int x = bx0 + V3_PIX(k, l) % DT_V3_WW, y = by0 + V3_PIX(k, l) / DT_V3_WW;
+      d = make_uint4(0u, 0u, 0u, 0u); h = make_uint4(0u, 0u, 0u, __float_as_uint(-1.f));
+      if (x < R.W && y < R.H) { const uint4* sp = reinterpret_cast<const uint4*>(samptab + y * R.W + x); d = sp[0]; h = sp[1]; }
+    };
+    uint32_t blk_reach;
+    {
+      float blr[PPT], blf[PPT];
+#pragma unroll
+      for (int k = 0; k < PPT; ++k) { uint4 d, h; rec_of(k, flane, d, h); blr[k] = __uint_as_float(h.y); blf[k] = __uint_as_float(h.z); }
+      blk_reach = block_reach(blr, blf);
+    }
+    auto uni4 = [](const uint4 v) __attribute__((always_inline)) -> uint4 {
+      return make_uint4((uint32_t)__builtin_amdgcn_readfirstlane((int)v.x), (uint32_t)__builtin_amdgcn_readfirstlane((int)v.y),
+                        (uint32_t)__builtin_amdgcn_readfirstlane((int)v.z), (uint32_t)__builtin_amdgcn_readfirstlane((int)v.w));
+    };
+    auto half = [&](auto half_tag) __attribute__((always_inline)) {
+      constexpr int HALF = decltype(half_tag)::value, K0 = 2 * HALF;
+      int hlane = lane;
+      asm volatile("" : "+v"(hlane));
+      uint4 fd[2], fh[2];
+#pragma unroll
+      for (int j = 0; j < 2; ++j) rec_of(K0 + j, hlane, fd[j], fh[j]);
+      uint32_t wm = (uint32_t)-(int)wide;
+      asm volatile("" : "+v"(wm));
+      const uint32_t lane_half = (((uint32_t)(hlane % V3_ROW16) / (V3_ROW16 / 2)) & wm) | (((uint32_t)((hlane * 4) % DT_V3_WW) / (2 * DT_V3_SW)) & ~wm);
+      const uint32_t st_half = lane_half == (uint32_t)HALF ? st_v : 0x80000000u;
+      for (int e = e0; e < e1; ++e) {
+        const uint4* fl = s_envq + (e - e0) * 4;
+        const uint4 a4 = uni4(fl[0]), qb = uni4(fl[1]), qc = uni4(fl[2]), qd = uni4(fl[3]);
+        const uint32_t reach = qd.x, env = qd.y, tab3 = qd.z, hor = qc.x;
+        const float A = __uint_as_float(a4.x), B = __uint_as_float(a4.y), Cx = __uint_as_float(a4.z), Cz = __uint_as_float(a4.w);
+        const float Xhi = __uint_as_float(qb.x), Zhi = __uint_as_float(qb.y);
+        const bool noclamp = reach > blk_reach;
+        C3 c[PPT] = {{0u, 0u}, {0u, 0u}, {0u, 0u}, {0u, 0u}};
+#pragma unroll
+        for (int j = 0; j < 2; ++j) {
+          if (j) __builtin_amdgcn_sched_barrier(0);
+          SampTab sp{{fd[j].x, fd[j].y}, {fd[j].z, fd[j].w}, fh[j].x, {fh[j].y, fh[j].z, fh[j].w}};
+          asm volatile("" : "+v"(sp.dlr[0]), "+v"(sp.dlr[1]), "+v"(sp.dlf[0]), "+v"(sp.dlf[1]), "+v"(sp.flags));
+          const float lrk = __uint_as_float(fh[j].y), lfk = __uint_as_float(fh[j].z), litk = __uint_as_float(fh[j].w);
+          const bool candk = litk > 0.f, validk = litk >= 0.f;
+          const uint32_t rgb = exact_rgb_v3<LIGHT>(R, candk, sp, a4, qb, qd, reinterpret_cast<const float4*>(cams + env),
+                                                   LIGHT ? envl + min(e, R.N - 1) : nullptr, qtex, s_qtb);
+          C3& ck = c[K0 + j];
+          ck.rb = candk ? rgb : validk ? hor : 0u; ck.g = ck.rb;
+          float X = fmaf(lfk, B, fmaf(lrk, A, Cx)) + Q8_SNAP, Z = fmaf(lfk, -A, fmaf(lrk, B, Cz)) + Q8_SNAP;
+          if (!noclamp) { X = med3f(X, lo + Q8_SNAP, Xhi + Q8_SNAP); Z = med3f(Z, lo + Q8_SNAP, Zhi + Q8_SNAP); }
+          const uint32_t ta = (__builtin_amdgcn_perm(__float_as_uint(Z), __float_as_uint(X), V3_SEL_TILE) << 2) + tab3;
+          const unsigned long long gm = __ballot(candk & ((fh[j].x & SAMP_PLAIN) != 0u) & (*reinterpret_cast<const uint32_t*>(s_qtb + ta) == 0u));
+          if (gm) (void)ground_fast(lrk, lfk, fh[j].x, env, gm, ck);
+        }
+        store_at(env, transpose(c), st_half);
+      }
+    };
+    half(std::integral_constant<int, 0>{});
+    half(std::integral_constant<int, 1>{});
+    if (lane == 0) qcount[rwg * (RB / 64) + wave] = 0;
   } else {
     typedef float f2 __attribute__((ext_vector_type(2)));
     f2 lr2[PPT / 2], lf2[PPT / 2], lit2[PPT / 2];
@@ -291,16 +412,7 @@
     bool mixed = false;
 #pragma unroll
     for (int k = 0; k < PPT; ++k) mixed |= candm[k] != ~0ull;
-    uint32_t blk_reach;
-    {
-      float r2 = 0.f;
-#pragma unroll
-      for (int k = 0; k < PPT; ++k) r2 = fmaxf(r2, lr[k] * lr[k] + lf[k] * lf[k]);
-#pragma unroll
-      for (int d = 32; d > 0; d >>= 1) r2 = fmaxf(r2, __shfl_xor(r2, d));
-      const float r = fsqrt_(r2) * R.q_per_m * 1.0001f + 1.f;
-      blk_reach = (uint32_t)__builtin_amdgcn_readfirstlane((int)(r < 1.0e9f ? (uint32_t)r : 0x7FFFFFFFu));
-    }
+    const uint32_t blk_reach = block_reach(lr, lf);
     typedef uint4 Rec;
     struct QStage { Rec q[PPT]; f2 ax2[PPT / 2], az2[PPT / 2]; };
     auto issue_t = [&](const EnvV& f, QStage& st, auto clamp_tag) __attribute__((always_inline)) {
@@ -336,19 +448,6 @@
 #if DT_Q_PRIO
       __builtin_amdgcn_s_setprio(0);
 #endif
-    };
-    auto ground_rgb = [&](const GndK& c, const float lrk, const float lfk) __attribute__((always_inline)) -> uint32_t {
-      const float wx = c.Cx + lrk * c.sa + lfk * c.ca, wz = c.Cz + lrk * c.ca - lfk * c.sa;
-      const float wxg = fmaf(c.kg, wx - c.Cx, c.Cx), wzg = fmaf(c.kg, wz - c.Cz, c.Cz);
-      const float a = fminf(fmaxf((wxg + GROUND_HALF) * (0.5f / GROUND_HALF), 0.f), 1.f);
-      const float b = fminf(fmaxf((wzg + GROUND_HALF) * (0.5f / GROUND_HALF), 0.f), 1.f);
-      const float n0 = c.gndl[0] + a * (c.gndl[1] - c.gndl[0]), n1 = c.gndl[2] + a * (c.gndl[3] - c.gndl[2]);
-      const float ndl = n0 + b * (n1 - n0);
-      uint32_t rgb = 0;
-      rgb = __builtin_amdgcn_cvt_pk_u8_f32(c.gnd[0] * fminf(c.base[0] + c.dif[0] * ndl, 1.f), 0, rgb);
-      rgb = __builtin_amdgcn_cvt_pk_u8_f32(c.gnd[1] * fminf(c.base[1] + c.dif[1] * ndl, 1.f), 1, rgb);
-      rgb = __builtin_amdgcn_cvt_pk_u8_f32(c.gnd[2] * fminf(c.base[2] + c.dif[2] * ndl, 1.f), 2, rgb);
-      return rgb;
     };
     auto append_edges = [&](const int e, const unsigned long long em[PPT]) __attribute__((always_inline)) {
       const uint32_t etag = (uint32_t)(e - e0) << 8;
@@ -414,27 +513,7 @@
           if (!sk) continue;
           em[k] = sk;
           const unsigned long long gm = sk & __ballot((q[k].w >> 16) != 0u) & plainm[k];
-          if (gm) {
-            uint32_t mik = Mi[k];
-            asm volatile("" : "+v"(mik));
-            const float mrgk = __half2float(__ushort_as_half((unsigned short)(mik >> 16)));
-            const EnvFast g = fasts[env];
-            const EnvCam cc = cams[env];
-            GndK K;
-            K.Cx = cc.Cx; K.Cz = cc.Cz; K.sa = cc.sa; K.ca = cc.ca; K.kg = g.kg;
-#pragma unroll
-            for (int t = 0; t < 3; ++t) { K.gnd[t] = cc.gnd[t]; K.base[t] = cc.base[t]; K.dif[t] = cc.dif[t]; }
-#pragma unroll
-            for (int t = 0; t < 4; ++t) K.gndl[t] = cc.gndl[t];
-            const float wx = K.Cx + lr[k] * K.sa + lf[k] * K.ca, wz = K.Cz + lr[k] * K.ca - lf[k] * K.sa;
-            const float wxg = fmaf(K.kg, wx - K.Cx, K.Cx), wzg = fmaf(K.kg, wz - K.Cz, K.Cz);
-            const bool clear = (wx < -mrgk) | (wx > g.gw_m + mrgk) | (wz < -mrgk) | (wz > g.gh_m + mrgk);
-            const bool inq = (fabsf(wxg) + 2.f * mrgk < GROUND_HALF) & (fabsf(wzg) + 2.f * mrgk < GROUND_HALF);
-            const bool gfast = __builtin_amdgcn_inverse_ballot_w64(gm) & clear & inq;
-            const C3 gc = c3_of_rgb(ground_rgb(K, lr[k], lf[k]));
-            c[k].rb = gfast ? gc.rb : c[k].rb; c[k].g = gfast ? gc.g : c[k].g;
-            em[k] = sk & ~__ballot(gfast);
-          }
+          if (gm) em[k] = sk & ~ground_fast(lr[k], lf[k], Mi[k], env, gm, c[k]);
         }
       }
       if (OBJ && om) {
```

Result: slower. 2.688 million (-2.3%).
